# ChainSafe/co-zkvms

Measured on AMD Instinct MI355X. Metric: RISC-V cycles proved/sec (co-Jolt hot path: PST13 commit + dense GKR grand product + openings), higher is better.
Workload: dtype u32-limb BN254 Fr/Fq (254-bit Montgomery integers); 1 GPU; configs[1] restated (SURVEY 8d): 2^20-cycle trace per GPU, plain prover, 128 polys (64 Fr + 32 u16 + 16 u32 + 16 flags) PST13 batch commit, dense grand product 8 x 2^21 leaves, batch evaluate + opening reduction + PST13 open; log_n=20, polys=128, gp_batch=8, parallelism=single GPU, ranks_per_gpu=1

## Files before the change

### co-zkvms_amd/build.py

```python
import os
import subprocess
import sys

HERE = os.path.dirname(os.path.abspath(__file__))
CSRC = os.path.join(HERE, "csrc")
OUT = os.path.join(HERE, "libcozk.so")
PRIMS_SRC = os.path.join(os.path.dirname(HERE), "tests", "native", "prims.hip")
PRIMS_OUT = os.path.join(os.path.dirname(HERE), "tests", "native", "libcozk_prims.so")
HIPCC_FLAGS = ["--offload-arch=gfx950", "-O3", "-std=c++17", "-fPIC"]
SOURCES = ["capi.hip", "msm.hip", "poly.hip", "harness.hip", "shm_hub.hip", "ring.hip", "shamir.hip", "lasso_witness.hip", "rw_memory_witness.hip", "rw_memory_leaves.hip", "ts_range_witness.hip"]
HEADERS = [os.path.join("host", "spartan_pub_workers.hpp"), "fr9.hip.hpp", "fr9_consts.inc", os.path.join("host", "flow_harness.hpp"), os.path.join("host", "ts_range_proof.hpp"), os.path.join("host", "rw_memory_proof.hpp"), os.path.join("host", "jolt_r1cs.hpp"), os.path.join("host", "spartan_jolt.hpp"), "spartan_inner.inc", "ff.hip.hpp", "prf.hip.hpp", "ff_macc.inc", "ff_mul2.inc", "ec.hip.hpp", "fq9.hip.hpp", "fq9_consts.inc", "fq9_mac.inc", "fq9_mul.inc", "common.hpp", "lasso_walk.hip.hpp", "radix_pass.hip.hpp", "poly.hip.hpp", "toggle_layer.inc", "spartan_group.inc", "sparse_layer.inc", "primary_sumcheck.inc", "primary_group.inc", "shamir_deal.hip.hpp", "spartan_outer.inc", "outer_group.inc", "logup.inc", "compact_open.inc", "output_check.inc", os.path.join("host", "memory_proof.hpp"), os.path.join("host", "wire.hpp"), os.path.join("host", "net.hpp"), os.path.join("host", "prover.hpp"), os.path.join("host", "sparse_rule.hpp"), os.path.join("host", "split.hpp"), os.path.join("host", "split_harness.hpp"), os.path.join("host", "spartan_harness.hpp"), os.path.join("host", "lookups_harness.hpp"), os.path.join("host", "outer_harness.hpp"), os.path.join("host", "runner.hpp"), os.path.join("host", "shamir_gp.hpp"), os.path.join("host", "shamir_harness.hpp"), os.path.join("host", "shamir_spartan.hpp"), os.path.join("host", "shamir_jolt_spartan.hpp"), os.path.join("host", "shamir_primary.hpp"), os.path.join("..", "..", "include", "cozk.h")]


def _newer(target, deps):
    if not os.path.exists(target):
        return True
    t = os.path.getmtime(target)
    return any(os.path.getmtime(d) > t for d in deps)


def build(force=False, verbose=True):
    srcs = [os.path.join(CSRC, s) for s in SOURCES]
    deps = srcs + [os.path.join(CSRC, h) for h in HEADERS]
    objs = []
    os.makedirs(os.path.join(HERE, "build"), exist_ok=True)
    procs = []
    for s in srcs:
        o = os.path.join(HERE, "build", os.path.basename(s) + ".o")
        objs.append(o)
        if force or _newer(o, deps):
            cmd = ["hipcc"] + HIPCC_FLAGS + ["-c", s, "-o", o]
            if verbose:
                print(" ".join(cmd), flush=True)
            procs.append((cmd, subprocess.Popen(cmd)))
    for cmd, p in procs:
        if p.wait() != 0:
            raise RuntimeError("hipcc failed: " + " ".join(cmd))
    if force or procs or _newer(OUT, objs):
        cmd = ["hipcc", "--offload-arch=gfx950", "-shared", "-fPIC", "-o", OUT] + objs + ["-ldl"]
        if verbose:
            print(" ".join(cmd), flush=True)
        subprocess.check_call(cmd)
    build_prims(force, verbose)
    return OUT


def build_prims(force=False, verbose=True):
    if force or _newer(PRIMS_OUT, [PRIMS_SRC] + [os.path.join(CSRC, h) for h in HEADERS]):
        tmp = PRIMS_OUT[:-3] + ".tmp.so"
        cmd = ["hipcc"] + HIPCC_FLAGS + ["-shared", PRIMS_SRC, "-o", tmp]
        if verbose:
            print(" ".join(cmd), flush=True)
        subprocess.check_call(cmd)
        os.replace(tmp, PRIMS_OUT)
    return PRIMS_OUT


if __name__ == "__main__":
    if "--prims" in sys.argv:
        build_prims(force="--force" in sys.argv)
    else:
        build(force="--force" in sys.argv)
```

### co-zkvms_amd/csrc/ff.hip.hpp

```cpp
#pragma once
#include <hip/hip_runtime.h>
#include <stdint.h>

#define FF_HD __host__ __device__ __forceinline__
#if defined(__HIP_DEVICE_COMPILE__)
#include "ff_macc.inc"
#include "ff_mul2.inc"
#endif

struct alignas(16) fe {
    uint32_t l[8];
};

struct FrParams {
    static constexpr uint32_t MOD[8] = {0xf0000001u, 0x43e1f593u, 0x79b97091u, 0x2833e848u,
                                        0x8181585du, 0xb85045b6u, 0xe131a029u, 0x30644e72u};
    static constexpr uint32_t INV = 0xefffffffu;
    static constexpr uint32_t ONE[8] = {0x4ffffffbu, 0xac96341cu, 0x9f60cd29u, 0x36fc7695u,
                                        0x7879462eu, 0x666ea36fu, 0x9a07df2fu, 0x0e0a77c1u};
    static constexpr uint32_t R2[8] = {0xae216da7u, 0x1bb8e645u, 0xe35c59e3u, 0x53fe3ab1u,
                                       0x53bb8085u, 0x8c49833du, 0x7f4e44a5u, 0x0216d0b1u};
};

struct FqParams {
// ... 280 lines not shown
        MACC5_VS(lo, hi, m[0], m[1], m[2], m[3], m[4], P_(5), P_(4), P_(3), P_(2), P_(1));
        MSTEP_(5);
        MACC7_VV(lo, hi, A[0], A[1], A[2], A[3], A[4], A[5], A[6], B[6], B[5], B[4], B[3], B[2], B[1], B[0]);
        MACC7_VV(lo, hi, C[0], C[1], C[2], C[3], C[4], C[5], C[6], D[6], D[5], D[4], D[3], D[2], D[1], D[0]);
        MACC6_VS(lo, hi, m[0], m[1], m[2], m[3], m[4], m[5], P_(6), P_(5), P_(4), P_(3), P_(2), P_(1));
        MSTEP_(6);
        MACC8_VV(lo, hi, A[0], A[1], A[2], A[3], A[4], A[5], A[6], A[7], B[7], B[6], B[5], B[4], B[3], B[2], B[1], B[0]);
        MACC8_VV(lo, hi, C[0], C[1], C[2], C[3], C[4], C[5], C[6], C[7], D[7], D[6], D[5], D[4], D[3], D[2], D[1], D[0]);
        MACC7_VS(lo, hi, m[0], m[1], m[2], m[3], m[4], m[5], m[6], P_(7), P_(6), P_(5), P_(4), P_(3), P_(2), P_(1));
        MSTEP_(7);
        MACC7_VV(lo, hi, A[1], A[2], A[3], A[4], A[5], A[6], A[7], B[7], B[6], B[5], B[4], B[3], B[2], B[1]);
        MACC7_VV(lo, hi, C[1], C[2], C[3], C[4], C[5], C[6], C[7], D[7], D[6], D[5], D[4], D[3], D[2], D[1]);
        MACC7_VS(lo, hi, m[1], m[2], m[3], m[4], m[5], m[6], m[7], P_(7), P_(6), P_(5), P_(4), P_(3), P_(2), P_(1));
        r[0] = (uint32_t)lo; SHIFT_();
        MACC6_VV(lo, hi, A[2], A[3], A[4], A[5], A[6], A[7], B[7], B[6], B[5], B[4], B[3], B[2]);
        MACC6_VV(lo, hi, C[2], C[3], C[4], C[5], C[6], C[7], D[7], D[6], D[5], D[4], D[3], D[2]);
        MACC6_VS(lo, hi, m[2], m[3], m[4], m[5], m[6], m[7], P_(7), P_(6), P_(5), P_(4), P_(3), P_(2));
        r[1] = (uint32_t)lo; SHIFT_();
        MACC5_VV(lo, hi, A[3], A[4], A[5], A[6], A[7], B[7], B[6], B[5], B[4], B[3]);
        MACC5_VV(lo, hi, C[3], C[4], C[5], C[6], C[7], D[7], D[6], D[5], D[4], D[3]);
        MACC5_VS(lo, hi, m[3], m[4], m[5], m[6], m[7], P_(7), P_(6), P_(5), P_(4), P_(3));
        r[2] = (uint32_t)lo; SHIFT_();
        MACC4_VV(lo, hi, A[4], A[5], A[6], A[7], B[7], B[6], B[5], B[4]);
        MACC4_VV(lo, hi, C[4], C[5], C[6], C[7], D[7], D[6], D[5], D[4]);
        MACC4_VS(lo, hi, m[4], m[5], m[6], m[7], P_(7), P_(6), P_(5), P_(4));
        r[3] = (uint32_t)lo; SHIFT_();
        MACC3_VV(lo, hi, A[5], A[6], A[7], B[7], B[6], B[5]);
        MACC3_VV(lo, hi, C[5], C[6], C[7], D[7], D[6], D[5]);
        MACC3_VS(lo, hi, m[5], m[6], m[7], P_(7), P_(6), P_(5));
        r[4] = (uint32_t)lo; SHIFT_();
        MACC2_VV(lo, hi, A[6], A[7], B[7], B[6]);
        MACC2_VV(lo, hi, C[6], C[7], D[7], D[6]);
        MACC2_VS(lo, hi, m[6], m[7], P_(7), P_(6));
        r[5] = (uint32_t)lo; SHIFT_();
        MACC1_VV(lo, hi, A[7], B[7]);
        MACC1_VV(lo, hi, C[7], D[7]);
        MACC1_VS(lo, hi, m[7], P_(7));
        r[6] = (uint32_t)lo;
        r[7] = (uint32_t)(lo >> 32);
#undef P_
#undef SHIFT_
#undef MSTEP_
        fe o;
#pragma unroll
        for (int i = 0; i < 8; i++) o.l[i] = r[i];
        return o;
    }
#endif
    static FF_HD fe mul_sub2(const fe& a, const fe& b, const fe& c, const fe& d) { return mul_add2(a, b, neg(c), d); }

    static FF_HD void mul2(const fe& a, const fe& b, const fe& c, const fe& d, fe& o1, fe& o2) {
#if defined(__HIP_DEVICE_COMPILE__)
        uint64_t lo1 = 0, lo2 = 0;
        uint32_t hi1 = 0, hi2 = 0;
        uint32_t m1[8], m2[8], r1[8], r2[8];
        const uint32_t* A = a.l;
        const uint32_t* B = b.l;
        const uint32_t* C = c.l;
        const uint32_t* D = d.l;
        FF_MUL2_BODY
        fe t1, t2;
#pragma unroll
        for (int i = 0; i < 8; i++) {
            t1.l[i] = r1[i];
            t2.l[i] = r2[i];
        }
        o1 = reduce_once(t1);
        o2 = reduce_once(t2);
#else
        o1 = mul(a, b);
        o2 = mul(c, d);
#endif
    }

    static FF_HD fe two_mod() {
        fe r;
        uint32_t c = 0;
#pragma unroll
        for (int i = 0; i < 8; i++) {
            r.l[i] = (Pm::MOD[i] << 1) | c;
            c = Pm::MOD[i] >> 31;
        }
        return r;
    }
    static FF_HD fe lcanon(const fe& a) {
#if defined(__HIP_DEVICE_COMPILE__)
        return reduce_once(a);
#else
        return a;
#endif
    }
    static FF_HD fe lmul(const fe& a, const fe& b) {
#if defined(__HIP_DEVICE_COMPILE__)
        return mul_nr(a, b);
#else
        return mul(a, b);
#endif
    }
    static FF_HD void lmul2(const fe& a, const fe& b, const fe& c, const fe& d, fe& o1, fe& o2) {
#if defined(__HIP_DEVICE_COMPILE__)
        uint64_t lo1 = 0, lo2 = 0;
        uint32_t hi1 = 0, hi2 = 0;
        uint32_t m1[8], m2[8], r1[8], r2[8];
        const uint32_t* A = a.l;
        const uint32_t* B = b.l;
        const uint32_t* C = c.l;
        const uint32_t* D = d.l;
        FF_MUL2_BODY
#pragma unroll
        for (int i = 0; i < 8; i++) {
            o1.l[i] = r1[i];
            o2.l[i] = r2[i];
        }
#else
        o1 = mul(a, b);
        o2 = mul(c, d);
#endif
    }
    static FF_HD fe ladd(const fe& a, const fe& b) {
#if defined(__HIP_DEVICE_COMPILE__)
        fe s;
        uint64_t c = 0;
#pragma unroll
        for (int i = 0; i < 8; i++) {
            uint64_t t = (uint64_t)a.l[i] + b.l[i] + c;
            s.l[i] = (uint32_t)t;
            c = t >> 32;
        }
        const fe tm = two_mod();
        fe d;
        uint64_t borrow = 0;
#pragma unroll
        for (int i = 0; i < 8; i++) {
            uint64_t t = (uint64_t)s.l[i] - tm.l[i] - borrow;
            d.l[i] = (uint32_t)t;
            borrow = (t >> 63) & 1;
        }
        fe r;
#pragma unroll
        for (int i = 0; i < 8; i++) r.l[i] = borrow ? s.l[i] : d.l[i];
        return r;
#else
        return add(a, b);
#endif
    }
    static FF_HD fe lsub(const fe& a, const fe& b) {
#if defined(__HIP_DEVICE_COMPILE__)
        fe d;
        uint64_t borrow = 0;
#pragma unroll
        for (int i = 0; i < 8; i++) {
            uint64_t t = (uint64_t)a.l[i] - b.l[i] - borrow;
            d.l[i] = (uint32_t)t;
            borrow = (t >> 63) & 1;
        }
        const fe tm = two_mod();
        uint32_t mask = borrow ? 0xffffffffu : 0u;
        fe r;
        uint64_t c = 0;
#pragma unroll
        for (int i = 0; i < 8; i++) {
            uint64_t t = (uint64_t)d.l[i] + (tm.l[i] & mask) + c;
            r.l[i] = (uint32_t)t;
            c = t >> 32;
        }
        return r;
#else
        return sub(a, b);
#endif
    }
    static FF_HD fe ldbl(const fe& a) { return ladd(a, a); }
    static FF_HD fe lneg(const fe& a) { return lsub(zero(), a); }
    static FF_HD bool lis_zero(const fe& a) {
#if defined(__HIP_DEVICE_COMPILE__)
        uint32_t z = 0, m = 0;
#pragma unroll
        for (int i = 0; i < 8; i++) {
            z |= a.l[i];
            m |= a.l[i] ^ Pm::MOD[i];
        }
        return z == 0 || m == 0;
#else
        return is_zero(a);
#endif
    }
    static FF_HD fe lmul_sub2(const fe& a, const fe& b, const fe& c, const fe& d) {
#if defined(__HIP_DEVICE_COMPILE__)
        fe x = mul_add2_nr(a, b, lneg(c), d);
        const fe tm = two_mod();
        fe t;
        uint64_t borrow = 0;
#pragma unroll
        for (int i = 0; i < 8; i++) {
            uint64_t u = (uint64_t)x.l[i] - tm.l[i] - borrow;
            t.l[i] = (uint32_t)u;
            borrow = (u >> 63) & 1;
        }
        uint32_t mask = borrow ? 0u : 0xffffffffu;
        fe r;
        uint64_t bb = 0;
#pragma unroll
        for (int i = 0; i < 8; i++) {
            uint64_t u = (uint64_t)x.l[i] - (Pm::MOD[i] & mask) - bb;
            r.l[i] = (uint32_t)u;
            bb = (u >> 63) & 1;
        }
        return r;
#else
        return mul_sub2(a, b, c, d);
#endif
    }

    static FF_HD fe to_mont(const fe& a) { return mul(a, r2()); }
    static FF_HD fe from_mont(const fe& a) {
#if defined(__HIP_DEVICE_COMPILE__)
        uint64_t lo = 0;
        uint32_t hi = 0;
        uint32_t m[8], r[8];
        const uint32_t* A = a.l;
#define P_(j) Pm::MOD[j]
#define SHIFT_() lo = (lo >> 32) | ((uint64_t)hi << 32); hi = 0
#define ADDA_(k) { uint64_t t_ = lo + A[k]; hi += t_ < lo ? 1u : 0u; lo = t_; }
#define MSTEP_(k) m[k] = (uint32_t)lo * Pm::INV; MACC1_VS(lo, hi, m[k], P_(0)); SHIFT_()
        ADDA_(0);
        MSTEP_(0);
        ADDA_(1);
        MACC1_VS(lo, hi, m[0], P_(1));
        MSTEP_(1);
        ADDA_(2);
        MACC2_VS(lo, hi, m[0], m[1], P_(2), P_(1));
        MSTEP_(2);
        ADDA_(3);
        MACC3_VS(lo, hi, m[0], m[1], m[2], P_(3), P_(2), P_(1));
        MSTEP_(3);
        ADDA_(4);
        MACC4_VS(lo, hi, m[0], m[1], m[2], m[3], P_(4), P_(3), P_(2), P_(1));
        MSTEP_(4);
        ADDA_(5);
        MACC5_VS(lo, hi, m[0], m[1], m[2], m[3], m[4], P_(5), P_(4), P_(3), P_(2), P_(1));
        MSTEP_(5);
        ADDA_(6);
        MACC6_VS(lo, hi, m[0], m[1], m[2], m[3], m[4], m[5], P_(6), P_(5), P_(4), P_(3), P_(2), P_(1));
        MSTEP_(6);
        ADDA_(7);
        MACC7_VS(lo, hi, m[0], m[1], m[2], m[3], m[4], m[5], m[6], P_(7), P_(6), P_(5), P_(4), P_(3), P_(2), P_(1));
        MSTEP_(7);
        MACC7_VS(lo, hi, m[1], m[2], m[3], m[4], m[5], m[6], m[7], P_(7), P_(6), P_(5), P_(4), P_(3), P_(2), P_(1));
        r[0] = (uint32_t)lo; SHIFT_();
        MACC6_VS(lo, hi, m[2], m[3], m[4], m[5], m[6], m[7], P_(7), P_(6), P_(5), P_(4), P_(3), P_(2));
        r[1] = (uint32_t)lo; SHIFT_();
        MACC5_VS(lo, hi, m[3], m[4], m[5], m[6], m[7], P_(7), P_(6), P_(5), P_(4), P_(3));
        r[2] = (uint32_t)lo; SHIFT_();
        MACC4_VS(lo, hi, m[4], m[5], m[6], m[7], P_(7), P_(6), P_(5), P_(4));
        r[3] = (uint32_t)lo; SHIFT_();
        MACC3_VS(lo, hi, m[5], m[6], m[7], P_(7), P_(6), P_(5));
        r[4] = (uint32_t)lo; SHIFT_();
        MACC2_VS(lo, hi, m[6], m[7], P_(7), P_(6));
        r[5] = (uint32_t)lo; SHIFT_();
        MACC1_VS(lo, hi, m[7], P_(7));
        r[6] = (uint32_t)lo;
        r[7] = (uint32_t)(lo >> 32);
#undef P_
#undef SHIFT_
#undef ADDA_
#undef MSTEP_
        fe o;
#pragma unroll
        for (int i = 0; i < 8; i++) o.l[i] = r[i];
        return reduce_once(o);
#else
        fe o = zero();
        o.l[0] = 1;
        return mul(a, o);
#endif
    }
    static FF_HD fe from_u64(uint64_t v) {
        fe o = zero();
        o.l[0] = (uint32_t)v;
        o.l[1] = (uint32_t)(v >> 32);
        return to_mont(o);
    }
    static FF_HD fe pow(const fe& a, const uint32_t e[8]) {
        fe acc = one();
        for (int i = 7; i >= 0; i--) {
            for (int b = 31; b >= 0; b--) {
                acc = sqr(acc);
                if ((e[i] >> b) & 1) acc = mul(acc, a);
            }
        }
        return acc;
    }
    static FF_HD fe inv(const fe& a) {
        uint32_t e[8];
#pragma unroll
        for (int i = 0; i < 8; i++) e[i] = Pm::MOD[i];
        e[0] -= 2;
        return pow(a, e);
    }
};

typedef Field<FrParams> Fr;
typedef Field<FqParams> Fq;

static __device__ __forceinline__ fe fe_load(const fe* p) {
    const uint4* q = reinterpret_cast<const uint4*>(p);
    uint4 lo = q[0], hi = q[1];
    fe r;
    r.l[0] = lo.x; r.l[1] = lo.y; r.l[2] = lo.z; r.l[3] = lo.w;
    r.l[4] = hi.x; r.l[5] = hi.y; r.l[6] = hi.z; r.l[7] = hi.w;
    return r;
}
static __device__ __forceinline__ void fe_store(fe* p, const fe& v) {
    uint4* q = reinterpret_cast<uint4*>(p);
    q[0] = make_uint4(v.l[0], v.l[1], v.l[2], v.l[3]);
    q[1] = make_uint4(v.l[4], v.l[5], v.l[6], v.l[7]);
}
```

### co-zkvms_amd/csrc/poly.hip

```cpp
#include <atomic>
#include <chrono>
#include <map>
#include <mutex>
#include <string.h>
#include "poly.hip.hpp"
#include "prf.hip.hpp"
#include "fr9.hip.hpp"
#include "shamir_deal.hip.hpp"

static constexpr int PT = 256;
static constexpr int MAXBLK = 2048;
static constexpr unsigned ROUND_GRID_MAX = 1024;
static constexpr unsigned BATCH_GRID_MAX = 512;
static constexpr unsigned EVAL_GRID_MAX = 192;
static constexpr size_t LAYER_F9_MIN_CHUNKS = 1024;
static constexpr size_t LAYER_GROUPED_MIN_E1H = 512;

struct cozk_poly {
    cozk_ctx* ctx;
    int mode;
    fe* a0; fe* b0;
    bool own0;
    fe* buf[2][2];
    size_t cap[2];
    int cur;
    size_t len;
    size_t orig_len;
};

struct cozk_layer {
    cozk_ctx* ctx;
    int mode;
    fe* buf[2][2];
    size_t cap[2];
    int cur;
    size_t len;
};

struct cozk_spliteq {
    cozk_ctx* ctx;
    fe* E1[2]; fe* E2[2];
    int c1, c2;
    size_t E1_len, E2_len, E1_cap, E2_cap;
    int num_vars;
};

static inline unsigned grid_for(size_t n) { return (unsigned)((n + PT - 1) / PT); }
static inline unsigned grid_capped(size_t n, unsigned cap = MAXBLK) {
    size_t g = (n + PT - 1) / PT;
    return (unsigned)(g > cap ? cap : (g ? g : 1));
}
static inline unsigned sum_grid(unsigned gx) {
    const char* e = getenv("COZK_SUM_GRID_MAX");
    const long n = e ? atol(e) : 0;
    return n > 0 && (unsigned long)n < gx ? (unsigned)n : gx;
}

static unsigned eval_grid_max() {
    static const unsigned cap = getenv("COZK_EVAL_GX") ? (unsigned)atoi(getenv("COZK_EVAL_GX")) : EVAL_GRID_MAX;
    return cap;
}

static unsigned resident_grid(const void* kernel, size_t nblocks_needed, int device) {
    static const int legacy = getenv("COZK_RESIDENT_GRID") && atoi(getenv("COZK_RESIDENT_GRID")) == 0;
    if (legacy) return (unsigned)(nblocks_needed < 1024 ? (nblocks_needed ? nblocks_needed : 1) : 1024);
    static std::mutex mu;
    static std::map<std::pair<const void*, int>, unsigned> cache;
    unsigned cap;
    {
        std::lock_guard<std::mutex> g(mu);
        auto it = cache.find({kernel, device});
        if (it == cache.end()) {
            int per_cu = 0, cus = 0;
            HIP_TRY(hipOccupancyMaxActiveBlocksPerMultiprocessor(&per_cu, kernel, PT, 0));
            HIP_TRY(hipDeviceGetAttribute(&cus, hipDeviceAttributeMultiprocessorCount, device));
            unsigned v = (unsigned)(per_cu > 0 ? per_cu : 1) * (unsigned)(cus > 0 ? cus : 1);
            if (v > MAXBLK) v = MAXBLK;
            it = cache.emplace(std::make_pair(kernel, device), v).first;
        }
        cap = it->second;
    }
    return (unsigned)(nblocks_needed < cap ? (nblocks_needed ? nblocks_needed : 1) : cap);
}

static const fe* poly_a(const cozk_poly* p) { return p->cur < 0 ? p->a0 : p->buf[p->cur][0]; }
static const fe* poly_b(const cozk_poly* p) { return p->cur < 0 ? p->b0 : p->buf[p->cur][1]; }

template <int NC, int ORDER>
__global__ void __launch_bounds__(PT) k_poly_bind(const fe* __restrict__ ia, const fe* __restrict__ ib, fe* oa, fe* ob,
                                               size_t n_out, fe r) {
    size_t i = (size_t)blockIdx.x * PT + threadIdx.x;
    if (i >= n_out) return;
    size_t lo_i = ORDER == COZK_LOW_TO_HIGH ? 2 * i : i;
    size_t hi_i = ORDER == COZK_LOW_TO_HIGH ? 2 * i + 1 : i + n_out;
    Sh<NC> lo = sh_load<NC>(ia, ib, lo_i), hi = sh_load<NC>(ia, ib, hi_i);
    sh_store<NC>(oa, ob, i, sh_lerp<NC>(lo, hi, r));
}

template <int NC>
__global__ void __launch_bounds__(PT) k_poly_eval_chi(const fe* const* __restrict__ pa, const fe* const* __restrict__ pb,
                                                   const size_t* __restrict__ lens, const fe* __restrict__ chi, int k,
                                                   fe* __restrict__ partial) {
    __shared__ fe sh4[4];
    const int p0 = 2 * blockIdx.y, p1 = p0 + 1;
    const bool two = p1 < k;
    const fe* a0 = pa[p0];
    const fe* b0 = NC == 2 ? pb[p0] : nullptr;
    const fe* a1 = two ? pa[p1] : nullptr;
    const fe* b1 = (two && NC == 2) ? pb[p1] : nullptr;
    const size_t n0 = lens[p0], n1 = two ? lens[p1] : 0;
    const size_t n = n0 > n1 ? n0 : n1;
    FrWide w0, w1;
    fr_wide_zero(w0);
    fr_wide_zero(w1);
    for (size_t i = (size_t)blockIdx.x * PT + threadIdx.x; i < n; i += (size_t)gridDim.x * PT) {
        fe c = fe_load(chi + i);
        if (i < n0) fr_wide_mac(w0, sh_ab_sum<NC>(sh_load<NC>(a0, b0, i)), c);
        if (i < n1) fr_wide_mac(w1, sh_ab_sum<NC>(sh_load<NC>(a1, b1, i)), c);
    }
    fe acc = fr_block_sum(fr_wide_reduce(w0), sh4);
    if (threadIdx.x == 0) fe_store(partial + (size_t)p0 * gridDim.x + blockIdx.x, acc);
    if (two) {
        acc = fr_block_sum(fr_wide_reduce(w1), sh4);
        if (threadIdx.x == 0) fe_store(partial + (size_t)p1 * gridDim.x + blockIdx.x, acc);
    }
}

struct RoundPublish {
    unsigned* ticket;
    uint32_t* flag;
    uint32_t seq;
};
__global__ void __launch_bounds__(PT) k_finish_sums(const fe* __restrict__ partial, unsigned nper, fe scale, int apply_scale,
                                                 fe* __restrict__ out, RoundPublish pub) {
    __shared__ fe sh4[4];
    fe acc = Fr::zero();
    for (unsigned x = threadIdx.x; x < nper; x += PT) acc = Fr::add(acc, fe_load(partial + (size_t)blockIdx.x * nper + x));
    acc = fr_block_sum(acc, sh4);
    if (threadIdx.x == 0) {
        fe_store(out + blockIdx.x, apply_scale ? Fr::mul(acc, scale) : acc);
        if (pub.ticket) {
            __threadfence_system();
            if (atomicAdd(pub.ticket, 1u) == gridDim.x - 1) {
                *pub.ticket = 0;
                __threadfence_system();
                __hip_atomic_store(pub.flag, pub.seq, __ATOMIC_RELEASE, __HIP_MEMORY_SCOPE_SYSTEM);
            }
        }
    }
}

template <int NC>
__global__ void __launch_bounds__(PT) k_poly_dot_public(const fe* __restrict__ a, const fe* __restrict__ b,
                                                     const fe* __restrict__ pub, size_t n, fe* __restrict__ partial) {
    __shared__ fe sh4[4];
    FrWide w[NC];
#pragma unroll
    for (int k = 0; k < NC; k++) fr_wide_zero(w[k]);
    for (size_t i = (size_t)blockIdx.x * PT + threadIdx.x; i < n; i += (size_t)gridDim.x * PT) {
        Sh<NC> s = sh_load<NC>(a, b, i);
        fe p = fe_load(pub + i);
#pragma unroll
        for (int k = 0; k < NC; k++) fr_wide_mac(w[k], s.c[k], p);
    }
#pragma unroll
    for (int k = 0; k < NC; k++) {
        fe v = fr_block_sum(fr_wide_reduce(w[k]), sh4);
        if (threadIdx.x == 0) fe_store(partial + (size_t)k * gridDim.x + blockIdx.x, v);
    }
}

template <int NC>
__global__ void __launch_bounds__(PT) k_poly_lincomb(const fe* const* __restrict__ pa, const fe* const* __restrict__ pb,
                                                  const size_t* __restrict__ lens, const fe* __restrict__ coeffs, int k,
                                                  fe* oa, fe* ob, size_t n) {
    size_t i = (size_t)blockIdx.x * PT + threadIdx.x;
    if (i >= n) return;
    Sh<NC> acc;
    if (k >= 8) {
        FrWide w[NC];
#pragma unroll
        for (int c = 0; c < NC; c++) fr_wide_zero(w[c]);
        for (int j = 0; j < k; j++) {
            if (i < lens[j]) {
                fe cf = fe_load(coeffs + j);
                if (pa[j]) fr_wide_mac(w[0], fe_load(pa[j] + i), cf);
                if (NC == 2 && pb[j]) fr_wide_mac(w[NC - 1], fe_load(pb[j] + i), cf);
            }
        }
#pragma unroll
        for (int c = 0; c < NC; c++) acc.c[c] = fr_wide_reduce(w[c]);
        sh_store<NC>(oa, ob, i, acc);
        return;
    }
    for (int c = 0; c < NC; c++) acc.c[c] = Fr::zero();
    for (int j = 0; j < k; j++) {
        if (i < lens[j]) {
            fe cf = fe_load(coeffs + j);
            if (pa[j]) acc.c[0] = Fr::add(acc.c[0], Fr::mul(fe_load(pa[j] + i), cf));
            if (NC == 2 && pb[j]) acc.c[NC - 1] = Fr::add(acc.c[NC - 1], Fr::mul(fe_load(pb[j] + i), cf));
        }
    }
    sh_store<NC>(oa, ob, i, acc);
}

struct OpenQuadArgs {
    const fe* a[16];
    const fe* b[16];
    const fe* eq[16];
    size_t half[16];
};
template <int NC>
__global__ void __launch_bounds__(PT) k_open_quadratic_args(OpenQuadArgs args, fe* __restrict__ partial) {
    __shared__ fe sh4[4];
    const fe* a = args.a[blockIdx.y];
    const fe* b = NC == 2 ? args.b[blockIdx.y] : nullptr;
    const fe* eq = args.eq[blockIdx.y];
    size_t h = args.half[blockIdx.y];
    fe e0 = Fr::zero(), e2 = Fr::zero();
    for (size_t i = (size_t)blockIdx.x * PT + threadIdx.x; i < h; i += (size_t)gridDim.x * PT) {
        fe q0 = fe_load(eq + i), q1 = fe_load(eq + i + h);
        fe p0 = sh_ab_sum<NC>(sh_load<NC>(a, b, i)), p1 = sh_ab_sum<NC>(sh_load<NC>(a, b, i + h));
        e0 = Fr::add(e0, Fr::mul(p0, q0));
        fe pb2 = Fr::sub(Fr::dbl(p1), p0), qb2 = Fr::sub(Fr::dbl(q1), q0);
        e2 = Fr::add(e2, Fr::mul(pb2, qb2));
    }
    e0 = fr_block_sum(e0, sh4);
    if (threadIdx.x == 0) fe_store(partial + (size_t)(2 * blockIdx.y) * gridDim.x + blockIdx.x, e0);
    e2 = fr_block_sum(e2, sh4);
    if (threadIdx.x == 0) fe_store(partial + (size_t)(2 * blockIdx.y + 1) * gridDim.x + blockIdx.x, e2);
}

struct SmallCol {
    const void* p;
    int kind;
};
static __device__ __forceinline__ uint64_t small_load(const SmallCol& c, size_t i) {
    switch (c.kind) {
        case COZK_SCALAR_U8: return reinterpret_cast<const uint8_t*>(c.p)[i];
        case COZK_SCALAR_U16: return reinterpret_cast<const uint16_t*>(c.p)[i];
        case COZK_SCALAR_U32: return reinterpret_cast<const uint32_t*>(c.p)[i];
        default: return reinterpret_cast<const uint64_t*>(c.p)[i];
    }
}
template <int NC>
__global__ void __launch_bounds__(PT) k_fingerprint_leaves(const SmallCol* __restrict__ cols, const fe* __restrict__ cs, int ks,
                                                        const fe* const* __restrict__ pa, const fe* const* __restrict__ pb,
                                                        const fe* __restrict__ ds, int kp, fe constant, int pub_a, int pub_b, fe* oa, fe* ob,
                                                        size_t n) {
    size_t i = (size_t)blockIdx.x * PT + threadIdx.x;
    if (i >= n) return;
    fe pub = constant;
    for (int k = 0; k < ks; k++) {
        uint64_t v = small_load(cols[k], i);
        fe x = Fr::zero();
        x.l[0] = (uint32_t)v;
        x.l[1] = (uint32_t)(v >> 32);
        pub = Fr::add(pub, Fr::mul(fe_load(cs + k), x));
    }
    Sh<NC> acc;
    for (int c = 0; c < NC; c++) acc.c[c] = Fr::zero();
    for (int j = 0; j < kp; j++) {
        fe d = fe_load(ds + j);
        if (pa[j]) acc.c[0] = Fr::add(acc.c[0], Fr::mul(fe_load(pa[j] + i), d));
        if (NC == 2 && pb[j]) acc.c[NC - 1] = Fr::add(acc.c[NC - 1], Fr::mul(fe_load(pb[j] + i), d));
    }
    if (pub_a) acc.c[0] = Fr::add(acc.c[0], pub);
    if (NC == 2 && pub_b) acc.c[NC - 1] = Fr::add(acc.c[NC - 1], pub);
    sh_store<NC>(oa, ob, i, acc);
}

struct FingerprintArgs {
    SmallCol cols[16];
    fe cs[16];
    const fe* pa[8];
    const fe* pb[8];
    fe ds[8];
};
template <int NC>
__global__ void __launch_bounds__(PT) k_fingerprint_leaves_args(FingerprintArgs a, int ks, int kp, fe constant, int pub_a, int pub_b, fe* oa, fe* ob,
                                                             size_t n) {
    size_t i = (size_t)blockIdx.x * PT + threadIdx.x;
    if (i >= n) return;
    fe pub = constant;
    for (int k = 0; k < ks; k++) {
        uint64_t v = small_load(a.cols[k], i);
        fe x = Fr::zero();
        x.l[0] = (uint32_t)v;
        x.l[1] = (uint32_t)(v >> 32);
        pub = Fr::add(pub, Fr::mul(a.cs[k], x));
    }
    Sh<NC> acc;
    for (int c = 0; c < NC; c++) acc.c[c] = Fr::zero();
    for (int j = 0; j < kp; j++) {
        if (a.pa[j]) acc.c[0] = Fr::add(acc.c[0], Fr::mul(fe_load(a.pa[j] + i), a.ds[j]));
        if (NC == 2 && a.pb[j]) acc.c[NC - 1] = Fr::add(acc.c[NC - 1], Fr::mul(fe_load(a.pb[j] + i), a.ds[j]));
    }
    if (pub_a) acc.c[0] = Fr::add(acc.c[0], pub);
    if (NC == 2 && pub_b) acc.c[NC - 1] = Fr::add(acc.c[NC - 1], pub);
    sh_store<NC>(oa, ob, i, acc);
}

template <int NC>
__global__ void __launch_bounds__(PT) k_open_quadratic(const fe* const* __restrict__ pa, const fe* const* __restrict__ pb,
                                                    const fe* const* __restrict__ peq, const size_t* __restrict__ halves,
                                                    fe* __restrict__ partial) {
    __shared__ fe sh4[4];
    const fe* a = pa[blockIdx.y];
    const fe* b = NC == 2 ? pb[blockIdx.y] : nullptr;
    const fe* eq = peq[blockIdx.y];
    size_t h = halves[blockIdx.y];
    fe e0 = Fr::zero(), e2 = Fr::zero();
    for (size_t i = (size_t)blockIdx.x * PT + threadIdx.x; i < h; i += (size_t)gridDim.x * PT) {
        fe q0 = fe_load(eq + i), q1 = fe_load(eq + i + h);
        fe p0 = sh_ab_sum<NC>(sh_load<NC>(a, b, i)), p1 = sh_ab_sum<NC>(sh_load<NC>(a, b, i + h));
        e0 = Fr::add(e0, Fr::mul(p0, q0));
        fe pb2 = Fr::sub(Fr::dbl(p1), p0), qb2 = Fr::sub(Fr::dbl(q1), q0);
        e2 = Fr::add(e2, Fr::mul(pb2, qb2));
    }
    e0 = fr_block_sum(e0, sh4);
    if (threadIdx.x == 0) fe_store(partial + (size_t)(2 * blockIdx.y) * gridDim.x + blockIdx.x, e0);
    e2 = fr_block_sum(e2, sh4);
    if (threadIdx.x == 0) fe_store(partial + (size_t)(2 * blockIdx.y + 1) * gridDim.x + blockIdx.x, e2);
}

__global__ void __launch_bounds__(PT) k_pst_fold(const fe* __restrict__ r, fe* __restrict__ q, fe* __restrict__ rn, size_t half, fe p) {
    size_t i = (size_t)blockIdx.x * PT + threadIdx.x;
    if (i >= half) return;
    fe lo = fe_load(r + 2 * i), hi = fe_load(r + 2 * i + 1);
    fe d = Fr::sub(hi, lo);
    fe_store(q + i, d);
    fe_store(rn + i, Fr::add(lo, Fr::mul(d, p)));
}

template <int NC>
static __device__ __forceinline__ void layer_bind_chunk(const fe* ia, const fe* ib, size_t len_in, size_t ci, const fe& r, fe* oa, fe* ob, Sh<NC>& lo,
                                                        Sh<NC>& hi) {
    Sh<NC> u0 = sh_load_or_zero<NC>(ia, ib, 4 * ci, len_in), u1 = sh_load_or_zero<NC>(ia, ib, 4 * ci + 1, len_in);
    Sh<NC> u2 = sh_load_or_zero<NC>(ia, ib, 4 * ci + 2, len_in), u3 = sh_load_or_zero<NC>(ia, ib, 4 * ci + 3, len_in);
    lo = sh_lerp<NC>(u0, u2, r);
    sh_store<NC>(oa, ob, 2 * ci, lo);
    hi = sh_lerp<NC>(u1, u3, r);
    sh_store<NC>(oa, ob, 2 * ci + 1, hi);
}

static __device__ __forceinline__ void eq3(const fe& e0, const fe& e1, fe out[3]) {
    fe m = Fr::sub(e1, e0);
    out[0] = e0;
    out[1] = Fr::add(e1, m);
    out[2] = Fr::add(out[1], m);
}

static __device__ __forceinline__ size_t layer_chunk_count(size_t len, bool nested, size_t E1_half, size_t E2_len) {
    size_t nch = (len + 3) / 4;
    size_t limit = nested ? E1_half * E2_len : E2_len / 2;
    return nch > limit ? limit : nch;
}

static __device__ __forceinline__ void split_eq_at(bool nested, const fe* E1, int log_E1_half, const fe* E2, size_t c, fe e[3], fe& scale) {
    if (nested) {
        size_t x2 = c >> log_E1_half, x1 = c & (((size_t)1 << log_E1_half) - 1);
        eq3(fe_load(E1 + 2 * x1), fe_load(E1 + 2 * x1 + 1), e);
        scale = fe_load(E2 + x2);
    } else {
        eq3(fe_load(E2 + 2 * c), fe_load(E2 + 2 * c + 1), e);
    }
}
static __device__ __forceinline__ void layer_eq_at(bool nested, const fe* E1, size_t E1_half, const fe* E2, size_t c, fe e[3], fe& scale) {
    split_eq_at(nested, E1, __ffsll((long long)E1_half) - 1, E2, c, e, scale);
}
template <int NESTED>
static __device__ __forceinline__ size_t split_eq_limit(size_t E2_len, int log_E1_half) {
    return NESTED ? ((size_t)E2_len << log_E1_half) : E2_len / 2;
}
static __device__ __forceinline__ void partial_row_sum(fe v, fe* sh, fe* __restrict__ partial, size_t row) {
    v = fr_block_sum(v, sh);
    if (threadIdx.x == 0) fe_store(partial + row * gridDim.x + blockIdx.x, v);
}

template <int NC>
static __device__ __forceinline__ void layer_terms(const Sh<NC>& l0, const Sh<NC>& r0, const Sh<NC>& l1, const Sh<NC>& r1, const fe e[3], bool nested,
                                                   const fe& scale, fe& t0, fe& t2, fe& t3) {
    Sh<NC> ml = sh_sub<NC>(l1, l0), mr = sh_sub<NC>(r1, r0);
    Sh<NC> l2 = sh_add<NC>(l1, ml), r2 = sh_add<NC>(r1, mr);
    Sh<NC> l3 = sh_add<NC>(l2, ml), r3 = sh_add<NC>(r2, mr);
    t0 = Fr::mul(sh_local_mul<NC>(l0, r0), e[0]);
    t2 = Fr::mul(sh_local_mul<NC>(l2, r2), e[1]);
    t3 = Fr::mul(sh_local_mul<NC>(l3, r3), e[2]);
    if (nested) {
        t0 = Fr::mul(t0, scale);
        t2 = Fr::mul(t2, scale);
        t3 = Fr::mul(t3, scale);
    }
}

template <class Out>
static __device__ __forceinline__ void layer_finish(fe s0, fe s2, fe s3, fe* sh, Out out) {
    s0 = fr_block_sum(s0, sh);
    if (threadIdx.x == 0) fe_store(out(0), s0);
    s2 = fr_block_sum(s2, sh);
    if (threadIdx.x == 0) fe_store(out(1), s2);
    s3 = fr_block_sum(s3, sh);
    if (threadIdx.x == 0) fe_store(out(2), s3);
}

static __device__ __forceinline__ fe fold_pair(const fe* in, size_t i, const fe& r) {
    fe lo = fe_load(in + 2 * i), hi = fe_load(in + 2 * i + 1);
    return Fr::add(lo, Fr::mul(Fr::sub(hi, lo), r));
}

template <int NC>
__global__ void __launch_bounds__(PT) k_layer_bind(const fe* __restrict__ ia, const fe* __restrict__ ib, fe* oa, fe* ob,
                                                size_t len, fe r) {
    size_t c = (size_t)blockIdx.x * PT + threadIdx.x;
    size_t nch = (len + 3) / 4;
    if (c >= nch) return;
    Sh<NC> lo, hi;
    layer_bind_chunk<NC>(ia, ib, len, c, r, oa, ob, lo, hi);
}

template <int NC, int NESTED>
__global__ void __launch_bounds__(PT) k_layer_cubic(const fe* __restrict__ a, const fe* __restrict__ b, size_t len,
                                                 const fe* __restrict__ E1, size_t E1_half, const fe* __restrict__ E2,
                                                 size_t E2_len, fe* __restrict__ partial) {
    __shared__ fe sh4[4];
    const size_t nch = layer_chunk_count(len, NESTED, E1_half, E2_len);
    fe s0 = Fr::zero(), s2 = Fr::zero(), s3 = Fr::zero();
    for (size_t c = (size_t)blockIdx.x * PT + threadIdx.x; c < nch; c += (size_t)gridDim.x * PT) {
        fe e[3];
        fe scale;
        layer_eq_at(NESTED, E1, E1_half, E2, c, e, scale);
        Sh<NC> l0 = sh_load_or_zero<NC>(a, b, 4 * c, len), r0 = sh_load_or_zero<NC>(a, b, 4 * c + 1, len);
        Sh<NC> l1 = sh_load_or_zero<NC>(a, b, 4 * c + 2, len), r1 = sh_load_or_zero<NC>(a, b, 4 * c + 3, len);
        fe t0, t2, t3;
        layer_terms<NC>(l0, r0, l1, r1, e, NESTED, scale, t0, t2, t3);
        s0 = Fr::add(s0, t0);
        s2 = Fr::add(s2, t2);
        s3 = Fr::add(s3, t3);
    }
    layer_finish(s0, s2, s3, sh4, [&](unsigned k) { return partial + k * gridDim.x + blockIdx.x; });
}

template <int NC, int NESTED>
__global__ void __launch_bounds__(PT) k_layer_bind_cubic(const fe* __restrict__ ia, const fe* __restrict__ ib, fe* oa, fe* ob, size_t len_in, fe r,
                                                      const fe* __restrict__ E1, size_t E1_half, const fe* __restrict__ E2, size_t E2_len,
                                                      fe* __restrict__ partial) {
    __shared__ fe sh4[4];
    const size_t nch_in = (len_in + 3) / 4;
    const size_t len_out = 2 * nch_in;
    const size_t nch_out = (len_out + 3) / 4;
    const size_t nsum = layer_chunk_count(len_out, NESTED, E1_half, E2_len);
    fe s0 = Fr::zero(), s2 = Fr::zero(), s3 = Fr::zero();
    for (size_t c = (size_t)blockIdx.x * PT + threadIdx.x; c < nch_out; c += (size_t)gridDim.x * PT) {
        Sh<NC> v[4];
#pragma unroll
        for (int h = 0; h < 2; h++) {
            size_t ci = 2 * c + h;
            if (ci < nch_in) {
                layer_bind_chunk<NC>(ia, ib, len_in, ci, r, oa, ob, v[2 * h], v[2 * h + 1]);
            } else {
                for (int k = 0; k < NC; k++) v[2 * h].c[k] = v[2 * h + 1].c[k] = Fr::zero();
            }
        }
        if (c < nsum) {
            fe e[3];
            fe scale;
            layer_eq_at(NESTED, E1, E1_half, E2, c, e, scale);
            fe t0, t2, t3;
            layer_terms<NC>(v[0], v[1], v[2], v[3], e, NESTED, scale, t0, t2, t3);
            s0 = Fr::add(s0, t0);
            s2 = Fr::add(s2, t2);
            s3 = Fr::add(s3, t3);
        }
    }
    layer_finish(s0, s2, s3, sh4, [&](unsigned k) { return partial + k * gridDim.x + blockIdx.x; });
}

struct Layer9Group {
    f9 g0, g2, g3;
    size_t x2;
};
static __device__ __forceinline__ void layer9_group_flush(Layer9Group& grp, const fe* __restrict__ E2, f9& s0, f9& s2, f9& s3) {
    if (grp.x2 == (size_t)-1) return;
    const f9 sc = f9_from_fe(fe_load(E2 + grp.x2));
    s0 = f9_norm(fr9_add(s0, fr9_mul(grp.g0, sc)));
    s2 = f9_norm(fr9_add(s2, fr9_mul(grp.g2, sc)));
    s3 = f9_norm(fr9_add(s3, fr9_mul(grp.g3, sc)));
}
template <int NESTED>
static __device__ __forceinline__ void layer9_fold(size_t it, f9& s0, f9& s2, f9& s3, Layer9Group& grp) {
    if (it == 0 || (it & (FR9_FOLD_PERIOD - 1)) != 0) return;
    fr9_fold(s0);
    fr9_fold(s2);
    fr9_fold(s3);
    if (NESTED == 2) {
        fr9_fold(grp.g0);
        fr9_fold(grp.g2);
        fr9_fold(grp.g3);
    }
}
template <int NC, int NESTED>
static __device__ __forceinline__ void layer9_terms(const Sh9<NC>& l0, const Sh9<NC>& r0, const Sh9<NC>& l1, const Sh9<NC>& r1, const fe* __restrict__ E1,
                                                    size_t E1_half, int e1_shift, const fe* __restrict__ E2, size_t c, f9& s0, f9& s2, f9& s3,
                                                    Layer9Group& grp) {
    f9 e0, e1;
    if (NESTED == 2) {
        const size_t x2 = c >> e1_shift, x1 = c & (E1_half - 1);
        if (x2 != grp.x2) {
            layer9_group_flush(grp, E2, s0, s2, s3);
            grp.g0 = grp.g2 = grp.g3 = fr9_zero();
            grp.x2 = x2;
        }
        e0 = f9_from_fe(fe_load(E1 + 2 * x1));
        e1 = f9_from_fe(fe_load(E1 + 2 * x1 + 1));
    } else if (NESTED) {
        const size_t x2 = c >> e1_shift, x1 = c & (E1_half - 1);
        const f9 sc = f9_from_fe(fe_load(E2 + x2));
        e0 = fr9_mul(f9_from_fe(fe_load(E1 + 2 * x1)), sc);
        e1 = fr9_mul(f9_from_fe(fe_load(E1 + 2 * x1 + 1)), sc);
    } else {
        e0 = f9_from_fe(fe_load(E2 + 2 * c));
        e1 = f9_from_fe(fe_load(E2 + 2 * c + 1));
    }
    const f9 me = f9_norm(f9_sub(e1, FR9_C2, e0));
    const f9 e2 = fr9_add(e1, me), e3 = fr9_add(e2, me);
    const Sh9<NC> ml = sh9_diff<NC>(l1, l0), mr = sh9_diff<NC>(r1, r0);
    const Sh9<NC> l2 = sh9_add_norm<NC>(l1, ml), r2 = sh9_add_norm<NC>(r1, mr);
    const Sh9<NC> l3 = sh9_add_norm<NC>(l2, ml), r3 = sh9_add_norm<NC>(r2, mr);
    f9& a0 = NESTED == 2 ? grp.g0 : s0;
    f9& a2 = NESTED == 2 ? grp.g2 : s2;
    f9& a3 = NESTED == 2 ? grp.g3 : s3;
    a0 = f9_norm(fr9_add(a0, fr9_mul(e0, sh9_local_mul<NC>(l0, r0))));
    a2 = f9_norm(fr9_add(a2, fr9_mul(e2, sh9_local_mul<NC>(l2, r2))));
    a3 = f9_norm(fr9_add(a3, fr9_mul(e3, sh9_local_mul<NC>(l3, r3))));
}
static __device__ __forceinline__ void layer9_walk(int nested, size_t nch, size_t& first, size_t& end, size_t& step) {
    if (nested == 2) {
        const size_t per = ((nch + gridDim.x - 1) / gridDim.x + PT - 1) / PT * PT;
        first = (size_t)blockIdx.x * per + (threadIdx.x & ~63u);
        end = (size_t)(blockIdx.x + 1) * per < nch ? (size_t)(blockIdx.x + 1) * per : nch;
        step = PT;
    } else {
        first = (size_t)blockIdx.x * PT + (threadIdx.x & ~63u);
        end = nch;
        step = (size_t)gridDim.x * PT;
    }
}
template <int NESTED>
static __device__ __forceinline__ void layer9_finish(const f9& s0, const f9& s2, const f9& s3, fe* __restrict__ partial, fe* sh4) {
    const f9 K = f9_const(NESTED ? FR9_K3 : FR9_K2);
    fe v = fr_block_sum(fr9_to_canonical(fr9_mul(s0, K)), sh4);
    if (threadIdx.x == 0) fe_store(partial + blockIdx.x, v);
    v = fr_block_sum(fr9_to_canonical(fr9_mul(s2, K)), sh4);
    if (threadIdx.x == 0) fe_store(partial + gridDim.x + blockIdx.x, v);
    v = fr_block_sum(fr9_to_canonical(fr9_mul(s3, K)), sh4);
    if (threadIdx.x == 0) fe_store(partial + 2 * gridDim.x + blockIdx.x, v);
}


static constexpr int ST_ROW = 144;
static constexpr int ST_WAVE_BYTES = 64 * ST_ROW;
static __device__ __forceinline__ void stage_fence() {
    __builtin_amdgcn_fence(__ATOMIC_RELEASE, "wavefront");
    __builtin_amdgcn_wave_barrier();
    __builtin_amdgcn_fence(__ATOMIC_ACQUIRE, "wavefront");
}
static __device__ __forceinline__ void stage_in_rows(const char* __restrict__ g, size_t row_stride, char* st, fe out[4]) {
    const int lane = threadIdx.x & 63, piece = lane & 7, sub = lane >> 3;
    uint4 t[8];
#pragma unroll
    for (int k = 0; k < 8; k++) t[k] = *reinterpret_cast<const uint4*>(g + (size_t)(8 * k + sub) * row_stride + 16 * piece);
#pragma unroll
    for (int k = 0; k < 8; k++) *reinterpret_cast<uint4*>(st + (8 * k + sub) * ST_ROW + 16 * piece) = t[k];
    stage_fence();
#pragma unroll
    for (int j = 0; j < 4; j++) {
        const uint4 lo = *reinterpret_cast<const uint4*>(st + lane * ST_ROW + 32 * j);
        const uint4 hi = *reinterpret_cast<const uint4*>(st + lane * ST_ROW + 32 * j + 16);
        out[j].l[0] = lo.x; out[j].l[1] = lo.y; out[j].l[2] = lo.z; out[j].l[3] = lo.w;
        out[j].l[4] = hi.x; out[j].l[5] = hi.y; out[j].l[6] = hi.z; out[j].l[7] = hi.w;
    }
    stage_fence();
}
static __device__ __forceinline__ void stage_out_rows(char* __restrict__ g, char* st, const fe in[4], size_t row_stride = 128) {
    const int lane = threadIdx.x & 63, piece = lane & 7, sub = lane >> 3;
#pragma unroll
    for (int j = 0; j < 4; j++) {
        *reinterpret_cast<uint4*>(st + lane * ST_ROW + 32 * j) = make_uint4(in[j].l[0], in[j].l[1], in[j].l[2], in[j].l[3]);
        *reinterpret_cast<uint4*>(st + lane * ST_ROW + 32 * j + 16) = make_uint4(in[j].l[4], in[j].l[5], in[j].l[6], in[j].l[7]);
    }
    stage_fence();
#pragma unroll
    for (int k = 0; k < 8; k++)
        *reinterpret_cast<uint4*>(g + (size_t)(8 * k + sub) * row_stride + 16 * piece) = *reinterpret_cast<const uint4*>(st + (8 * k + sub) * ST_ROW + 16 * piece);
    stage_fence();
}

template <int NC, int NESTED>
__global__ void __launch_bounds__(PT) k_layer_cubic9(const fe* __restrict__ a, const fe* __restrict__ b, size_t len, const fe* __restrict__ E1, size_t E1_half,
                                                  const fe* __restrict__ E2, size_t E2_len, fe* __restrict__ partial) {
    __shared__ fe sh4[4];
    __shared__ __attribute__((aligned(16))) char stage[PT / 64][ST_WAVE_BYTES];
    char* st = stage[threadIdx.x >> 6];
    size_t nch = (len + 3) / 4;
    const size_t limit = NESTED ? E1_half * E2_len : E2_len / 2;
    if (nch > limit) nch = limit;
    const int e1_shift = NESTED ? __ffsll((long long)E1_half) - 1 : 0;
    f9 s0 = fr9_zero(), s2 = fr9_zero(), s3 = fr9_zero();
    Layer9Group grp;
    grp.g0 = grp.g2 = grp.g3 = fr9_zero();
    grp.x2 = (size_t)-1;
    size_t c_first, c_end, c_step;
    layer9_walk(NESTED, nch, c_first, c_end, c_step);
    size_t it = 0;
    for (size_t c0 = c_first; c0 < c_end; c0 += c_step, it++) {
        layer9_fold<NESTED>(it, s0, s2, s3, grp);
        const size_t c = c0 + (threadIdx.x & 63);
        if (c0 + 64 <= nch && 4 * (c0 + 64) <= len) {
            Sh9<NC> q[4];
            const fe* comp[2] = {a, b};
#pragma unroll
            for (int k = 0; k < NC; k++) {
                fe raw[4];
                stage_in_rows(reinterpret_cast<const char*>(comp[k] + 4 * c0), 128, st, raw);
#pragma unroll
                for (int j = 0; j < 4; j++) q[j].c[k] = f9_from_fe(raw[j]);
            }
            layer9_terms<NC, NESTED>(q[0], q[1], q[2], q[3], E1, E1_half, e1_shift, E2, c, s0, s2, s3, grp);
        } else if (c < nch) {
            const Sh9<NC> l0 = sh9_load_or_zero<NC>(a, b, 4 * c, len), r0 = sh9_load_or_zero<NC>(a, b, 4 * c + 1, len);
            const Sh9<NC> l1 = sh9_load_or_zero<NC>(a, b, 4 * c + 2, len), r1 = sh9_load_or_zero<NC>(a, b, 4 * c + 3, len);
            layer9_terms<NC, NESTED>(l0, r0, l1, r1, E1, E1_half, e1_shift, E2, c, s0, s2, s3, grp);
        }
    }
    if (NESTED == 2) layer9_group_flush(grp, E2, s0, s2, s3);
    layer9_finish<NESTED>(s0, s2, s3, partial, sh4);
}

template <int NC, int NESTED>
__global__ void __launch_bounds__(PT) k_layer_bind_cubic9(const fe* __restrict__ ia, const fe* __restrict__ ib, fe* oa, fe* ob, size_t len_in, fe r5,
                                                       const fe* __restrict__ E1, size_t E1_half, const fe* __restrict__ E2, size_t E2_len,
                                                       fe* __restrict__ partial) {
    __shared__ fe sh4[4];
    const size_t nch_in = (len_in + 3) / 4;
    const size_t len_out = 2 * nch_in;
    const size_t nch_out = (len_out + 3) / 4;
    const size_t limit = NESTED ? E1_half * E2_len : E2_len / 2;
    const int e1_shift = NESTED ? __ffsll((long long)E1_half) - 1 : 0;
    const f9 r9 = f9_from_fe(r5);
    f9 s0 = fr9_zero(), s2 = fr9_zero(), s3 = fr9_zero();
    __shared__ __attribute__((aligned(16))) char stage[PT / 64][ST_WAVE_BYTES];
    char* st = stage[threadIdx.x >> 6];
    Layer9Group grp;
    grp.g0 = grp.g2 = grp.g3 = fr9_zero();
    grp.x2 = (size_t)-1;
    size_t c_first, c_end, c_step;
    layer9_walk(NESTED, nch_out, c_first, c_end, c_step);
    size_t it = 0;
    for (size_t c0 = c_first; c0 < c_end; c0 += c_step, it++) {
        layer9_fold<NESTED>(it, s0, s2, s3, grp);
        const size_t c = c0 + (threadIdx.x & 63);
        Sh9<NC> v[4];
        if (c0 + 64 <= nch_out && 8 * (c0 + 64) <= len_in) {
            const fe* icomp[2] = {ia, ib};
            fe* ocomp[2] = {oa, ob};
#pragma unroll
            for (int h = 0; h < 2; h++) {
                Sh9<NC> u[4];
#pragma unroll
                for (int k = 0; k < NC; k++) {
                    fe raw[4];
                    stage_in_rows(reinterpret_cast<const char*>(icomp[k] + 8 * c0 + 4 * h), 256, st, raw);
#pragma unroll
                    for (int j = 0; j < 4; j++) u[j].c[k] = f9_from_fe(raw[j]);
                }
                v[2 * h] = sh9_lerp<NC>(u[0], u[2], r9);
                v[2 * h + 1] = sh9_lerp<NC>(u[1], u[3], r9);
            }
#pragma unroll
            for (int k = 0; k < NC; k++) {
                fe outv[4];
#pragma unroll
                for (int j = 0; j < 4; j++) outv[j] = fr9_to_canonical(v[j].c[k]);
                stage_out_rows(reinterpret_cast<char*>(ocomp[k] + 4 * c0), st, outv);
            }
            if (c < limit) layer9_terms<NC, NESTED>(v[0], v[1], v[2], v[3], E1, E1_half, e1_shift, E2, c, s0, s2, s3, grp);
            continue;
        }
        if (c >= nch_out) continue;
#pragma unroll
        for (int h = 0; h < 2; h++) {
            const size_t ci = 2 * c + h;
            if (ci < nch_in) {
                const Sh9<NC> u0 = sh9_load_or_zero<NC>(ia, ib, 4 * ci, len_in), u1 = sh9_load_or_zero<NC>(ia, ib, 4 * ci + 1, len_in);
                const Sh9<NC> u2 = sh9_load_or_zero<NC>(ia, ib, 4 * ci + 2, len_in), u3 = sh9_load_or_zero<NC>(ia, ib, 4 * ci + 3, len_in);
                v[2 * h] = sh9_lerp<NC>(u0, u2, r9);
                v[2 * h + 1] = sh9_lerp<NC>(u1, u3, r9);
                sh9_store<NC>(oa, ob, 2 * ci, v[2 * h]);
                sh9_store<NC>(oa, ob, 2 * ci + 1, v[2 * h + 1]);
            } else {
                for (int k = 0; k < NC; k++) v[2 * h].c[k] = v[2 * h + 1].c[k] = fr9_zero();
            }
        }
        if (c < limit) layer9_terms<NC, NESTED>(v[0], v[1], v[2], v[3], E1, E1_half, e1_shift, E2, c, s0, s2, s3, grp);
    }
    if (NESTED == 2) layer9_group_flush(grp, E2, s0, s2, s3);
    layer9_finish<NESTED>(s0, s2, s3, partial, sh4);
}

static constexpr int RT = 1024;
static constexpr size_t ROUND_SMALL_MAX = 2048;
template <int NC>
__global__ void __launch_bounds__(RT) k_layer_round_small(const fe* __restrict__ ia, const fe* __restrict__ ib, fe* oa, fe* ob, size_t len_in,
                                                       int do_bind, fe r, const fe* fold_in, fe* fold_out, size_t fold_n, fe* scale_vec,
                                                       size_t scale_n, const fe* ca, const fe* cb, size_t len, const fe* E1, size_t E1_half,
                                                       const fe* E2, size_t E2_len, int nested, fe* __restrict__ res) {
    __shared__ fe sh16[16];
    if (do_bind) {
        size_t nch_in = (len_in + 3) / 4;
        for (size_t c = threadIdx.x; c < nch_in; c += RT) {
            Sh<NC> lo, hi;
            layer_bind_chunk<NC>(ia, ib, len_in, c, r, oa, ob, lo, hi);
        }
        for (size_t i = threadIdx.x; i < fold_n; i += RT) fe_store(fold_out + i, fold_pair(fold_in, i, r));
        __syncthreads();
        if (scale_n) {
            fe s = fe_load(fold_out);
            for (size_t i = threadIdx.x; i < scale_n; i += RT) fe_store(scale_vec + i, Fr::mul(fe_load(scale_vec + i), s));
            __syncthreads();
        }
    }
    size_t nch = (len + 3) / 4;
    size_t limit = nested ? E1_half * E2_len : E2_len / 2;
    if (nch > limit) nch = limit;
    fe s0 = Fr::zero(), s2 = Fr::zero(), s3 = Fr::zero();
    for (size_t c = threadIdx.x; c < nch; c += RT) {
        fe e[3];
        fe scale = Fr::zero();
        if (nested) {
            size_t x2 = c >> (__ffsll((long long)E1_half) - 1), x1 = c & (E1_half - 1);
            eq3(fe_load(E1 + 2 * x1), fe_load(E1 + 2 * x1 + 1), e);
            scale = fe_load(E2 + x2);
        } else {
            eq3(fe_load(E2 + 2 * c), fe_load(E2 + 2 * c + 1), e);
        }
        Sh<NC> l0 = sh_load_or_zero<NC>(ca, cb, 4 * c, len), r0 = sh_load_or_zero<NC>(ca, cb, 4 * c + 1, len);
        Sh<NC> l1 = sh_load_or_zero<NC>(ca, cb, 4 * c + 2, len), r1 = sh_load_or_zero<NC>(ca, cb, 4 * c + 3, len);
        fe t0, t2, t3;
        layer_terms<NC>(l0, r0, l1, r1, e, nested, scale, t0, t2, t3);
        s0 = Fr::add(s0, t0);
        s2 = Fr::add(s2, t2);
        s3 = Fr::add(s3, t3);
    }
    layer_finish(s0, s2, s3, sh16, [&](unsigned k) { return res + k; });
}

struct LayerGroupArgs {
    const fe* ia[COZK_LAYER_GROUP_MAX];
    const fe* ib[COZK_LAYER_GROUP_MAX];
    fe* oa[COZK_LAYER_GROUP_MAX];
    fe* ob[COZK_LAYER_GROUP_MAX];
};
template <int NC>
__global__ void __launch_bounds__(RT) k_layer_group_round_small(LayerGroupArgs a, size_t len_in, int do_bind, fe r, size_t len, const fe* E1, size_t E1_half,
                                                             const fe* E2, size_t E2_len, int nested, fe* __restrict__ res) {
    __shared__ fe sh16[16];
    const unsigned m = blockIdx.x;
    const size_t c = threadIdx.x;
    const fe *ca = a.ia[m], *cb = a.ib[m];
    if (do_bind) {
        const fe *ia = a.ia[m], *ib = a.ib[m];
        fe *oa = a.oa[m], *ob = a.ob[m];
        if (c < (len_in + 3) / 4) {
#pragma unroll 1
            for (int h = 0; h < 2; h++) {
                const Sh<NC> lo = sh_load_or_zero<NC>(ia, ib, 4 * c + h, len_in), hi = sh_load_or_zero<NC>(ia, ib, 4 * c + 2 + h, len_in);
                sh_store<NC>(oa, ob, 2 * c + h, sh_lerp<NC>(lo, hi, r));
            }
        }
        __syncthreads();
        ca = oa;
        cb = ob;
    }
    const bool on = c < layer_chunk_count(len, nested, E1_half, E2_len);
    const fe* ep = E2 + 2 * c;
    const fe* sp = nullptr;
    if (nested) {
        ep = E1 + 2 * (c & (E1_half - 1));
        sp = E2 + (c >> (__ffsll((long long)E1_half) - 1));
    }
    auto side = [&](int s, int X) {
        const Sh<NC> v0 = sh_load_or_zero<NC>(ca, cb, 4 * c + s, len), v1 = sh_load_or_zero<NC>(ca, cb, 4 * c + 2 + s, len);
        if (X == 0) return v0;
        const Sh<NC> d = sh_sub<NC>(v1, v0);
        Sh<NC> v = sh_add<NC>(v1, d);
        if (X == 3) v = sh_add<NC>(v, d);
        return v;
    };
#pragma unroll 1
    for (int p = 0; p < 3; p++) {
        const int X = p ? p + 1 : 0;
        fe t = Fr::zero();
        if (on) {
            fe e = fe_load(ep);
            if (X) {
                const fe e1 = fe_load(ep + 1), d = Fr::sub(e1, e);
                e = Fr::add(e1, d);
                if (X == 3) e = Fr::add(e, d);
            }
            if (nested) e = Fr::mul(e, fe_load(sp));
            t = Fr::mul(sh_local_mul<NC>(side(0, X), side(1, X)), e);
        }
        t = fr_block_sum(t, sh16);
        if (threadIdx.x == 0) fe_store(res + 3 * m + p, t);
    }
}

static constexpr int GFT = 64;
template <int NC>
__global__ void __launch_bounds__(GFT) k_layer_group_final(LayerGroupArgs a, size_t len_in, int do_bind, fe r, fe* __restrict__ res) {
    const unsigned m = blockIdx.x, j = threadIdx.x;
    if (j >= 2) return;
    const fe *ia = a.ia[m], *ib = a.ib[m];
    Sh<NC> v;
    if (do_bind) {
        v = sh_lerp<NC>(sh_load_or_zero<NC>(ia, ib, j, len_in), sh_load_or_zero<NC>(ia, ib, j + 2, len_in), r);
        sh_store<NC>(a.oa[m], a.ob[m], j, v);
    } else {
        v = sh_load<NC>(ia, ib, j);
    }
    for (int c = 0; c < NC; c++) fe_store(res + (size_t)(2 * m + j) * NC + c, v.c[c]);
}

struct alignas(64) RoundMailbox {
    uint32_t cmd[16];
    uint32_t pad0[16];
    uint32_t res_seq;
    uint32_t status;
    uint32_t pad2[14];
    fe res[4];
    unsigned long long dbg[8];
};
static constexpr long long MB_TICKS_PER_S = 100000000ll;
static int resident_timeout_s() {
    const char* e = getenv("COZK_RESIDENT_TIMEOUT_S");
    int t = e ? atoi(e) : 10;
    return t < 1 ? 1 : (t > 600 ? 600 : t);
}
static constexpr size_t ROUND_PERSIST_MAX = 2048;

template <int NC, int TRACE>
__global__ void __launch_bounds__(RT) k_layer_rounds_persistent(fe* la0, fe* lb0, fe* la1, fe* lb1, int lcur, size_t len, fe* e1_0, fe* e1_1,
                                                             int c1, size_t E1_len, fe* e2_0, fe* e2_1, int c2, size_t E2_len, int nrounds,
                                                             int bind_first, fe r_first, RoundMailbox* mb, long long timeout_ticks) {
    __shared__ fe sh16[16];
    __shared__ fe sh_r;
    __shared__ int sh_ok;
    fe* la[2] = {la0, la1};
    fe* lb[2] = {lb0, lb1};
    fe* e1[2] = {e1_0, e1_1};
    fe* e2[2] = {e2_0, e2_1};
    uint32_t seq = 0;
    long long tk0 = TRACE ? wall_clock64() : 0, tk_wait = 0, tk_bind = 0, tk_cubic = 0, tk_pub = 0;
    for (int round = 0; round <= nrounds; round++) {
        bool do_bind = round > 0 || bind_first;
        fe r = r_first;
        if (TRACE) tk0 = wall_clock64();
        if (round > 0) {
            if (threadIdx.x < 64) {
                typedef uint32_t v4u __attribute__((ext_vector_type(4)));
                const int lane = threadIdx.x;
                const long long t0 = wall_clock64();
                int ok = 1;
                v4u v = {0u, 0u, 0u, 0u};
                for (;;) {
                    if (lane < 4) v = *reinterpret_cast<volatile v4u*>(&mb->cmd[4 * lane]);
                    const unsigned long long ready = __ballot(lane < 3 && v.w == (uint32_t)round);
                    const unsigned long long aborted = __ballot(lane == 3 && v.x != 0u);
                    if ((ready & 7ull) == 7ull) break;
                    if (aborted) {
                        ok = 0;
                        if (lane == 0) __hip_atomic_store(&mb->status, 2u, __ATOMIC_RELEASE, __HIP_MEMORY_SCOPE_SYSTEM);
                        break;
                    }
                    if (__shfl((int)(wall_clock64() - t0 > timeout_ticks), 0)) {
                        ok = 0;
                        if (lane == 0) __hip_atomic_store(&mb->status, 1u, __ATOMIC_RELEASE, __HIP_MEMORY_SCOPE_SYSTEM);
                        break;
                    }
                    __builtin_amdgcn_s_sleep(2);
                }
                fe rr;
                rr.l[0] = __shfl(v.x, 0); rr.l[1] = __shfl(v.y, 0); rr.l[2] = __shfl(v.z, 0);
                rr.l[3] = __shfl(v.x, 1); rr.l[4] = __shfl(v.y, 1); rr.l[5] = __shfl(v.z, 1);
                rr.l[6] = __shfl(v.x, 2); rr.l[7] = __shfl(v.y, 2);
                if (lane == 0) {
                    if (ok) sh_r = rr;
                    sh_ok = ok;
                }
            }
            __syncthreads();
            if (!sh_ok) return;
            r = sh_r;
        }
        if (TRACE) {
            long long t = wall_clock64();
            tk_wait += t - tk0;
            tk0 = t;
        }
        if (do_bind) {
            const fe *ia = la[lcur], *ib = lb[lcur];
            fe *oa = la[1 - lcur], *ob = lb[1 - lcur];
            size_t nch_in = (len + 3) / 4;
            for (size_t c = threadIdx.x; c < nch_in; c += RT) {
                Sh<NC> lo, hi;
                layer_bind_chunk<NC>(ia, ib, len, c, r, oa, ob, lo, hi);
            }
            lcur = 1 - lcur;
            len = 2 * nch_in;
            if (E1_len == 1) {
                size_t n = E2_len / 2;
                const fe* in = e2[c2];
                fe* out = e2[1 - c2];
                for (size_t i = RT - 1 - threadIdx.x; i < n; i += RT) fe_store(out + i, fold_pair(in, i, r));
                c2 = 1 - c2;
                E2_len = n;
                __syncthreads();
            } else {
                size_t n = E1_len / 2;
                const fe* in = e1[c1];
                fe* out = e1[1 - c1];
                for (size_t i = RT - 1 - threadIdx.x; i < n; i += RT) fe_store(out + i, fold_pair(in, i, r));
                c1 = 1 - c1;
                E1_len = n;
                __syncthreads();
                if (n == 1) {
                    fe sc = fe_load(e1[c1]);
                    fe* v = e2[c2];
                    for (size_t i = threadIdx.x; i < E2_len; i += RT) fe_store(v + i, Fr::mul(fe_load(v + i), sc));
                    __syncthreads();
                }
            }
        }
        seq++;
        if (TRACE) {
            long long t = wall_clock64();
            tk_bind += t - tk0;
            tk0 = t;
        }
        if (round == nrounds) {
            if (threadIdx.x == 0) {
                mb->dbg[0] = (unsigned long long)tk_wait;
                mb->dbg[1] = (unsigned long long)tk_bind;
                mb->dbg[2] = (unsigned long long)tk_cubic;
                mb->dbg[3] = (unsigned long long)tk_pub;
                fe z = Fr::zero();
                fe v[4] = {fe_load(la[lcur]), NC == 2 ? fe_load(lb[lcur]) : z, fe_load(la[lcur] + 1), NC == 2 ? fe_load(lb[lcur] + 1) : z};
                for (int k = 0; k < 4; k++) fe_store(&mb->res[k], v[k]);
                __threadfence_system();
                __hip_atomic_store(&mb->res_seq, seq, __ATOMIC_RELEASE, __HIP_MEMORY_SCOPE_SYSTEM);
            }
            return;
        }
        const fe *ca = la[lcur], *cb = lb[lcur];
        const fe *E1 = e1[c1], *E2 = e2[c2];
        const bool nested = E1_len != 1;
        const size_t E1_half = E1_len / 2;
        const size_t nch = layer_chunk_count(len, nested, E1_half, E2_len);
        const int wave = threadIdx.x >> 6;
        const int pt = wave / 5;
        fe acc = Fr::zero();
        if (pt < 3) {
            for (size_t c = threadIdx.x - 320 * pt; c < nch; c += 320) {
                fe e0, e1v, ek;
                if (nested) {
                    size_t x2 = c >> (__ffsll((long long)E1_half) - 1), x1 = c & (E1_half - 1);
                    e0 = fe_load(E1 + 2 * x1);
                    e1v = fe_load(E1 + 2 * x1 + 1);
                } else {
                    e0 = fe_load(E2 + 2 * c);
                    e1v = fe_load(E2 + 2 * c + 1);
                }
                Sh<NC> l0 = sh_load_or_zero<NC>(ca, cb, 4 * c, len), r0 = sh_load_or_zero<NC>(ca, cb, 4 * c + 1, len);
                Sh<NC> lk = l0, rk = r0;
                ek = e0;
                if (pt > 0) {
                    Sh<NC> l1 = sh_load_or_zero<NC>(ca, cb, 4 * c + 2, len), r1 = sh_load_or_zero<NC>(ca, cb, 4 * c + 3, len);
                    Sh<NC> ml = sh_sub<NC>(l1, l0), mr = sh_sub<NC>(r1, r0);
                    fe me = Fr::sub(e1v, e0);
                    lk = sh_add<NC>(l1, ml);
                    rk = sh_add<NC>(r1, mr);
                    ek = Fr::add(e1v, me);
                    if (pt == 2) {
                        lk = sh_add<NC>(lk, ml);
                        rk = sh_add<NC>(rk, mr);
                        ek = Fr::add(ek, me);
                    }
                }
                fe lr = sh_local_mul<NC>(lk, rk);
                fe es = nested ? Fr::mul(ek, fe_load(E2 + (c >> (__ffsll((long long)E1_half) - 1)))) : ek;
                acc = Fr::add(acc, Fr::mul(lr, es));
            }
        }
        acc = fr_wave_sum(acc);
        __syncthreads();
        if ((threadIdx.x & 63) == 0) sh16[wave] = acc;
        __syncthreads();
        if (TRACE) {
            long long t = wall_clock64();
            tk_cubic += t - tk0;
            tk0 = t;
        }
        if (threadIdx.x < 3) {
            fe v = sh16[5 * threadIdx.x];
            for (int i = 1; i < 5; i++) v = Fr::add(v, sh16[5 * threadIdx.x + i]);
            fe_store(&mb->res[threadIdx.x], v);
            __threadfence_system();
        }
        __syncthreads();
        if (threadIdx.x == 0) __hip_atomic_store(&mb->res_seq, seq, __ATOMIC_RELEASE, __HIP_MEMORY_SCOPE_SYSTEM);
        if (TRACE) {
            long long t = wall_clock64();
            tk_pub += t - tk0;
            tk0 = t;
        }
    }
}

template <int NC>
__global__ void __launch_bounds__(PT) k_layer_output(const fe* __restrict__ a, const fe* __restrict__ b, size_t len,
                                                  fe* __restrict__ out, size_t n_out, int masked, prf_key key_self,
                                                  prf_key key_prev, uint64_t ctr) {
    size_t j = (size_t)blockIdx.x * PT + threadIdx.x;
    if (j >= n_out) return;
    Sh<NC> l = sh_load_or_zero<NC>(a, b, 2 * j, len), r = sh_load_or_zero<NC>(a, b, 2 * j + 1, len);
    fe v = sh_local_mul<NC>(l, r);
    if (masked) v = Fr::add(v, Fr::sub(prf_fr(key_self, ctr + j), prf_fr(key_prev, ctr + j)));
    fe_store(out + j, v);
}

template <int NC>
__global__ void __launch_bounds__(PT) k_mul_vec_local(const fe* __restrict__ xa, const fe* __restrict__ xb,
                                                   const fe* __restrict__ ya, const fe* __restrict__ yb, size_t n,
                                                   fe* __restrict__ out, int masked, prf_key key_self, prf_key key_prev,
                                                   uint64_t ctr) {
    size_t j = (size_t)blockIdx.x * PT + threadIdx.x;
    if (j >= n) return;
    fe v = sh_local_mul<NC>(sh_load<NC>(xa, xb, j), sh_load<NC>(ya, yb, j));
    if (masked) v = Fr::add(v, Fr::sub(prf_fr(key_self, ctr + j), prf_fr(key_prev, ctr + j)));
    fe_store(out + j, v);
}

struct ProdRoundPtrs {
    const fe* a[4];
    const fe* b[4];
};
template <int NC, int M>
__global__ void __launch_bounds__(PT) k_prod_round(ProdRoundPtrs tab, int shared_idx, size_t half, int degree, fe* __restrict__ partial) {
    const fe* const* pa = tab.a;
    const fe* const* pb = tab.b;
    __shared__ fe sh4[4];
    fe acc[4];
    for (int e = 0; e < 4; e++) acc[e] = Fr::zero();
    for (size_t i = (size_t)blockIdx.x * PT + threadIdx.x; i < half; i += (size_t)gridDim.x * PT) {
        fe cur[M], step[M];
        for (int j = 0; j < M; j++) {
            fe lo, hi;
            if (NC == 2 && j == shared_idx) {
                lo = Fr::add(fe_load(pa[j] + i), fe_load(pb[j] + i));
                hi = Fr::add(fe_load(pa[j] + i + half), fe_load(pb[j] + i + half));
            } else {
                lo = fe_load(pa[j] + i);
                hi = fe_load(pa[j] + i + half);
            }
            step[j] = Fr::sub(hi, lo);
            cur[j] = lo;
        }
        for (int e = 0; e < degree; e++) {
            if (e == 1)
                for (int j = 0; j < M; j++) cur[j] = Fr::add(Fr::add(cur[j], step[j]), step[j]);
            else if (e > 1)
                for (int j = 0; j < M; j++) cur[j] = Fr::add(cur[j], step[j]);
            fe prod = cur[0];
            for (int j = 1; j < M; j++) prod = Fr::mul(prod, cur[j]);
            acc[e] = Fr::add(acc[e], prod);
        }
    }
    for (int e = 0; e < degree; e++) {
        fe v = fr_block_sum(acc[e], sh4);
        if (threadIdx.x == 0) fe_store(partial + (size_t)e * gridDim.x + blockIdx.x, v);
    }
}

template <int NC>
__global__ void __launch_bounds__(PT) k_spartan_first(const fe* __restrict__ aa, const fe* __restrict__ ab, const fe* __restrict__ ba,
                                                   const fe* __restrict__ bb, const fe* __restrict__ ca, const fe* __restrict__ cb,
                                                   const fe* __restrict__ pub, size_t half, fe* __restrict__ partial) {
    __shared__ fe sh4[4];
    fe accp[4], accc[4];
    for (int e = 0; e < 4; e++) {
        accp[e] = Fr::zero();
        accc[e] = Fr::zero();
    }
    for (size_t b = (size_t)blockIdx.x * PT + threadIdx.x; b < half; b += (size_t)gridDim.x * PT) {
        Sh<NC> A = sh_load<NC>(aa, ab, 2 * b), B = sh_load<NC>(ba, bb, 2 * b), C = sh_load<NC>(ca, cb, 2 * b);
        Sh<NC> sA = sh_sub<NC>(sh_load<NC>(aa, ab, 2 * b + 1), A), sB = sh_sub<NC>(sh_load<NC>(ba, bb, 2 * b + 1), B),
               sC = sh_sub<NC>(sh_load<NC>(ca, cb, 2 * b + 1), C);
        fe P = fe_load(pub + 2 * b);
        fe sP = Fr::sub(fe_load(pub + 2 * b + 1), P);
        for (int e = 0; e < 4; e++) {
            accp[e] = Fr::add(accp[e], Fr::mul(sh_local_mul<NC>(A, B), P));
            accc[e] = Fr::add(accc[e], Fr::mul(sh_ab_sum<NC>(C), P));
            A = sh_add<NC>(A, sA);
            B = sh_add<NC>(B, sB);
            C = sh_add<NC>(C, sC);
            P = Fr::add(P, sP);
        }
    }
    for (int e = 0; e < 4; e++) {
        fe v = fr_block_sum(accp[e], sh4);
        if (threadIdx.x == 0) fe_store(partial + (size_t)e * gridDim.x + blockIdx.x, v);
        fe w = fr_block_sum(accc[e], sh4);
        if (threadIdx.x == 0) fe_store(partial + (size_t)(4 + e) * gridDim.x + blockIdx.x, w);
    }
}

template <int NC>
__global__ void __launch_bounds__(PT) k_spartan_second(const fe* __restrict__ za, const fe* __restrict__ zb, const fe* __restrict__ pa,
                                                    const fe* __restrict__ pbv, const fe* __restrict__ pc, fe c0, fe c1, fe c2,
                                                    size_t half, fe* __restrict__ partial) {
    __shared__ fe sh4[4];
    fe acc[NC][3];
    for (int k = 0; k < NC; k++)
        for (int e = 0; e < 3; e++) acc[k][e] = Fr::zero();
    for (size_t b = (size_t)blockIdx.x * PT + threadIdx.x; b < half; b += (size_t)gridDim.x * PT) {
        Sh<NC> Z = sh_load<NC>(za, zb, 2 * b);
        Sh<NC> sZ = sh_sub<NC>(sh_load<NC>(za, zb, 2 * b + 1), Z);
        fe A = fe_load(pa + 2 * b), B = fe_load(pbv + 2 * b), C = fe_load(pc + 2 * b);
        fe sA = Fr::sub(fe_load(pa + 2 * b + 1), A), sB = Fr::sub(fe_load(pbv + 2 * b + 1), B), sC = Fr::sub(fe_load(pc + 2 * b + 1), C);
        for (int e = 0; e < 3; e++) {
            fe lin = Fr::add(Fr::add(Fr::mul(A, c0), Fr::mul(B, c1)), Fr::mul(C, c2));
            for (int k = 0; k < NC; k++) acc[k][e] = Fr::add(acc[k][e], Fr::mul(Z.c[k], lin));
            Z = sh_add<NC>(Z, sZ);
            A = Fr::add(A, sA);
            B = Fr::add(B, sB);
            C = Fr::add(C, sC);
        }
    }
    for (int k = 0; k < NC; k++)
        for (int e = 0; e < 3; e++) {
            fe v = fr_block_sum(acc[k][e], sh4);
            if (threadIdx.x == 0) fe_store(partial + (size_t)(3 * k + e) * gridDim.x + blockIdx.x, v);
        }
}

static constexpr uint32_t SPMV_LONG = 64;
static constexpr uint32_t SPMV_CHUNK = 2048;
template <int NC>
__global__ void __launch_bounds__(PT) k_sparse_matvec3(const uint32_t* __restrict__ row_ptr, const uint32_t* __restrict__ col,
                                                    const fe* __restrict__ va, const fe* __restrict__ vb, const fe* __restrict__ vc,
                                                    const fe* __restrict__ za, const fe* __restrict__ zb, size_t nrows,
                                                    fe* oa0, fe* oa1, fe* ob0, fe* ob1, fe* oc0, fe* oc1,
                                                    uint32_t* __restrict__ q, uint32_t* __restrict__ q_rows, uint32_t* __restrict__ q_items) {
    size_t r = (size_t)blockIdx.x * PT + threadIdx.x;
    if (r >= nrows) return;
    uint32_t e0 = row_ptr[r], e1 = row_ptr[r + 1];
    if (e1 - e0 > SPMV_LONG) {
        uint32_t nchunks = (e1 - e0 + SPMV_CHUNK - 1) / SPMV_CHUNK;
        uint32_t ri = atomicAdd(&q[0], 1u);
        uint32_t first = atomicAdd(&q[1], nchunks);
        q_rows[3 * ri] = (uint32_t)r;
        q_rows[3 * ri + 1] = first;
        q_rows[3 * ri + 2] = nchunks;
        for (uint32_t j = 0; j < nchunks; j++) {
            q_items[2 * (first + j)] = (uint32_t)r;
            q_items[2 * (first + j) + 1] = j;
        }
        return;
    }
    Sh<NC> A, B, C;
    for (int k = 0; k < NC; k++) A.c[k] = B.c[k] = C.c[k] = Fr::zero();
    for (uint32_t e = e0; e < e1; e++) {
        Sh<NC> z = sh_load<NC>(za, zb, col[e]);
        A = sh_add<NC>(A, sh_mul_public<NC>(z, fe_load(va + e)));
        B = sh_add<NC>(B, sh_mul_public<NC>(z, fe_load(vb + e)));
        C = sh_add<NC>(C, sh_mul_public<NC>(z, fe_load(vc + e)));
    }
    sh_store<NC>(oa0, oa1, r, A);
    sh_store<NC>(ob0, ob1, r, B);
    sh_store<NC>(oc0, oc1, r, C);
}
template <int NC>
__global__ void __launch_bounds__(PT) k_sparse_matvec3_items(const uint32_t* __restrict__ row_ptr, const uint32_t* __restrict__ col,
                                                          const fe* __restrict__ va, const fe* __restrict__ vb, const fe* __restrict__ vc,
                                                          const fe* __restrict__ za, const fe* __restrict__ zb, const uint32_t* __restrict__ q,
                                                          const uint32_t* __restrict__ q_items, fe* __restrict__ partial) {
    __shared__ fe sh4[4];
    uint32_t nitems = q[1];
    for (uint32_t it = blockIdx.x; it < nitems; it += gridDim.x) {
        uint32_t r = q_items[2 * it], j = q_items[2 * it + 1];
        uint32_t lo = row_ptr[r] + j * SPMV_CHUNK;
        uint32_t hi = min(lo + SPMV_CHUNK, row_ptr[r + 1]);
        Sh<NC> A, B, C;
        for (int k = 0; k < NC; k++) A.c[k] = B.c[k] = C.c[k] = Fr::zero();
        for (uint32_t e = lo + threadIdx.x; e < hi; e += PT) {
            Sh<NC> z = sh_load<NC>(za, zb, col[e]);
            A = sh_add<NC>(A, sh_mul_public<NC>(z, fe_load(va + e)));
            B = sh_add<NC>(B, sh_mul_public<NC>(z, fe_load(vb + e)));
            C = sh_add<NC>(C, sh_mul_public<NC>(z, fe_load(vc + e)));
        }
        fe* out = partial + (size_t)it * 3 * NC;
        for (int k = 0; k < NC; k++) {
            fe a = fr_block_sum(A.c[k], sh4), b = fr_block_sum(B.c[k], sh4), c = fr_block_sum(C.c[k], sh4);
            if (threadIdx.x == 0) {
                fe_store(out + k, a);
                fe_store(out + NC + k, b);
                fe_store(out + 2 * NC + k, c);
            }
        }
    }
}
template <int NC>
__global__ void __launch_bounds__(PT) k_sparse_matvec3_rows(const uint32_t* __restrict__ q, const uint32_t* __restrict__ q_rows,
                                                         const fe* __restrict__ partial, fe* oa0, fe* oa1, fe* ob0, fe* ob1, fe* oc0, fe* oc1) {
    __shared__ fe sh4[4];
    uint32_t nlong = q[0];
    for (uint32_t ri = blockIdx.x; ri < nlong; ri += gridDim.x) {
        uint32_t r = q_rows[3 * ri], first = q_rows[3 * ri + 1], n = q_rows[3 * ri + 2];
        fe acc[3 * NC];
        for (int k = 0; k < 3 * NC; k++) acc[k] = Fr::zero();
        for (uint32_t j = threadIdx.x; j < n; j += PT)
            for (int k = 0; k < 3 * NC; k++) acc[k] = Fr::add(acc[k], fe_load(partial + (size_t)(first + j) * 3 * NC + k));
        fe tot[3 * NC];
        for (int k = 0; k < 3 * NC; k++) tot[k] = fr_block_sum(acc[k], sh4);
        if (threadIdx.x == 0) {
            Sh<NC> A, B, C;
            for (int k = 0; k < NC; k++) {
                A.c[k] = tot[k];
                B.c[k] = tot[NC + k];
                C.c[k] = tot[2 * NC + k];
            }
            sh_store<NC>(oa0, oa1, r, A);
            sh_store<NC>(ob0, ob1, r, B);
            sh_store<NC>(oc0, oc1, r, C);
        }
    }
}

__global__ void __launch_bounds__(PT) k_fold_pairs(const fe* __restrict__ in, fe* __restrict__ out, size_t n_out, fe r) {
    size_t i = (size_t)blockIdx.x * PT + threadIdx.x;
    if (i >= n_out) return;
    fe_store(out + i, fold_pair(in, i, r));
}
__global__ void __launch_bounds__(PT) k_fold_halves(fe* __restrict__ v, size_t n_out, fe r) {
    size_t i = (size_t)blockIdx.x * PT + threadIdx.x;
    if (i >= n_out) return;
    fe lo = fe_load(v + i), hi = fe_load(v + i + n_out);
    fe_store(v + i, Fr::add(lo, Fr::mul(Fr::sub(hi, lo), r)));
}
__global__ void __launch_bounds__(PT) k_scale_by_first(fe* __restrict__ v, size_t n, const fe* __restrict__ s) {
    size_t i = (size_t)blockIdx.x * PT + threadIdx.x;
    if (i >= n) return;
    fe_store(v + i, Fr::mul(fe_load(v + i), fe_load(s)));
}
__global__ void __launch_bounds__(PT) k_eq_expand(const fe* __restrict__ in, fe* __restrict__ out, size_t n_in, fe rj) {
    size_t i = (size_t)blockIdx.x * PT + threadIdx.x;
    if (i >= n_in) return;
    fe e = fe_load(in + i);
    fe hi = Fr::mul(e, rj);
    fe_store(out + 2 * i, Fr::sub(e, hi));
    fe_store(out + 2 * i + 1, hi);
}

__global__ void k_store_fe(fe* out, fe v) { fe_store(out, v); }
__global__ void k_store_u32s(uint32_t* out, const uint32_t* __restrict__ in0, const uint32_t* __restrict__ in1, int n0, size_t stride0) {
    int i = threadIdx.x;
    if (i < n0) out[i] = in0[(size_t)i * stride0];
    if (i == n0 && in1) out[n0] = *in1;
}
struct EqBuildPoint {
    fe r[13];
};
__global__ void __launch_bounds__(1024) k_eq_build(EqBuildPoint pt, int nv, fe* __restrict__ out) {
    if (threadIdx.x == 0) fe_store(out, Fr::one());
    __syncthreads();
    size_t n = 1;
    for (int j = 0; j < nv; j++) {
        fe rj = pt.r[j];
        fe e[8];
        int cnt = 0;
        for (size_t i = threadIdx.x; i < n; i += 1024) e[cnt++] = fe_load(out + i);
        __syncthreads();
        cnt = 0;
        for (size_t i = threadIdx.x; i < n; i += 1024) {
            fe hi = Fr::mul(e[cnt], rj);
            fe_store(out + 2 * i, Fr::sub(e[cnt], hi));
            fe_store(out + 2 * i + 1, hi);
            cnt++;
        }
        __syncthreads();
        n *= 2;
    }
}

static fe* dev_alloc_fe(size_t n) { return (fe*)ctx_dev_alloc(t_cur_ctx, (n ? n : 1) * sizeof(fe)); }

static bool sync_rounds() {
    static const bool on = getenv("COZK_SYNC_ROUNDS") != nullptr;
    return on;
}
static bool trace_rounds() {
    static const bool on = getenv("COZK_TRACE_ROUNDS") != nullptr;
    return on;
}

static void stream_drain_by_flag(cozk_ctx* ctx) {
    if (sync_rounds()) {
        HIP_TRY(hipStreamSynchronize(ctx->stream));
        return;
    }
    if (!ctx->round_flag) HIP_TRY(hipHostMalloc((void**)&ctx->round_flag, 64, hipHostMallocMapped | hipHostMallocCoherent));
    uint32_t seq = ++ctx->round_seq;
    HIP_TRY(hipStreamWriteValue32(ctx->stream, (void*)ctx->round_flag, seq, 0));
    volatile uint32_t* f = ctx->round_flag;
    uint64_t spins = 0;
    while (*f != seq) {
        __builtin_ia32_pause();
        if (++spins > (1ull << 22)) {
            HIP_TRY(hipStreamSynchronize(ctx->stream));
            break;
        }
    }
}
static RoundPublish arm_round_publish(cozk_ctx* ctx) {
    static const bool on = !(getenv("COZK_FLAG_IN_FINISH") && atoi(getenv("COZK_FLAG_IN_FINISH")) == 0);
    if (!on || sync_rounds()) return RoundPublish{nullptr, nullptr, 0};
    if (!ctx->round_flag) HIP_TRY(hipHostMalloc((void**)&ctx->round_flag, 64, hipHostMallocMapped | hipHostMallocCoherent));
    if (!ctx->finish_ticket) {
        HIP_TRY(hipMalloc((void**)&ctx->finish_ticket, 64));
        HIP_TRY(hipMemsetAsync(ctx->finish_ticket, 0, 64, ctx->stream));
    }
    ctx->armed_seq = ++ctx->round_seq;
    return RoundPublish{ctx->finish_ticket, ctx->round_flag, ctx->armed_seq};
}
static void fetch_fe(cozk_ctx* ctx, const fe* d, size_t k, fe* h) {
    fe* pin = (fe*)ctx_pinned(ctx, k * sizeof(fe));
    const uint32_t armed = ctx->armed_seq;
    ctx->armed_seq = 0;
    if (d == pin && armed) {
        volatile uint32_t* f = ctx->round_flag;
        uint64_t spins = 0;
        while (*f != armed) {
            __builtin_ia32_pause();
            if (++spins > (1ull << 22)) {
                HIP_TRY(hipStreamSynchronize(ctx->stream));
                break;
            }
        }
        std::atomic_thread_fence(std::memory_order_acquire);
    } else {
        if (d != pin) HIP_TRY(hipMemcpyAsync(pin, d, k * sizeof(fe), hipMemcpyDeviceToHost, ctx->stream));
        stream_drain_by_flag(ctx);
    }
    for (size_t i = 0; i < k; i++) h[i] = pin[i];
}
static fe* result_slot(cozk_ctx* ctx, size_t k) { return (fe*)ctx_pinned(ctx, k * sizeof(fe)); }

struct SumLaunch {
    fe* partial;
    fe* res;
    char* meta;
    size_t cap;
    size_t n_res;
};
static SumLaunch sum_launch(cozk_ctx* ctx, unsigned rows, unsigned gx_max, size_t n_res, size_t meta_bytes = 0) {
    const size_t meta = (meta_bytes + 31) & ~(size_t)31, cap = (size_t)rows * gx_max;
    ctx->scratch.reserve(meta + (cap + rows) * sizeof(fe));
    char* base = (char*)ctx->scratch.p;
    return SumLaunch{(fe*)(base + meta), result_slot(ctx, n_res), base, cap, n_res};
}
static void finish_sums(cozk_ctx* ctx, const SumLaunch& sl, unsigned rows, unsigned gx, fe scale, int apply_scale, fe* out) {
    COZK_REQUIRE((size_t)rows * gx <= sl.cap && rows <= sl.n_res, "finish_sums: more block partials than sum_launch reserved");
    struct Disarm {
        cozk_ctx* ctx;
        ~Disarm() { ctx->armed_seq = 0; }
    } disarm{ctx};
    k_finish_sums<<<rows, PT, 0, ctx->stream>>>(sl.partial, gx, scale, apply_scale, sl.res, arm_round_publish(ctx));
    HIP_TRY(hipGetLastError());
    fetch_fe(ctx, sl.res, sl.n_res, out);
}


static void drain_streams(const std::vector<cozk_ctx*>& owners, const cozk_ctx* skip = nullptr) {
    for (size_t i = 0; i < owners.size(); i++) {
        cozk_ctx* c = owners[i];
        if (c == skip || std::find(owners.begin(), owners.end(), c) != owners.begin() + (long)i) continue;
        HIP_TRY(hipStreamSynchronize(c->stream));
    }
}

struct MemberNouns {
    const char *one, *on_device, *dup;
};
static constexpr MemberNouns MEMBER{"member", "member", "member"};
template <bool PLAIN, class T>
static void group_member_check(const std::string& what, const MemberNouns& w, const cozk_ctx* driver, T* const* members, int i) {
    const T* m = members[i];
    COZK_REQUIRE(m && m->ctx, what + ": null " + w.one);
    if constexpr (PLAIN) COZK_REQUIRE(m->mode == COZK_MODE_PLAIN, what + ": every " + w.one + " must be PLAIN");
    COZK_REQUIRE(m->ctx->device == driver->device, what + ": every " + w.on_device + " must live on the driver's device");
    for (int j = 0; j < i; j++) COZK_REQUIRE(members[j] != m, what + ": duplicate " + w.dup);
}

struct GroupPub {
    fe* buf[2] = {nullptr, nullptr};
    int cur = 0;
    size_t len = 0;
    void create(cozk_ctx* driver, const cozk_poly* pub) {
        len = pub->len;
        buf[0] = (fe*)ctx_dev_alloc(driver, len * sizeof(fe));
        buf[1] = (fe*)ctx_dev_alloc(driver, (len / 2) * sizeof(fe));
        HIP_TRY(hipMemcpyAsync(buf[0], poly_a(pub), len * sizeof(fe), hipMemcpyDeviceToDevice, driver->stream));
        HIP_TRY(hipStreamSynchronize(driver->stream));
    }
    void free(cozk_ctx* driver) {
        for (int i = 0; i < 2; i++) ctx_dev_free(driver, buf[i]);
    }
    const fe* in() const { return buf[cur]; }
    fe* out() const { return buf[1 - cur]; }
    void advance(size_t new_len) {
        cur = 1 - cur;
        len = new_len;
    }
    void download(cozk_ctx* ctx, uint64_t* out) const {
        std::vector<fe> h(len);
        HIP_TRY(hipMemcpyAsync(h.data(), buf[cur], len * sizeof(fe), hipMemcpyDeviceToHost, ctx->stream));
        HIP_TRY(hipStreamSynchronize(ctx->stream));
        for (size_t i = 0; i < len; i++) fe_to_u64x4(h[i], out + 4 * i);
    }
};

static constexpr unsigned GROUP_GRID_MAX = 2048;
struct GroupSums {
    cozk_ctx* ctx;
    unsigned rows, gx;
    bool small;
    SumLaunch sl;
    fe* partial;
    void fetch(fe* out) const {
        if (small) fetch_fe(ctx, partial, rows, out);
        else finish_sums(ctx, sl, rows, gx, Fr::one(), 0, out);
    }
};
static GroupSums group_sums(cozk_ctx* ctx, unsigned rows, size_t items, bool small, unsigned grid_cap) {
    GroupSums s{ctx, rows, 1u, small, SumLaunch{}, nullptr};
    if (small) s.partial = result_slot(ctx, rows);
    else {
        s.gx = sum_grid(grid_capped(items, grid_cap));
        s.sl = sum_launch(ctx, rows, s.gx, rows);
        s.partial = s.sl.partial;
    }
    return s;
}

static void fetch_u64x4(cozk_ctx* ctx, const fe* res, size_t n, uint64_t* out) {
    fe h[4 * COZK_LAYER_GROUP_MAX];
    COZK_REQUIRE(n <= sizeof h / sizeof h[0], "fetch_u64x4: more values than a group's final call returns");
    fetch_fe(ctx, res, n, h);
    for (size_t i = 0; i < n; i++) fe_to_u64x4(h[i], out + 4 * i);
}

template <class P>
static void pingpong_ensure(P* p, int which, size_t n) {
    if (p->cap[which] >= n) return;
    for (int c = 0; c < 2; c++) {
        if (p->buf[which][c]) ctx_dev_free(p->ctx, p->buf[which][c]);
        p->buf[which][c] = nullptr;
    }
    const size_t bytes = (n ? n : 1) * sizeof(fe);
    p->buf[which][0] = (fe*)ctx_dev_alloc(p->ctx, bytes);
    if (p->mode == COZK_MODE_REP3) p->buf[which][1] = (fe*)ctx_dev_alloc(p->ctx, bytes);
    p->cap[which] = n;
}

struct LayerStep {
    const fe *ia, *ib;
    fe *oa, *ob;
    size_t len_in, len_out;
};
static LayerStep layer_advance(cozk_layer* l) {
    const int dst = 1 - l->cur;
    const size_t len_out = 2 * ((l->len + 3) / 4);
    pingpong_ensure(l, dst, len_out);
    const LayerStep s{l->buf[l->cur][0], l->buf[l->cur][1], l->buf[dst][0], l->buf[dst][1], l->len, len_out};
    l->cur = dst;
    l->len = len_out;
    return s;
}

static void cubic_coeffs_out(const fe s[3], const uint64_t prev_claim[4], uint64_t out_coeffs[16]) {
    fe ev[4] = {s[0], Fr::sub(fe_from_u64x4(prev_claim), s[0]), s[1], s[2]};
    fe cf[4];
    unipoly_from_evals(ev, 4, cf);
    for (int i = 0; i < 4; i++) fe_to_u64x4(cf[i], out_coeffs + 4 * i);
}

static void eq_evals_device(cozk_ctx* ctx, const fe* r, int nv, fe* out, fe* tmp) {
    if (nv <= 13) {
        (void)tmp;
        EqBuildPoint pt;
        for (int j = 0; j < nv; j++) pt.r[j] = r[j];
        for (int j = nv; j < 13; j++) pt.r[j] = Fr::zero();
        k_eq_build<<<1, 1024, 0, ctx->stream>>>(pt, nv, out);
        HIP_TRY(hipGetLastError());
        return;
    }
    fe* cur = (nv % 2 == 0) ? out : tmp;
    fe* nxt = (nv % 2 == 0) ? tmp : out;
    k_store_fe<<<1, 1, 0, ctx->stream>>>(cur, Fr::one());
    size_t n = 1;
    for (int j = 0; j < nv; j++) {
        k_eq_expand<<<grid_for(n), PT, 0, ctx->stream>>>(cur, nxt, n, r[j]);
        std::swap(cur, nxt);
        n *= 2;
    }
    HIP_TRY(hipGetLastError());
}

extern "C" {

int cozk_poly_create(cozk_ctx* ctx, int mode, const cozk_vec* a, const cozk_vec* b, cozk_poly** out) {
    return cozk_guard(ctx, [&] {
        COZK_REQUIRE(ctx && out && a && a->kind == COZK_SCALAR_FR && (mode == COZK_MODE_PLAIN || mode == COZK_MODE_REP3),
                     "poly_create: bad argument");
        COZK_REQUIRE(mode == COZK_MODE_PLAIN || (b && b->kind == COZK_SCALAR_FR && b->n == a->n), "poly_create: share b missing");
        cozk_poly* p = new cozk_poly();
        p->ctx = ctx;
        p->mode = mode;
        p->len = p->orig_len = a->n;
        p->cur = -1;
        p->own0 = true;
        p->a0 = dev_alloc_fe(a->n);
        p->b0 = nullptr;
        HIP_TRY(hipMemcpyAsync(p->a0, a->d, a->n * sizeof(fe), hipMemcpyDeviceToDevice, ctx->stream));
        if (mode == COZK_MODE_REP3) {
            p->b0 = dev_alloc_fe(a->n);
            HIP_TRY(hipMemcpyAsync(p->b0, b->d, a->n * sizeof(fe), hipMemcpyDeviceToDevice, ctx->stream));
        }
        *out = p;
    });
}

int cozk_poly_chunk(cozk_ctx* ctx, const cozk_poly* src, size_t offset, size_t len, cozk_poly** out) {
    return cozk_guard(ctx, [&] {
        COZK_REQUIRE(ctx && src && out && src->cur < 0 && offset + len <= src->orig_len, "poly_chunk: bad argument (source must be unbound)");
        cozk_poly* p = new cozk_poly();
        p->ctx = ctx;
        p->mode = src->mode;
        p->len = p->orig_len = len;
        p->cur = -1;
        p->own0 = false;
        p->a0 = src->a0 + offset;
        p->b0 = src->b0 ? src->b0 + offset : nullptr;
        *out = p;
    });
}

int cozk_poly_free(cozk_poly* p) {
    if (!p) return COZK_OK;
    if (p->own0) {
        if (p->a0) ctx_dev_free(p->ctx, p->a0);
        if (p->b0) ctx_dev_free(p->ctx, p->b0);
    }
    for (int w = 0; w < 2; w++)
        for (int c = 0; c < 2; c++)
            if (p->buf[w][c]) ctx_dev_free(p->ctx, p->buf[w][c]);
    delete p;
    return COZK_OK;
}

size_t cozk_poly_len(const cozk_poly* p) { return p ? p->len : 0; }
int cozk_poly_mode(const cozk_poly* p) { return p ? p->mode : 0; }

int cozk_poly_download(cozk_ctx* ctx, const cozk_poly* p, uint64_t* a, uint64_t* b) {
    return cozk_guard(ctx, [&] {
        COZK_REQUIRE(ctx && p && a, "poly_download: bad argument");
        HIP_TRY(hipMemcpyAsync(a, poly_a(p), p->len * sizeof(fe), hipMemcpyDeviceToHost, ctx->stream));
        if (p->mode == COZK_MODE_REP3 && b)
            HIP_TRY(hipMemcpyAsync(b, poly_b(p), p->len * sizeof(fe), hipMemcpyDeviceToHost, ctx->stream));
        HIP_TRY(hipStreamSynchronize(ctx->stream));
    });
}

int cozk_poly_share_view(cozk_ctx* ctx, const cozk_poly* p, int component, cozk_vec** out) {
    return cozk_guard(ctx, [&] {
        COZK_REQUIRE(ctx && p && out && (component == 0 || (component == 1 && p->mode == COZK_MODE_REP3)), "poly_share_view: bad argument");
        const fe* d = component == 0 ? poly_a(p) : poly_b(p);
        *out = new cozk_vec{ctx, p->len, COZK_SCALAR_FR, (void*)d, p->len * sizeof(fe), false};
    });
}

int cozk_poly_bind(cozk_ctx* ctx, cozk_poly* p, const uint64_t r[4], int order) {
    return cozk_guard(ctx, [&] {
        COZK_REQUIRE(ctx && p && r && p->len >= 2 && (order == COZK_LOW_TO_HIGH || order == COZK_HIGH_TO_LOW), "poly_bind: bad argument");
        size_t n = p->len / 2;
        fe rr = fe_from_u64x4(r);
        const fe* ia = poly_a(p);
        const fe* ib = poly_b(p);
        int dst;
        if (p->cur >= 0 && order == COZK_HIGH_TO_LOW) {
            dst = p->cur;
        } else {
            dst = p->cur < 0 ? 0 : 1 - p->cur;
            pingpong_ensure(p, dst, n);
        }
        fe* oa = p->buf[dst][0];
        fe* ob = p->buf[dst][1];
        if (p->mode == COZK_MODE_REP3) {
            if (order == COZK_LOW_TO_HIGH) k_poly_bind<2, COZK_LOW_TO_HIGH><<<grid_for(n), PT, 0, ctx->stream>>>(ia, ib, oa, ob, n, rr);
            else k_poly_bind<2, COZK_HIGH_TO_LOW><<<grid_for(n), PT, 0, ctx->stream>>>(ia, ib, oa, ob, n, rr);
        } else {
            if (order == COZK_LOW_TO_HIGH) k_poly_bind<1, COZK_LOW_TO_HIGH><<<grid_for(n), PT, 0, ctx->stream>>>(ia, ib, oa, ob, n, rr);
            else k_poly_bind<1, COZK_HIGH_TO_LOW><<<grid_for(n), PT, 0, ctx->stream>>>(ia, ib, oa, ob, n, rr);
        }
        HIP_TRY(hipGetLastError());
        p->cur = dst;
        p->len = n;
    });
}

int cozk_poly_get_coeff(cozk_ctx* ctx, const cozk_poly* p, size_t index, uint64_t a[4], uint64_t b[4]) {
    return cozk_guard(ctx, [&] {
        COZK_REQUIRE(ctx && p && a && index < p->len, "poly_get_coeff: bad argument");
        fe h[2];
        fetch_fe(ctx, poly_a(p) + index, 1, &h[0]);
        fe_to_u64x4(h[0], a);
        if (p->mode == COZK_MODE_REP3 && b) {
            fetch_fe(ctx, poly_b(p) + index, 1, &h[1]);
            fe_to_u64x4(h[1], b);
        }
    });
}

int cozk_eq_evals(cozk_ctx* ctx, const uint64_t* r, int nv, cozk_vec** out) {
    return cozk_guard(ctx, [&] {
        COZK_REQUIRE(ctx && out && nv >= 0 && nv < 40 && (r || nv == 0), "eq_evals: bad argument");
        size_t n = (size_t)1 << nv;
        std::vector<fe> rr(nv);
        for (int j = 0; j < nv; j++) rr[j] = fe_from_u64x4(r + 4 * j);
        fe* d = dev_alloc_fe(n);
        ctx->scratch2.reserve(n * sizeof(fe));
        eq_evals_device(ctx, rr.data(), nv, d, ctx->scratch2.as<fe>());
        *out = new cozk_vec{ctx, n, COZK_SCALAR_FR, d, n * sizeof(fe), true};
    });
}

int cozk_poly_batch_evaluate_at_chi(cozk_ctx* ctx, const cozk_poly* const* polys, size_t k, const cozk_vec* chi,
                                    uint64_t* out) {
    return cozk_guard(ctx, [&] {
        COZK_REQUIRE(ctx && polys && k > 0 && chi && out && chi->kind == COZK_SCALAR_FR, "batch_evaluate: bad argument");
        int mode = polys[0]->mode;
        size_t maxlen = 0;
        std::vector<const fe*> ha(k), hb(k);
        std::vector<size_t> hl(k);
        for (size_t i = 0; i < k; i++) {
            COZK_REQUIRE(polys[i] && polys[i]->mode == mode, "batch_evaluate: mixed share modes");
            COZK_REQUIRE(polys[i]->len <= chi->n, "batch_evaluate: chi shorter than polynomial");
            ha[i] = poly_a(polys[i]);
            hb[i] = poly_b(polys[i]);
            hl[i] = polys[i]->len;
            if (hl[i] > maxlen) maxlen = hl[i];
        }
        const unsigned gx = grid_capped(maxlen, eval_grid_max());
        const SumLaunch sl = sum_launch(ctx, (unsigned)k, gx, k, k * (2 * sizeof(void*) + sizeof(size_t)));
        const fe** da = (const fe**)sl.meta;
        const fe** db = da + k;
        size_t* dl = (size_t*)(db + k);
        HIP_TRY(hipMemcpyAsync(da, ha.data(), k * sizeof(void*), hipMemcpyHostToDevice, ctx->stream));
        HIP_TRY(hipMemcpyAsync(db, hb.data(), k * sizeof(void*), hipMemcpyHostToDevice, ctx->stream));
        HIP_TRY(hipMemcpyAsync(dl, hl.data(), k * sizeof(size_t), hipMemcpyHostToDevice, ctx->stream));
        HIP_TRY(hipStreamSynchronize(ctx->stream));
        dim3 grid(gx, (unsigned)((k + 1) / 2));
        {
            uint64_t alg = (uint64_t)chi->n * 32;
            for (size_t i = 0; i < k; i++) alg += (uint64_t)hl[i] * (mode == COZK_MODE_REP3 ? 64 : 32);
            ProfScope prof(ctx, COZK_PROF_EVAL_CHI, alg);
            if (mode == COZK_MODE_REP3) k_poly_eval_chi<2><<<grid, PT, 0, ctx->stream>>>(da, db, dl, (const fe*)chi->d, (int)k, sl.partial);
            else k_poly_eval_chi<1><<<grid, PT, 0, ctx->stream>>>(da, db, dl, (const fe*)chi->d, (int)k, sl.partial);
        }
        std::vector<fe> h(k);
        finish_sums(ctx, sl, (unsigned)k, gx, fr_two_inv(), mode == COZK_MODE_REP3 ? 1 : 0, h.data());
        for (size_t i = 0; i < k; i++) fe_to_u64x4(h[i], out + 4 * i);
    });
}

int cozk_poly_dot_product_with_public(cozk_ctx* ctx, const cozk_poly* p, const cozk_vec* pub, uint64_t a[4], uint64_t b[4]) {
    return cozk_guard(ctx, [&] {
        COZK_REQUIRE(ctx && p && pub && a && pub->kind == COZK_SCALAR_FR && pub->n == p->len, "dot_product: length mismatch (zip_eq)");
        const unsigned gx = grid_capped(p->len, BATCH_GRID_MAX);
        const int nc = p->mode == COZK_MODE_REP3 ? 2 : 1;
        const SumLaunch sl = sum_launch(ctx, nc, gx, nc);
        if (nc == 2) k_poly_dot_public<2><<<gx, PT, 0, ctx->stream>>>(poly_a(p), poly_b(p), (const fe*)pub->d, p->len, sl.partial);
        else k_poly_dot_public<1><<<gx, PT, 0, ctx->stream>>>(poly_a(p), poly_b(p), (const fe*)pub->d, p->len, sl.partial);
        fe h[2];
        finish_sums(ctx, sl, nc, gx, Fr::one(), 0, h);
        fe_to_u64x4(h[0], a);
        if (nc == 2 && b) fe_to_u64x4(h[1], b);
    });
}

int cozk_poly_linear_combination(cozk_ctx* ctx, const cozk_poly* const* polys, const uint64_t* coeffs, size_t k,
                                 int out_mode, int party_id, cozk_poly** out) {
    return cozk_guard(ctx, [&] {
        COZK_REQUIRE(ctx && polys && coeffs && k > 0 && out && (out_mode == COZK_MODE_PLAIN || out_mode == COZK_MODE_REP3) &&
                         party_id >= 0 && party_id < 3,
                     "linear_combination: bad argument");
        size_t maxlen = 0;
        std::vector<const fe*> ha(k), hb(k);
        std::vector<size_t> hl(k);
        std::vector<fe> hc(k);
        for (size_t i = 0; i < k; i++) {
            const cozk_poly* p = polys[i];
            COZK_REQUIRE(p, "linear_combination: null polynomial");
            hl[i] = p->len;
            hc[i] = fe_from_u64x4(coeffs + 4 * i);
            if (p->len > maxlen) maxlen = p->len;
            if (p->mode == COZK_MODE_REP3) {
                COZK_REQUIRE(out_mode == COZK_MODE_REP3, "linear_combination: shared input needs a shared output");
                ha[i] = poly_a(p);
                hb[i] = poly_b(p);
            } else if (out_mode == COZK_MODE_REP3) {
                ha[i] = party_id == 0 ? poly_a(p) : nullptr;
                hb[i] = party_id == 1 ? poly_a(p) : nullptr;
            } else {
                ha[i] = poly_a(p);
                hb[i] = nullptr;
            }
        }
        cozk_poly* o = new cozk_poly();
        o->ctx = ctx;
        o->mode = out_mode;
        o->len = o->orig_len = maxlen;
        o->cur = -1;
        o->own0 = true;
        o->a0 = dev_alloc_fe(maxlen);
        o->b0 = out_mode == COZK_MODE_REP3 ? dev_alloc_fe(maxlen) : nullptr;
        size_t meta = k * (2 * sizeof(void*) + sizeof(size_t)) + 64 + k * sizeof(fe);
        ctx->scratch.reserve(meta + 64);
        char* base = (char*)ctx->scratch.p;
        const fe** da = (const fe**)base;
        const fe** db = da + k;
        size_t* dl = (size_t*)(db + k);
        fe* dc = (fe*)(((uintptr_t)(dl + k) + 31) & ~(uintptr_t)31);
        HIP_TRY(hipMemcpyAsync(da, ha.data(), k * sizeof(void*), hipMemcpyHostToDevice, ctx->stream));
        HIP_TRY(hipMemcpyAsync(db, hb.data(), k * sizeof(void*), hipMemcpyHostToDevice, ctx->stream));
        HIP_TRY(hipMemcpyAsync(dl, hl.data(), k * sizeof(size_t), hipMemcpyHostToDevice, ctx->stream));
        HIP_TRY(hipMemcpyAsync(dc, hc.data(), k * sizeof(fe), hipMemcpyHostToDevice, ctx->stream));
        HIP_TRY(hipStreamSynchronize(ctx->stream));
        {
            uint64_t alg = (uint64_t)maxlen * (out_mode == COZK_MODE_REP3 ? 64 : 32);
            for (size_t i = 0; i < k; i++) alg += (uint64_t)hl[i] * ((ha[i] ? 32 : 0) + (out_mode == COZK_MODE_REP3 && hb[i] ? 32 : 0));
            ProfScope prof(ctx, COZK_PROF_LINCOMB, alg);
            if (out_mode == COZK_MODE_REP3) k_poly_lincomb<2><<<grid_for(maxlen), PT, 0, ctx->stream>>>(da, db, dl, dc, (int)k, o->a0, o->b0, maxlen);
            else k_poly_lincomb<1><<<grid_for(maxlen), PT, 0, ctx->stream>>>(da, db, dl, dc, (int)k, o->a0, o->b0, maxlen);
        }
        HIP_TRY(hipGetLastError());
        *out = o;
    });
}

int cozk_fingerprint_leaves(cozk_ctx* ctx, const cozk_vec* const* cols, const uint64_t* col_coeffs, size_t ks, const cozk_poly* const* polys,
                            const uint64_t* poly_coeffs, size_t kp, const uint64_t constant[4], int mode, int party_id, cozk_vec* out_a,
                            cozk_vec* out_b, size_t offset, size_t n) {
    return cozk_guard(ctx, [&] {
        COZK_REQUIRE(ctx && constant && out_a && out_a->kind == COZK_SCALAR_FR && (mode == COZK_MODE_PLAIN || mode == COZK_MODE_REP3) &&
                         party_id >= 0 && party_id < 3 && n > 0 && offset + n <= out_a->n && (ks == 0 || (cols && col_coeffs)) &&
                         (kp == 0 || (polys && poly_coeffs)) && ks <= 32 && kp <= 32,
                     "fingerprint_leaves: bad argument");
        COZK_REQUIRE(mode == COZK_MODE_PLAIN || (out_b && out_b->kind == COZK_SCALAR_FR && out_b->n == out_a->n), "fingerprint_leaves: share b output missing");
        std::vector<SmallCol> hcols(ks);
        std::vector<fe> hcs(ks), hds(kp);
        std::vector<const fe*> ha(kp), hb(kp);
        for (size_t k = 0; k < ks; k++) {
            const cozk_vec* v = cols[k];
            COZK_REQUIRE(v && v->n >= n && (v->kind == COZK_SCALAR_U8 || v->kind == COZK_SCALAR_U16 || v->kind == COZK_SCALAR_U32 || v->kind == COZK_SCALAR_U64),
                         "fingerprint_leaves: compact columns are U8 / U16 / U32 / U64 vectors of >= n entries");
            hcols[k] = SmallCol{v->d, v->kind};
            hcs[k] = Fr::to_mont(fe_from_u64x4(col_coeffs + 4 * k));
        }
        for (size_t j = 0; j < kp; j++) {
            const cozk_poly* p = polys[j];
            COZK_REQUIRE(p && p->len >= n, "fingerprint_leaves: polynomial shorter than n");
            hds[j] = fe_from_u64x4(poly_coeffs + 4 * j);
            if (p->mode == COZK_MODE_REP3) {
                COZK_REQUIRE(mode == COZK_MODE_REP3, "fingerprint_leaves: shared input needs a shared output");
                ha[j] = poly_a(p);
                hb[j] = poly_b(p);
            } else if (mode == COZK_MODE_REP3) {
                ha[j] = party_id == 0 ? poly_a(p) : nullptr;
                hb[j] = party_id == 1 ? poly_a(p) : nullptr;
            } else {
                ha[j] = poly_a(p);
                hb[j] = nullptr;
            }
        }
        fe cst0 = fe_from_u64x4(constant);
        if (ks <= 16 && kp <= 8) {
            FingerprintArgs fa;
            memset(&fa, 0, sizeof fa);
            for (size_t k = 0; k < ks; k++) {
                fa.cols[k] = hcols[k];
                fa.cs[k] = hcs[k];
            }
            for (size_t j = 0; j < kp; j++) {
                fa.pa[j] = ha[j];
                fa.pb[j] = hb[j];
                fa.ds[j] = hds[j];
            }
            fe* oa0 = (fe*)out_a->d + offset;
            if (mode == COZK_MODE_REP3)
                k_fingerprint_leaves_args<2><<<grid_for(n), PT, 0, ctx->stream>>>(fa, (int)ks, (int)kp, cst0, party_id == 0, party_id == 1, oa0,
                                                                                 (fe*)out_b->d + offset, n);
            else
                k_fingerprint_leaves_args<1><<<grid_for(n), PT, 0, ctx->stream>>>(fa, (int)ks, (int)kp, cst0, 1, 0, oa0, nullptr, n);
            HIP_TRY(hipGetLastError());
            return;
        }
        size_t meta = ks * sizeof(SmallCol) + 64 + (ks + kp) * sizeof(fe) + 64 + 2 * kp * sizeof(void*) + 64;
        ctx->scratch.reserve(meta);
        char* base = (char*)ctx->scratch.p;
        SmallCol* dcols = (SmallCol*)base;
        fe* dcs = (fe*)(((uintptr_t)(dcols + ks) + 31) & ~(uintptr_t)31);
        fe* dds = dcs + ks;
        const fe** da = (const fe**)(((uintptr_t)(dds + kp) + 15) & ~(uintptr_t)15);
        const fe** db = da + kp;
        if (ks) {
            HIP_TRY(hipMemcpyAsync(dcols, hcols.data(), ks * sizeof(SmallCol), hipMemcpyHostToDevice, ctx->stream));
            HIP_TRY(hipMemcpyAsync(dcs, hcs.data(), ks * sizeof(fe), hipMemcpyHostToDevice, ctx->stream));
        }
        if (kp) {
            HIP_TRY(hipMemcpyAsync(dds, hds.data(), kp * sizeof(fe), hipMemcpyHostToDevice, ctx->stream));
            HIP_TRY(hipMemcpyAsync(da, ha.data(), kp * sizeof(void*), hipMemcpyHostToDevice, ctx->stream));
            HIP_TRY(hipMemcpyAsync(db, hb.data(), kp * sizeof(void*), hipMemcpyHostToDevice, ctx->stream));
        }
        HIP_TRY(hipStreamSynchronize(ctx->stream));
        fe cst = fe_from_u64x4(constant);
        fe* oa = (fe*)out_a->d + offset;
        if (mode == COZK_MODE_REP3)
            k_fingerprint_leaves<2><<<grid_for(n), PT, 0, ctx->stream>>>(dcols, dcs, (int)ks, da, db, dds, (int)kp, cst, party_id == 0, party_id == 1, oa,
                                                                        (fe*)out_b->d + offset, n);
        else
            k_fingerprint_leaves<1><<<grid_for(n), PT, 0, ctx->stream>>>(dcols, dcs, (int)ks, da, db, dds, (int)kp, cst, 1, 0, oa, nullptr, n);
        HIP_TRY(hipGetLastError());
    });
}

int cozk_open_quadratic_evals(cozk_ctx* ctx, const cozk_poly* const* polys, const cozk_poly* const* eqs, size_t k,
                              uint64_t* out) {
    return cozk_guard(ctx, [&] {
        COZK_REQUIRE(ctx && polys && eqs && k > 0 && out, "open_quadratic: bad argument");
        COZK_REQUIRE(polys[0], "open_quadratic: null polynomial");
        int mode = polys[0]->mode;
        std::vector<const fe*> ha(k), hb(k), he(k);
        std::vector<size_t> hh(k);
        size_t maxh = 0;
        for (size_t i = 0; i < k; i++) {
            COZK_REQUIRE(polys[i] && eqs[i] && polys[i]->mode == mode && eqs[i]->mode == COZK_MODE_PLAIN &&
                             eqs[i]->len == polys[i]->len && polys[i]->len >= 2,
                         "open_quadratic: polynomial / eq mismatch");
            ha[i] = poly_a(polys[i]);
            hb[i] = poly_b(polys[i]);
            he[i] = poly_a(eqs[i]);
            hh[i] = polys[i]->len / 2;
            if (hh[i] > maxh) maxh = hh[i];
        }
        const unsigned gx = grid_capped(maxh, BATCH_GRID_MAX);
        const SumLaunch sl = sum_launch(ctx, (unsigned)(2 * k), gx, 2 * k, k * (3 * sizeof(void*) + sizeof(size_t)));
        fe* partial = sl.partial;
        const fe** da = (const fe**)sl.meta;
        const fe** db = da + k;
        const fe** de = db + k;
        size_t* dh = (size_t*)(de + k);
        dim3 grid(gx, (unsigned)k);
        if (k <= 16) {
            OpenQuadArgs args;
            for (size_t i = 0; i < 16; i++) {
                args.a[i] = i < k ? ha[i] : nullptr;
                args.b[i] = i < k ? hb[i] : nullptr;
                args.eq[i] = i < k ? he[i] : nullptr;
                args.half[i] = i < k ? hh[i] : 0;
            }
            if (mode == COZK_MODE_REP3) k_open_quadratic_args<2><<<grid, PT, 0, ctx->stream>>>(args, partial);
            else k_open_quadratic_args<1><<<grid, PT, 0, ctx->stream>>>(args, partial);
        } else {
            HIP_TRY(hipMemcpyAsync(da, ha.data(), k * sizeof(void*), hipMemcpyHostToDevice, ctx->stream));
            HIP_TRY(hipMemcpyAsync(db, hb.data(), k * sizeof(void*), hipMemcpyHostToDevice, ctx->stream));
            HIP_TRY(hipMemcpyAsync(de, he.data(), k * sizeof(void*), hipMemcpyHostToDevice, ctx->stream));
            HIP_TRY(hipMemcpyAsync(dh, hh.data(), k * sizeof(size_t), hipMemcpyHostToDevice, ctx->stream));
            HIP_TRY(hipStreamSynchronize(ctx->stream));
            if (mode == COZK_MODE_REP3) k_open_quadratic<2><<<grid, PT, 0, ctx->stream>>>(da, db, de, dh, partial);
            else k_open_quadratic<1><<<grid, PT, 0, ctx->stream>>>(da, db, de, dh, partial);
        }
        std::vector<fe> h(2 * k);
        finish_sums(ctx, sl, (unsigned)(2 * k), gx, fr_two_inv(), mode == COZK_MODE_REP3 ? 1 : 0, h.data());
        for (size_t i = 0; i < 2 * k; i++) fe_to_u64x4(h[i], out + 4 * i);
    });
}

int cozk_prod_sumcheck_evals(cozk_ctx* ctx, const cozk_poly* const* polys, size_t m, int degree, uint64_t* out) {
    return cozk_guard(ctx, [&] {
        COZK_REQUIRE(ctx && polys && out && m >= 1 && m <= 4 && degree >= 1 && degree <= 4, "prod_sumcheck: bad argument");
        COZK_REQUIRE(polys[0], "prod_sumcheck: null polynomial");
        size_t len = polys[0]->len;
        int shared = -1;
        const fe* ha[4] = {nullptr, nullptr, nullptr, nullptr};
        const fe* hb[4] = {nullptr, nullptr, nullptr, nullptr};
        for (size_t j = 0; j < m; j++) {
            COZK_REQUIRE(polys[j] && polys[j]->len == len && len >= 2, "prod_sumcheck: length mismatch");
            ha[j] = poly_a(polys[j]);
            hb[j] = poly_b(polys[j]);
            if (polys[j]->mode == COZK_MODE_REP3) {
                COZK_REQUIRE(shared < 0, "prod_sumcheck: at most one shared factor (a shared x shared product needs a reshare)");
                shared = (int)j;
            }
        }
        size_t half = len / 2;
        const unsigned gx = grid_capped(half, BATCH_GRID_MAX);
        const SumLaunch sl = sum_launch(ctx, 4, gx, (size_t)degree);
        ProdRoundPtrs tab;
        for (int j = 0; j < 4; j++) {
            tab.a[j] = ha[j];
            tab.b[j] = hb[j];
        }
        using ProdRoundKernel = void (*)(ProdRoundPtrs, int, size_t, int, fe*);
        static const ProdRoundKernel kernels[2][4] = {{k_prod_round<1, 1>, k_prod_round<1, 2>, k_prod_round<1, 3>, k_prod_round<1, 4>},
                                                      {k_prod_round<2, 1>, k_prod_round<2, 2>, k_prod_round<2, 3>, k_prod_round<2, 4>}};
        kernels[shared >= 0][m - 1]<<<gx, PT, 0, ctx->stream>>>(tab, shared, half, degree, sl.partial);
        fe h[4];
        finish_sums(ctx, sl, (unsigned)degree, gx, fr_two_inv(), shared >= 0 ? 1 : 0, h);
        for (int e = 0; e < degree; e++) fe_to_u64x4(h[e], out + 4 * e);
    });
}

int cozk_spartan_first_round(cozk_ctx* ctx, const cozk_poly* za, const cozk_poly* zb, const cozk_poly* zc, const cozk_poly* pub,
                             uint64_t out[16]) {
    return cozk_guard(ctx, [&] {
        COZK_REQUIRE(ctx && za && zb && zc && pub && out && pub->mode == COZK_MODE_PLAIN && za->mode == zb->mode && za->mode == zc->mode &&
                         za->len == zb->len && za->len == zc->len && za->len == pub->len && za->len >= 2,
                     "spartan_first_round: bad argument");
        size_t half = za->len / 2;
        const unsigned gx = grid_capped(half, BATCH_GRID_MAX);
        const SumLaunch sl = sum_launch(ctx, 8, gx, 8);
        fe* partial = sl.partial;
        if (za->mode == COZK_MODE_REP3)
// ... 115 lines not shown
            const_cast<cozk_vec*>(a)->owned = false;
            if (mode == COZK_MODE_REP3) {
                l->buf[0][1] = (fe*)b->d;
                const_cast<cozk_vec*>(b)->owned = false;
            }
        } else {
            l->buf[0][0] = dev_alloc_fe(a->n);
            HIP_TRY(hipMemcpyAsync(l->buf[0][0], a->d, a->n * sizeof(fe), hipMemcpyDeviceToDevice, ctx->stream));
            if (mode == COZK_MODE_REP3) {
                l->buf[0][1] = dev_alloc_fe(a->n);
                HIP_TRY(hipMemcpyAsync(l->buf[0][1], b->d, a->n * sizeof(fe), hipMemcpyDeviceToDevice, ctx->stream));
            }
        }
        *out = l;
    });
}

int cozk_layer_free(cozk_layer* l) {
    if (!l) return COZK_OK;
    for (int w = 0; w < 2; w++)
        for (int c = 0; c < 2; c++)
            if (l->buf[w][c]) ctx_dev_free(l->ctx, l->buf[w][c]);
    delete l;
    return COZK_OK;
}

size_t cozk_layer_len(const cozk_layer* l) { return l ? l->len : 0; }

int cozk_layer_download(cozk_ctx* ctx, const cozk_layer* l, uint64_t* a, uint64_t* b) {
    return cozk_guard(ctx, [&] {
        COZK_REQUIRE(ctx && l && a, "layer_download: bad argument");
        HIP_TRY(hipMemcpyAsync(a, l->buf[l->cur][0], l->len * sizeof(fe), hipMemcpyDeviceToHost, ctx->stream));
        if (l->mode == COZK_MODE_REP3 && b)
            HIP_TRY(hipMemcpyAsync(b, l->buf[l->cur][1], l->len * sizeof(fe), hipMemcpyDeviceToHost, ctx->stream));
        HIP_TRY(hipStreamSynchronize(ctx->stream));
    });
}

int cozk_layer_clone(cozk_ctx* ctx, const cozk_layer* src, cozk_layer** out) {
    return cozk_guard(ctx, [&] {
        COZK_REQUIRE(ctx && src && out, "layer_clone: bad argument");
        cozk_layer* l = new cozk_layer();
        l->ctx = ctx;
        l->mode = src->mode;
        l->len = src->len;
        l->cur = 0;
        l->cap[0] = src->len;
        for (int c = 0; c < (src->mode == COZK_MODE_REP3 ? 2 : 1); c++) {
            l->buf[0][c] = dev_alloc_fe(src->len);
            HIP_TRY(hipMemcpyAsync(l->buf[0][c], src->buf[src->cur][c], src->len * sizeof(fe), hipMemcpyDeviceToDevice, ctx->stream));
        }
        *out = l;
    });
}

int cozk_layer_as_poly(cozk_ctx* ctx, const cozk_layer* l, cozk_poly** out) {
    return cozk_guard(ctx, [&] {
        COZK_REQUIRE(ctx && l && out, "layer_as_poly: bad argument");
        cozk_poly* p = new cozk_poly();
        p->ctx = ctx;
        p->mode = l->mode;
        p->len = p->orig_len = l->len;
        p->cur = -1;
        p->own0 = false;
        p->a0 = l->buf[l->cur][0];
        p->b0 = l->buf[l->cur][1];
        *out = p;
    });
}

int cozk_layer_bind(cozk_ctx* ctx, cozk_layer* l, const uint64_t r[4]) {
    return cozk_guard(ctx, [&] {
        COZK_REQUIRE(ctx && l && r && l->len >= 2, "layer_bind: bad argument");
        const LayerStep b = layer_advance(l);
        auto* const kernel = l->mode == COZK_MODE_REP3 ? k_layer_bind<2> : k_layer_bind<1>;
        kernel<<<grid_for(b.len_out / 2), PT, 0, ctx->stream>>>(b.ia, b.ib, b.oa, b.ob, b.len_in, fe_from_u64x4(r));
        HIP_TRY(hipGetLastError());
    });
}

int cozk_spliteq_new(cozk_ctx* ctx, const uint64_t* w, int nv, cozk_spliteq** out) {
    return cozk_guard(ctx, [&] {
        COZK_REQUIRE(ctx && out && nv >= 0 && nv < 60 && (w || nv == 0), "spliteq_new: bad argument");
        int m = nv / 2;
        cozk_spliteq* e = new cozk_spliteq();
        e->ctx = ctx;
        e->num_vars = nv;
        e->E2_len = e->E2_cap = (size_t)1 << m;
        e->E1_len = e->E1_cap = (size_t)1 << (nv - m);
        for (int k = 0; k < 2; k++) {
            e->E1[k] = dev_alloc_fe(e->E1_cap);
            e->E2[k] = dev_alloc_fe(e->E2_cap);
        }
        std::vector<fe> rr(nv);
        for (int j = 0; j < nv; j++) rr[j] = fe_from_u64x4(w + 4 * j);
        eq_evals_device(ctx, rr.data(), m, e->E2[0], e->E2[1]);
        eq_evals_device(ctx, rr.data() + m, nv - m, e->E1[0], e->E1[1]);
        e->c1 = e->c2 = 0;
        *out = e;
    });
}

int cozk_spliteq_free(cozk_spliteq* e) {
    if (!e) return COZK_OK;
    for (int k = 0; k < 2; k++) {
        if (e->E1[k]) ctx_dev_free(e->ctx, e->E1[k]);
        if (e->E2[k]) ctx_dev_free(e->ctx, e->E2[k]);
    }
    delete e;
    return COZK_OK;
}

int cozk_spliteq_lens(const cozk_spliteq* e, size_t* e1_len, size_t* e2_len) {
    if (!e) return COZK_ERR_INVALID_ARG;
    if (e1_len) *e1_len = e->E1_len;
    if (e2_len) *e2_len = e->E2_len;
    return COZK_OK;
}

int cozk_spliteq_download(cozk_ctx* ctx, const cozk_spliteq* e, uint64_t* e1, uint64_t* e2) {
    return cozk_guard(ctx, [&] {
        COZK_REQUIRE(ctx && e, "spliteq_download: bad argument");
        COZK_REQUIRE(e->ctx == ctx, "spliteq_download: the eq polynomial belongs to another context");
        if (e1) HIP_TRY(hipMemcpyAsync(e1, e->E1[e->c1], e->E1_len * sizeof(fe), hipMemcpyDeviceToHost, ctx->stream));
        if (e2) HIP_TRY(hipMemcpyAsync(e2, e->E2[e->c2], e->E2_len * sizeof(fe), hipMemcpyDeviceToHost, ctx->stream));
        HIP_TRY(hipStreamSynchronize(ctx->stream));
    });
}

static bool spliteq_bound(const cozk_spliteq* e) { return e->E1_len == 1 && e->E2_len < 2; }
struct SpliteqStep {
    const fe* fold_in;
    fe* fold_out;
    size_t fold_n;
    fe* scale_vec;
    size_t scale_n;
};
static SpliteqStep spliteq_advance(cozk_spliteq* e) {
    SpliteqStep s{};
    if (e->E1_len == 1) {
        s.fold_in = e->E2[e->c2];
        s.fold_out = e->E2[1 - e->c2];
        s.fold_n = e->E2_len / 2;
        e->c2 = 1 - e->c2;
        e->E2_len = s.fold_n;
    } else {
        s.fold_in = e->E1[e->c1];
        s.fold_out = e->E1[1 - e->c1];
        s.fold_n = e->E1_len / 2;
        e->c1 = 1 - e->c1;
        e->E1_len = s.fold_n;
        if (s.fold_n == 1) {
            s.scale_vec = e->E2[e->c2];
            s.scale_n = e->E2_len;
        }
    }
    return s;
}
static void spliteq_bind_launch(cozk_ctx* ctx, cozk_spliteq* e, const fe& rr) {
    const SpliteqStep s = spliteq_advance(e);
    k_fold_pairs<<<grid_for(s.fold_n), PT, 0, ctx->stream>>>(s.fold_in, s.fold_out, s.fold_n, rr);
    if (s.scale_n) k_scale_by_first<<<grid_for(s.scale_n), PT, 0, ctx->stream>>>(s.scale_vec, s.scale_n, s.fold_out);
    HIP_TRY(hipGetLastError());
}
int cozk_spliteq_bind(cozk_ctx* ctx, cozk_spliteq* e, const uint64_t r[4]) {
    return cozk_guard(ctx, [&] {
        COZK_REQUIRE(ctx && e && r, "spliteq_bind: bad argument");
        COZK_REQUIRE(!spliteq_bound(e), "spliteq_bind: polynomial already fully bound");
        spliteq_bind_launch(ctx, e, fe_from_u64x4(r));
    });
}

struct LayerVariant {
    bool f9;
    int nested;
};
static LayerVariant layer_variant(const cozk_layer* l, const cozk_spliteq* e, size_t chunks) {
    static const bool f9_env = (getenv("COZK_LAYER_F9") ? atoi(getenv("COZK_LAYER_F9")) : 1) != 0;
    static const bool group_env = !(getenv("COZK_LAYER_GROUPED") && atoi(getenv("COZK_LAYER_GROUPED")) == 0);
    const bool f9 = f9_env && chunks >= LAYER_F9_MIN_CHUNKS, nested = e->E1_len != 1;
    const bool grouped = f9 && nested && group_env && l->mode == COZK_MODE_PLAIN && e->E1_len / 2 >= LAYER_GROUPED_MIN_E1H;
    return LayerVariant{f9, grouped ? 2 : (nested ? 1 : 0)};
}
using LayerCubicKernel = void (*)(const fe*, const fe*, size_t, const fe*, size_t, const fe*, size_t, fe*);
static LayerCubicKernel layer_cubic_kernel(int mode, LayerVariant v) {
    if (mode == COZK_MODE_REP3) {
        if (v.f9) return v.nested ? k_layer_cubic9<2, 1> : k_layer_cubic9<2, 0>;
        return v.nested ? k_layer_cubic<2, 1> : k_layer_cubic<2, 0>;
    }
    if (v.f9) return v.nested == 2 ? k_layer_cubic9<1, 2> : (v.nested ? k_layer_cubic9<1, 1> : k_layer_cubic9<1, 0>);
    return v.nested ? k_layer_cubic<1, 1> : k_layer_cubic<1, 0>;
}
using LayerBindCubicKernel = void (*)(const fe*, const fe*, fe*, fe*, size_t, fe, const fe*, size_t, const fe*, size_t, fe*);
static LayerBindCubicKernel layer_bind_cubic_kernel(int mode, LayerVariant v) {
    if (mode == COZK_MODE_REP3) {
        if (v.f9) return v.nested ? k_layer_bind_cubic9<2, 1> : k_layer_bind_cubic9<2, 0>;
        return v.nested ? k_layer_bind_cubic<2, 1> : k_layer_bind_cubic<2, 0>;
    }
    if (v.f9) return v.nested == 2 ? k_layer_bind_cubic9<1, 2> : (v.nested ? k_layer_bind_cubic9<1, 1> : k_layer_bind_cubic9<1, 0>);
    return v.nested ? k_layer_bind_cubic<1, 1> : k_layer_bind_cubic<1, 0>;
}
static unsigned layer_sum_grid(cozk_ctx* ctx, const void* kernel, bool f9, size_t chunks) {
    return sum_grid(f9 ? resident_grid(kernel, (chunks + PT - 1) / PT, ctx->device) : grid_capped(chunks, ROUND_GRID_MAX));
}

struct LayerCubicPlan {
    LayerVariant v;
    LayerCubicKernel kernel;
    unsigned gx;
};
static LayerCubicPlan layer_cubic_plan(cozk_ctx* ctx, const cozk_layer* l, const cozk_spliteq* eq) {
    const size_t nch = (l->len + 3) / 4;
    const LayerVariant v = layer_variant(l, eq, nch);
    const LayerCubicKernel kernel = layer_cubic_kernel(l->mode, v);
    return LayerCubicPlan{v, kernel, layer_sum_grid(ctx, (const void*)kernel, v.f9, nch)};
}
static void layer_cubic_launch(cozk_ctx* ctx, const cozk_layer* l, const cozk_spliteq* eq, const LayerCubicPlan& p, fe* partial) {
    p.kernel<<<p.gx, PT, 0, ctx->stream>>>(l->buf[l->cur][0], l->buf[l->cur][1], l->len, eq->E1[eq->c1], p.v.nested ? eq->E1_len / 2 : 0, eq->E2[eq->c2],
                                           eq->E2_len, partial);
}
static void layer_cubic_sums(cozk_ctx* ctx, const cozk_layer* l, const cozk_spliteq* eq, fe s[3]) {
    const LayerCubicPlan p = layer_cubic_plan(ctx, l, eq);
    const SumLaunch sl = sum_launch(ctx, 3, p.gx, 3);
    layer_cubic_launch(ctx, l, eq, p, sl.partial);
    finish_sums(ctx, sl, 3, p.gx, Fr::one(), 0, s);
}

struct LayerBindCubicPlan {
    LayerVariant v;
    LayerBindCubicKernel kernel;
    unsigned gx;
};
static LayerBindCubicPlan layer_bind_cubic_plan(cozk_ctx* ctx, const cozk_layer* l, const cozk_spliteq* e) {
    const size_t nout = 2 * ((l->len + 3) / 4), nch_out = (nout + 3) / 4;
    const LayerVariant v = layer_variant(l, e, nch_out);
    const LayerBindCubicKernel kernel = layer_bind_cubic_kernel(l->mode, v);
    return LayerBindCubicPlan{v, kernel, layer_sum_grid(ctx, (const void*)kernel, v.f9, nch_out)};
}
static void layer_bind_cubic_launch(cozk_ctx* ctx, cozk_layer* l, const cozk_spliteq* e, const LayerBindCubicPlan& p, const uint64_t r[4], fe* partial) {
    const LayerStep b = layer_advance(l);
    fe rr = fe_from_u64x4(r);
    if (p.v.f9)
        for (int d = 0; d < 5; d++) rr = Fr::dbl(rr);
    const bool rep3 = l->mode == COZK_MODE_REP3;
    {
        const uint64_t S = rep3 ? 64 : 32;
        ProfScope prof(ctx, COZK_PROF_BIND_CUBIC, (uint64_t)b.len_in * S + (uint64_t)b.len_out * S + (uint64_t)(e->E1_len + e->E2_len) * 32);
        p.kernel<<<p.gx, PT, 0, ctx->stream>>>(b.ia, b.ib, b.oa, b.ob, b.len_in, rr, e->E1[e->c1], p.v.nested ? e->E1_len / 2 : 0, e->E2[e->c2], e->E2_len,
                                               partial);
    }
}

int cozk_layer_compute_cubic(cozk_ctx* ctx, const cozk_layer* l, const cozk_spliteq* eq, const uint64_t prev_claim[4],
                             uint64_t out_coeffs[16]) {
    return cozk_guard(ctx, [&] {
        COZK_REQUIRE(ctx && l && eq && prev_claim && out_coeffs, "compute_cubic: bad argument");
        fe s[3];
        layer_cubic_sums(ctx, l, eq, s);
        cubic_coeffs_out(s, prev_claim, out_coeffs);
    });
}

int cozk_layer_round(cozk_ctx* ctx, cozk_layer* l, cozk_spliteq* e, const uint64_t* r, const uint64_t prev_claim[4],
                     uint64_t out_coeffs[16]) {
    if (!ctx || !l || !e || !prev_claim || !out_coeffs) return COZK_ERR_INVALID_ARG;
    if (l->len > ROUND_SMALL_MAX) {
        if (!r) return cozk_layer_compute_cubic(ctx, l, e, prev_claim, out_coeffs);
        int rc = cozk_spliteq_bind(ctx, e, r);
        if (rc != COZK_OK) return rc;
        return cozk_guard(ctx, [&] {
            const LayerBindCubicPlan p = layer_bind_cubic_plan(ctx, l, e);
            const SumLaunch sl = sum_launch(ctx, 3, p.gx, 3);
            layer_bind_cubic_launch(ctx, l, e, p, r, sl.partial);
            fe sres[3];
            finish_sums(ctx, sl, 3, p.gx, Fr::one(), 0, sres);
            cubic_coeffs_out(sres, prev_claim, out_coeffs);
        });
    }
    return cozk_guard(ctx, [&] {
        if (r) {
            COZK_REQUIRE(l->len >= 2, "layer_round: layer already fully bound");
            COZK_REQUIRE(!spliteq_bound(e), "layer_round: eq polynomial already fully bound");
        }
        LayerStep b{};
        SpliteqStep f{};
        fe rr = Fr::zero();
        if (r) {
            rr = fe_from_u64x4(r);
            b = layer_advance(l);
            f = spliteq_advance(e);
        }
        fe* res = result_slot(ctx, 3);
        auto* const kernel = l->mode == COZK_MODE_REP3 ? k_layer_round_small<2> : k_layer_round_small<1>;
        kernel<<<1, RT, 0, ctx->stream>>>(b.ia, b.ib, b.oa, b.ob, b.len_in, r != nullptr, rr, f.fold_in, f.fold_out, f.fold_n, f.scale_vec, f.scale_n,
                                          l->buf[l->cur][0], l->buf[l->cur][1], l->len, e->E1[e->c1], e->E1_len / 2, e->E2[e->c2], e->E2_len, e->E1_len != 1,
                                          res);
        HIP_TRY(hipGetLastError());
        fe sres[3];
        fetch_fe(ctx, res, 3, sres);
        cubic_coeffs_out(sres, prev_claim, out_coeffs);
    });
}

int cozk_layer_prove_rounds(cozk_ctx* ctx, cozk_layer* l, cozk_spliteq* e, const uint64_t claim[4], int num_rounds, cozk_round_cb cb,
                            void* user, uint64_t* out_r, uint64_t final_claims[16]) {
    if (!ctx || !l || !e || !claim || !cb || !final_claims || num_rounds < 0 || (num_rounds > 0 && !out_r)) return COZK_ERR_INVALID_ARG;
    static const bool no_persist = getenv("COZK_NO_PERSIST") != nullptr;
    uint64_t pc[4], rr[4], coeffs[16], nc[4];
    memcpy(pc, claim, sizeof pc);
    bool have_r = false;
    int round = 0;
    bool allow_resident = !no_persist && ctx_resident_rounds_enabled(ctx);
    for (;;) {
        for (; round < num_rounds; round++) {
            if (allow_resident && l->len <= ROUND_PERSIST_MAX && l->len >= 2) break;
            int rc = cozk_layer_round(ctx, l, e, have_r ? rr : nullptr, pc, coeffs);
            if (rc != COZK_OK) return rc;
            if (cb(user, round, coeffs, rr, nc) != 0) {
                ctx->last_error = "layer_prove_rounds: round callback failed";
                return COZK_ERR_INTERNAL;
            }
            memcpy(out_r + 4 * round, rr, sizeof rr);
            memcpy(pc, nc, sizeof pc);
            have_r = true;
        }
        if (round == num_rounds) {
            if (have_r) {
                int rc = cozk_layer_bind(ctx, l, rr);
                if (rc != COZK_OK) return rc;
                rc = cozk_spliteq_bind(ctx, e, rr);
                if (rc != COZK_OK) return rc;
            }
            return cozk_layer_final_claims(ctx, l, final_claims);
        }
        int rounds_done = -1;
        int rc = cozk_guard(ctx, [&] {
            const int nrem = num_rounds - round;
            pingpong_ensure(l, 1 - l->cur, l->len);
            if (!ctx->mailbox) HIP_TRY(hipHostMalloc(&ctx->mailbox, sizeof(RoundMailbox), hipHostMallocMapped | hipHostMallocCoherent));
            RoundMailbox* mb = (RoundMailbox*)ctx->mailbox;
            memset(mb, 0, sizeof *mb);
            std::atomic_thread_fence(std::memory_order_seq_cst);
            fe r_first = have_r ? fe_from_u64x4(rr) : Fr::zero();
            const long long ticks = (long long)resident_timeout_s() * MB_TICKS_PER_S;
            const bool rep3 = l->mode == COZK_MODE_REP3;
            auto* const kernel = rep3 ? (trace_rounds() ? k_layer_rounds_persistent<2, 1> : k_layer_rounds_persistent<2, 0>)
                                      : (trace_rounds() ? k_layer_rounds_persistent<1, 1> : k_layer_rounds_persistent<1, 0>);
            kernel<<<1, RT, 0, ctx->stream>>>(l->buf[0][0], l->buf[0][1], l->buf[1][0], l->buf[1][1], l->cur, l->len, e->E1[0], e->E1[1], e->c1, e->E1_len,
                                              e->E2[0], e->E2[1], e->c2, e->E2_len, nrem, have_r ? 1 : 0, r_first, mb, ticks);
            HIP_TRY(hipGetLastError());
            volatile uint32_t* res_seq = &mb->res_seq;
            volatile uint32_t* status = &mb->status;
            auto give_up = [&](const char* why) {
                *(volatile uint32_t*)&mb->cmd[12] = 1;
                std::atomic_thread_fence(std::memory_order_seq_cst);
                (void)hipStreamSynchronize(ctx->stream);
                throw CozkError(COZK_ERR_INTERNAL, why);
            };
            auto wait_result = [&](uint32_t want) -> bool {
                auto t0 = std::chrono::steady_clock::now();
                uint64_t spins = 0;
                while (*res_seq != want) {
                    if (*status == 1) return false;
                    if (*status) give_up("layer_prove_rounds: the resident kernel stopped");
                    __builtin_ia32_pause();
                    if ((++spins & 0xfffff) == 0 && std::chrono::steady_clock::now() - t0 > std::chrono::seconds(resident_timeout_s() + 5))
                        give_up("layer_prove_rounds: no result from the resident kernel");
                }
                std::atomic_thread_fence(std::memory_order_acquire);
                return true;
            };
            auto mirror_binds = [&](int binds) {
                for (int b = 0; b < binds; b++) {
                    (void)layer_advance(l);
                    (void)spliteq_advance(e);
                }
            };
            const int bind_first = have_r ? 1 : 0;
            int j = 0;
            bool alive = true;
            for (; j < nrem; j++) {
                if (!(alive = wait_result((uint32_t)j + 1))) break;
                const fe sres[3] = {mb->res[0], mb->res[1], mb->res[2]};
                cubic_coeffs_out(sres, pc, coeffs);
                if (cb(user, round + j, coeffs, rr, nc) != 0) give_up("layer_prove_rounds: round callback failed");
                memcpy(out_r + 4 * (round + j), rr, sizeof rr);
                memcpy(pc, nc, sizeof pc);
                have_r = true;
                {
                    const fe rv = fe_from_u64x4(rr);
                    const uint32_t tag = (uint32_t)j + 1;
                    const uint32_t pay[9] = {rv.l[0], rv.l[1], rv.l[2], rv.l[3], rv.l[4], rv.l[5], rv.l[6], rv.l[7], 0u};
                    for (int k = 0; k < 3; k++) {
                        volatile uint64_t* piece = reinterpret_cast<volatile uint64_t*>(&mb->cmd[4 * k]);
                        piece[0] = (uint64_t)pay[3 * k] | ((uint64_t)pay[3 * k + 1] << 32);
                        std::atomic_thread_fence(std::memory_order_release);
                        piece[1] = (uint64_t)pay[3 * k + 2] | ((uint64_t)tag << 32);
                    }
                }
            }
            if (alive) alive = wait_result((uint32_t)nrem + 1);
            if (!alive) {
                HIP_TRY(hipStreamSynchronize(ctx->stream));
                mirror_binds(j > 0 ? j - 1 + bind_first : 0);
                rounds_done = j;
                return;
            }
            for (int k = 0; k < 4; k++) fe_to_u64x4(mb->res[k], final_claims + 4 * k);
            if (trace_rounds())
                fprintf(stderr, "[mailbox] %d rounds: device us/round: wait %.1f bind %.1f cubic %.1f publish %.1f\n", nrem,
                        mb->dbg[0] / 100.0 / (nrem + 1), mb->dbg[1] / 100.0 / (nrem + 1), mb->dbg[2] / 100.0 / nrem, mb->dbg[3] / 100.0 / nrem);
            mirror_binds(nrem + bind_first);
        });
        if (rc != COZK_OK || rounds_done < 0) return rc;
        round += rounds_done;
        allow_resident = false;
    }
}

namespace {
struct EvalsShim {
    cozk_round_evals_cb cb;
    void* user;
};
int evals_shim_cb(void* user, int round, const uint64_t coeffs[16], uint64_t r_out[4], uint64_t next_claim_out[4]) {
    EvalsShim* sh = static_cast<EvalsShim*>(user);
    std::vector<fe> cf(4);
    for (int i = 0; i < 4; i++) cf[i] = fe_from_u64x4(coeffs + 4 * i);
    uint64_t ev[12];
    fe_to_u64x4(cf[0], ev);
    auto horner = [&](const fe& x) { return Fr::add(cf[0], Fr::mul(x, Fr::add(cf[1], Fr::mul(x, Fr::add(cf[2], Fr::mul(x, cf[3])))))); };
    fe_to_u64x4(horner(Fr::from_u64(2)), ev + 4);
    fe_to_u64x4(horner(Fr::from_u64(3)), ev + 8);
    for (int i = 0; i < 4; i++) next_claim_out[i] = 0;
    return sh->cb(sh->user, round, ev, r_out);
}
}
int cozk_layer_prove_rounds_evals(cozk_ctx* ctx, cozk_layer* l, cozk_spliteq* e, int num_rounds, cozk_round_evals_cb cb, void* user,
                                  uint64_t* out_r, uint64_t final_claims[16]) {
    if (!cb) return COZK_ERR_INVALID_ARG;
    EvalsShim sh{cb, user};
    const uint64_t zero[4] = {0, 0, 0, 0};
    return cozk_layer_prove_rounds(ctx, l, e, zero, num_rounds, evals_shim_cb, &sh, out_r, final_claims);
}

int cozk_layer_compute_cubic_evals(cozk_ctx* ctx, const cozk_layer* l, const cozk_spliteq* eq, uint64_t out_evals[12]) {
    return cozk_guard(ctx, [&] {
        COZK_REQUIRE(ctx && l && eq && out_evals, "compute_cubic_evals: bad argument");
        fe s[3];
        layer_cubic_sums(ctx, l, eq, s);
        for (int i = 0; i < 3; i++) fe_to_u64x4(s[i], out_evals + 4 * i);
    });
}

int cozk_layer_final_claims(cozk_ctx* ctx, const cozk_layer* l, uint64_t out[16]) {
    return cozk_guard(ctx, [&] {
        COZK_REQUIRE(ctx && l && out && l->len == 2, "final_claims: layer must be fully bound (len == 2)");
        fe h[2];
        fetch_fe(ctx, l->buf[l->cur][0], 2, h);
        fe_to_u64x4(h[0], out);
        fe_to_u64x4(h[1], out + 8);
        if (l->mode == COZK_MODE_REP3) {
            fetch_fe(ctx, l->buf[l->cur][1], 2, h);
            fe_to_u64x4(h[0], out + 4);
            fe_to_u64x4(h[1], out + 12);
        } else {
            for (int i = 0; i < 4; i++) out[4 + i] = out[12 + i] = 0;
        }
    });
}

struct cozk_layer_group {
    cozk_ctx* driver;
    int mode;
    std::vector<cozk_layer*> m;
};

static size_t layer_group_len(const cozk_layer_group* g, size_t k, const char* what) {
    for (size_t i = 1; i < k; i++) COZK_REQUIRE(g->m[i]->len == g->m[0]->len, std::string(what) + ": the members must have one length");
    return k ? g->m[0]->len : 0;
}

int cozk_layer_group_create(cozk_ctx* driver, cozk_layer* const* layers, int k, cozk_layer_group** out) {
    if (out) *out = nullptr;
    return cozk_guard(driver, [&] {
        COZK_REQUIRE(driver && layers && out, "layer_group_create: null argument");
        COZK_REQUIRE(k >= 1 && k <= COZK_LAYER_GROUP_MAX, "layer_group_create: 1 <= k <= COZK_LAYER_GROUP_MAX");
        std::vector<cozk_ctx*> owners;
        for (int i = 0; i < k; i++) {
            const cozk_layer* l = layers[i];
            group_member_check<false>("layer_group_create", MEMBER, driver, layers, i);
            COZK_REQUIRE(l->mode == layers[0]->mode, "layer_group_create: the members must have one mode");
            COZK_REQUIRE(l->len == layers[0]->len && l->len >= 2, "layer_group_create: the members must have one length >= 2");
            owners.push_back(l->ctx);
        }
        drain_streams(owners);
        for (int i = 0; i < k; i++) {
            cozk_layer* l = layers[i];
            pingpong_ensure(l, 1 - l->cur, 2 * ((l->len + 3) / 4));
        }
        cozk_layer_group* g = new cozk_layer_group();
        g->driver = driver;
        g->mode = layers[0]->mode;
        g->m.assign(layers, layers + k);
        *out = g;
    });
}

int cozk_layer_group_free(cozk_layer_group* g) {
    delete g;
    return COZK_OK;
}

static LayerGroupArgs layer_group_args(const cozk_layer_group* g, size_t k, bool bind) {
    LayerGroupArgs a;
    memset(&a, 0, sizeof a);
    for (size_t m = 0; m < k; m++) {
        cozk_layer* l = g->m[m];
        if (bind) {
            const LayerStep b = layer_advance(l);
            a.ia[m] = b.ia;
            a.ib[m] = b.ib;
            a.oa[m] = b.oa;
            a.ob[m] = b.ob;
        } else {
            a.ia[m] = l->buf[l->cur][0];
            a.ib[m] = l->buf[l->cur][1];
        }
    }
    return a;
}

int cozk_layer_group_round(cozk_layer_group* g, cozk_spliteq* e, const uint64_t* r, const uint64_t prev_claim[4], uint64_t* out_coeffs) {
    if (!g) return COZK_ERR_INVALID_ARG;
    cozk_ctx* const ctx = g->driver;
    return cozk_guard(ctx, [&] {
        COZK_REQUIRE(e && prev_claim && out_coeffs, "layer_group_round: null argument");
        COZK_REQUIRE(e->ctx == ctx, "layer_group_round: the eq polynomial must be the driver's");
        const unsigned k = (unsigned)g->m.size();
        const size_t len = layer_group_len(g, k, "layer_group_round");
        if (r) {
            COZK_REQUIRE(len > 2, "layer_group_round: the members are already fully bound");
            COZK_REQUIRE(!spliteq_bound(e), "layer_group_round: eq polynomial already fully bound");
        }
        const bool rep3 = g->mode == COZK_MODE_REP3;
        fe s[3 * COZK_LAYER_GROUP_MAX];
        if (len > ROUND_SMALL_MAX) {
            if (!r) {
                const LayerCubicPlan p = layer_cubic_plan(ctx, g->m[0], e);
                const SumLaunch sl = sum_launch(ctx, 3 * k, p.gx, 3 * k);
                for (unsigned m = 0; m < k; m++) layer_cubic_launch(ctx, g->m[m], e, p, sl.partial + (size_t)3 * m * p.gx);
                finish_sums(ctx, sl, 3 * k, p.gx, Fr::one(), 0, s);
            } else {
                spliteq_bind_launch(ctx, e, fe_from_u64x4(r));
                const LayerBindCubicPlan p = layer_bind_cubic_plan(ctx, g->m[0], e);
                const SumLaunch sl = sum_launch(ctx, 3 * k, p.gx, 3 * k);
                for (unsigned m = 0; m < k; m++) layer_bind_cubic_launch(ctx, g->m[m], e, p, r, sl.partial + (size_t)3 * m * p.gx);
                finish_sums(ctx, sl, 3 * k, p.gx, Fr::one(), 0, s);
            }
        } else {
            const LayerGroupArgs a = layer_group_args(g, k, r != nullptr);
            fe rr = Fr::zero();
            if (r) {
                rr = fe_from_u64x4(r);
                spliteq_bind_launch(ctx, e, rr);
            }
            const size_t len_now = g->m[0]->len;
            const int nested = e->E1_len != 1;
            fe* res = result_slot(ctx, (size_t)3 * k);
            auto* const kernel = rep3 ? k_layer_group_round_small<2> : k_layer_group_round_small<1>;
            kernel<<<k, RT, 0, ctx->stream>>>(a, len, r != nullptr, rr, len_now, e->E1[e->c1], e->E1_len / 2, e->E2[e->c2], e->E2_len, nested, res);
            HIP_TRY(hipGetLastError());
            fetch_fe(ctx, res, (size_t)3 * k, s);
        }
        for (unsigned m = 0; m < k; m++) cubic_coeffs_out(s + 3 * m, prev_claim, out_coeffs + 16 * m);
    });
}

int cozk_layer_group_final(cozk_layer_group* g, cozk_spliteq* e, const uint64_t* r, int k_final, uint64_t* out_claims) {
    if (!g) return COZK_ERR_INVALID_ARG;
    cozk_ctx* const ctx = g->driver;
    return cozk_guard(ctx, [&] {
        COZK_REQUIRE(e && out_claims, "layer_group_final: null argument");
        COZK_REQUIRE(e->ctx == ctx, "layer_group_final: the eq polynomial must be the driver's");
        COZK_REQUIRE(k_final >= 0 && k_final <= (int)g->m.size(), "layer_group_final: 0 <= k_final <= k");
        const size_t len = layer_group_len(g, (size_t)k_final, "layer_group_final");
        COZK_REQUIRE(k_final == 0 || (r ? len <= 4 : len == 2), "layer_group_final: the members must be fully bound (len == 2) after the bind");
        if (r) COZK_REQUIRE(!spliteq_bound(e), "layer_group_final: eq polynomial already fully bound");
        const bool rep3 = g->mode == COZK_MODE_REP3;
        const int nc = rep3 ? 2 : 1;
        const LayerGroupArgs a = layer_group_args(g, (size_t)k_final, r != nullptr);
        fe rr = Fr::zero();
        if (r) {
            rr = fe_from_u64x4(r);
            spliteq_bind_launch(ctx, e, rr);
        }
        if (k_final == 0) {
            if (r) stream_drain_by_flag(ctx);
            return;
        }
        const size_t n_res = (size_t)2 * nc * (size_t)k_final;
        fe* res = result_slot(ctx, n_res);
        auto* const kernel = rep3 ? k_layer_group_final<2> : k_layer_group_final<1>;
        kernel<<<k_final, GFT, 0, ctx->stream>>>(a, len, r != nullptr, rr, res);
        HIP_TRY(hipGetLastError());
        fe h[4 * COZK_LAYER_GROUP_MAX];
        fetch_fe(ctx, res, n_res, h);
        for (int m = 0; m < k_final; m++) {
            uint64_t* out = out_claims + 16 * m;
            for (int i = 0; i < 16; i++) out[i] = 0;
            for (int side = 0; side < 2; side++)
                for (int c = 0; c < nc; c++) fe_to_u64x4(h[(2 * m + side) * nc + c], out + 8 * side + 4 * c);
        }
    });
}

int cozk_layer_output_local(cozk_ctx* ctx, const cozk_layer* l, int masked, const uint8_t* key_self_b, const uint8_t* key_prev_b,
                            uint64_t counter, cozk_vec** out) {
    return cozk_guard(ctx, [&] {
        COZK_REQUIRE(ctx && l && out && l->len >= 2 && (!masked || (key_self_b && key_prev_b)), "layer_output_local: bad argument");
        prf_key seed_self{}, seed_prev{};
        if (masked) {
            seed_self = prf_key_from_bytes(key_self_b);
            seed_prev = prf_key_from_bytes(key_prev_b);
        }
        size_t n = (l->len + 1) / 2;
        fe* d = dev_alloc_fe(n);
        const fe* a = l->buf[l->cur][0];
        const fe* b = l->buf[l->cur][1];
        {
            ProfScope prof(ctx, COZK_PROF_LAYER_OUTPUT, (uint64_t)l->len * (l->mode == COZK_MODE_REP3 ? 64 : 32) + (uint64_t)n * 32);
            if (l->mode == COZK_MODE_REP3) k_layer_output<2><<<grid_for(n), PT, 0, ctx->stream>>>(a, b, l->len, d, n, masked, seed_self, seed_prev, counter);
            else k_layer_output<1><<<grid_for(n), PT, 0, ctx->stream>>>(a, b, l->len, d, n, masked, seed_self, seed_prev, counter);
        }
        HIP_TRY(hipGetLastError());
        *out = new cozk_vec{ctx, n, COZK_SCALAR_FR, d, n * sizeof(fe), true};
    });
}

int cozk_rep3_mul_vec_local(cozk_ctx* ctx, int mode, const cozk_vec* xa, const cozk_vec* xb, const cozk_vec* ya,
                            const cozk_vec* yb, int masked, const uint8_t* key_self_b, const uint8_t* key_prev_b, uint64_t counter,
                            cozk_vec** out) {
    return cozk_guard(ctx, [&] {
        COZK_REQUIRE(ctx && xa && ya && out && xa->n == ya->n && (mode == COZK_MODE_PLAIN || (xb && yb && xb->n == xa->n && yb->n == xa->n)) &&
                         (!masked || (key_self_b && key_prev_b)),
                     "mul_vec_local: bad argument");
        COZK_REQUIRE(xa->kind == COZK_SCALAR_FR && ya->kind == COZK_SCALAR_FR &&
                         (mode == COZK_MODE_PLAIN || (xb->kind == COZK_SCALAR_FR && yb->kind == COZK_SCALAR_FR)),
                     "mul_vec_local: the share components must be FR vectors");
        prf_key seed_self{}, seed_prev{};
        if (masked) {
            seed_self = prf_key_from_bytes(key_self_b);
            seed_prev = prf_key_from_bytes(key_prev_b);
        }
        size_t n = xa->n;
        fe* d = dev_alloc_fe(n);
        if (mode == COZK_MODE_REP3)
            k_mul_vec_local<2><<<grid_for(n), PT, 0, ctx->stream>>>((const fe*)xa->d, (const fe*)xb->d, (const fe*)ya->d, (const fe*)yb->d, n, d, masked, seed_self, seed_prev, counter);
        else
            k_mul_vec_local<1><<<grid_for(n), PT, 0, ctx->stream>>>((const fe*)xa->d, nullptr, (const fe*)ya->d, nullptr, n, d, masked, seed_self, seed_prev, counter);
        HIP_TRY(hipGetLastError());
        *out = new cozk_vec{ctx, n, COZK_SCALAR_FR, d, n * sizeof(fe), true};
    });
}

int cozk_layer_claimed_outputs(cozk_ctx* ctx, const cozk_layer* l, uint64_t* out) {
    return cozk_guard(ctx, [&] {
        COZK_REQUIRE(ctx && l && out && l->len >= 2 && l->len % 2 == 0, "claimed_outputs: bad argument");
        size_t n = l->len / 2;
        ctx->scratch.reserve(n * sizeof(fe));
        fe* d = ctx->scratch.as<fe>();
        const fe* a = l->buf[l->cur][0];
        const fe* b = l->buf[l->cur][1];
        if (l->mode == COZK_MODE_REP3) k_layer_output<2><<<grid_for(n), PT, 0, ctx->stream>>>(a, b, l->len, d, n, 0, prf_key{}, prf_key{}, 0);
        else k_layer_output<1><<<grid_for(n), PT, 0, ctx->stream>>>(a, b, l->len, d, n, 0, prf_key{}, prf_key{}, 0);
        HIP_TRY(hipGetLastError());
        std::vector<fe> h(n);
        fetch_fe(ctx, d, n, h.data());
        for (size_t i = 0; i < n; i++) fe_to_u64x4(h[i], out + 4 * i);
    });
}

}

#include "toggle_layer.inc"
#include "spartan_group.inc"
#include "sparse_layer.inc"
#include "primary_sumcheck.inc"
#include "primary_group.inc"
#include "spartan_outer.inc"
#include "outer_group.inc"
#include "spartan_inner.inc"
#include "logup.inc"
#include "compact_open.inc"
#include "output_check.inc"
```

### co-zkvms_amd/csrc/poly.hip.hpp

```cpp
#pragma once
#include "common.hpp"

template <int NC>
struct Sh {
    fe c[NC];
};

static FF_HD fe fr_two_inv() {
    fe r;
    const uint32_t v[8] = {0x1ffffffeu, 0x783c14d8u, 0x0c8d1eddu, 0xaf982f6fu,
                           0xfcfd4f45u, 0x8f5f7492u, 0x3d9cbfacu, 0x1f37631au};
    for (int i = 0; i < 8; i++) r.l[i] = v[i];
    return r;
}

template <int NC>
static __device__ __forceinline__ Sh<NC> sh_load(const fe* a, const fe* b, size_t i) {
    Sh<NC> s;
    s.c[0] = fe_load(a + i);
    if (NC == 2) s.c[NC - 1] = fe_load(b + i);
    return s;
}
template <int NC>
static __device__ __forceinline__ Sh<NC> sh_load_or_zero(const fe* a, const fe* b, size_t i, size_t len) {
    if (i < len) return sh_load<NC>(a, b, i);
    Sh<NC> s;
    for (int k = 0; k < NC; k++) s.c[k] = Fr::zero();
    return s;
}
template <int NC>
static __device__ __forceinline__ void sh_store(fe* a, fe* b, size_t i, const Sh<NC>& s) {
    fe_store(a + i, s.c[0]);
    if (NC == 2) fe_store(b + i, s.c[NC - 1]);
}
template <int NC>
static FF_HD Sh<NC> sh_add(const Sh<NC>& x, const Sh<NC>& y) {
    Sh<NC> r;
    for (int k = 0; k < NC; k++) r.c[k] = Fr::add(x.c[k], y.c[k]);
    return r;
}
template <int NC>
static FF_HD Sh<NC> sh_sub(const Sh<NC>& x, const Sh<NC>& y) {
    Sh<NC> r;
    for (int k = 0; k < NC; k++) r.c[k] = Fr::sub(x.c[k], y.c[k]);
    return r;
}
template <int NC>
static FF_HD Sh<NC> sh_mul_public(const Sh<NC>& x, const fe& p) {
    Sh<NC> r;
    for (int k = 0; k < NC; k++) r.c[k] = Fr::mul(x.c[k], p);
    return r;
}
template <int NC>
static FF_HD Sh<NC> sh_lerp(const Sh<NC>& lo, const Sh<NC>& hi, const fe& r) {
    Sh<NC> o;
    for (int k = 0; k < NC; k++) o.c[k] = Fr::add(lo.c[k], Fr::mul(Fr::sub(hi.c[k], lo.c[k]), r));
    return o;
}
template <int NC>
static FF_HD fe sh_local_mul(const Sh<NC>& x, const Sh<NC>& y) {
    if (NC == 1) return Fr::mul(x.c[0], y.c[0]);
    return Fr::add(Fr::mul(x.c[0], Fr::add(y.c[0], y.c[NC - 1])), Fr::mul(x.c[NC - 1], y.c[0]));
}
template <int NC>
static FF_HD fe sh_ab_sum(const Sh<NC>& x) {
    if (NC == 1) return x.c[0];
    return Fr::add(x.c[0], x.c[NC - 1]);
}

struct FrWide {
    uint64_t lo[15];
    uint32_t hi[15];
};
#if defined(__HIP_DEVICE_COMPILE__)
static __device__ __forceinline__ void fr_wide_zero(FrWide& w) {
#pragma unroll
    for (int k = 0; k < 15; k++) {
        w.lo[k] = 0;
        w.hi[k] = 0;
    }
}
static __device__ __forceinline__ void fr_wide_mac(FrWide& w, const fe& a, const fe& b) {
    const uint32_t* A = a.l;
    const uint32_t* B = b.l;
    MACC1_VV(w.lo[0], w.hi[0], A[0], B[0]);
    MACC2_VV(w.lo[1], w.hi[1], A[0], A[1], B[1], B[0]);
    MACC3_VV(w.lo[2], w.hi[2], A[0], A[1], A[2], B[2], B[1], B[0]);
    MACC4_VV(w.lo[3], w.hi[3], A[0], A[1], A[2], A[3], B[3], B[2], B[1], B[0]);
    MACC5_VV(w.lo[4], w.hi[4], A[0], A[1], A[2], A[3], A[4], B[4], B[3], B[2], B[1], B[0]);
    MACC6_VV(w.lo[5], w.hi[5], A[0], A[1], A[2], A[3], A[4], A[5], B[5], B[4], B[3], B[2], B[1], B[0]);
    MACC7_VV(w.lo[6], w.hi[6], A[0], A[1], A[2], A[3], A[4], A[5], A[6], B[6], B[5], B[4], B[3], B[2], B[1], B[0]);
    MACC8_VV(w.lo[7], w.hi[7], A[0], A[1], A[2], A[3], A[4], A[5], A[6], A[7], B[7], B[6], B[5], B[4], B[3], B[2], B[1], B[0]);
    MACC7_VV(w.lo[8], w.hi[8], A[1], A[2], A[3], A[4], A[5], A[6], A[7], B[7], B[6], B[5], B[4], B[3], B[2], B[1]);
    MACC6_VV(w.lo[9], w.hi[9], A[2], A[3], A[4], A[5], A[6], A[7], B[7], B[6], B[5], B[4], B[3], B[2]);
    MACC5_VV(w.lo[10], w.hi[10], A[3], A[4], A[5], A[6], A[7], B[7], B[6], B[5], B[4], B[3]);
    MACC4_VV(w.lo[11], w.hi[11], A[4], A[5], A[6], A[7], B[7], B[6], B[5], B[4]);
    MACC3_VV(w.lo[12], w.hi[12], A[5], A[6], A[7], B[7], B[6], B[5]);
    MACC2_VV(w.lo[13], w.hi[13], A[6], A[7], B[7], B[6]);
    MACC1_VV(w.lo[14], w.hi[14], A[7], B[7]);
}
static __device__ __forceinline__ fe fr_wide_reduce(const FrWide& w) {
    uint32_t t[18];
    uint64_t carry = 0;
#pragma unroll
    for (int k = 0; k < 15; k++) {
        uint64_t s = w.lo[k] + carry;
        uint32_t h = w.hi[k] + (s < carry ? 1u : 0u);
        t[k] = (uint32_t)s;
        carry = (s >> 32) | ((uint64_t)h << 32);
    }
    t[15] = (uint32_t)carry;
    t[16] = (uint32_t)(carry >> 32);
    t[17] = 0;
    fe t0, t1, t2 = Fr::zero();
#pragma unroll
    for (int i = 0; i < 8; i++) {
        t0.l[i] = t[i];
        t1.l[i] = t[8 + i];
    }
    t2.l[0] = t[16];
    t2.l[1] = t[17];
    fe r = Fr::add(Fr::from_mont(t0), Fr::to_mont(Fr::from_mont(t1)));
    return Fr::add(r, Fr::to_mont(t2));
}
#else
__device__ void fr_wide_zero(FrWide& w);
__device__ void fr_wide_mac(FrWide& w, const fe& a, const fe& b);
__device__ fe fr_wide_reduce(const FrWide& w);
#endif

static __device__ __forceinline__ fe fr_wave_sum(fe v) {
#pragma unroll
    for (int off = 32; off > 0; off >>= 1) {
        fe o;
#pragma unroll
        for (int k = 0; k < 8; k++) o.l[k] = __shfl_down(v.l[k], off);
        v = Fr::add(v, o);
    }
    return v;
}
static __device__ __forceinline__ fe fr_block_sum(fe v, fe* sh4) {
    v = fr_wave_sum(v);
    int lane = threadIdx.x & 63, w = threadIdx.x >> 6;
    __syncthreads();
    if (lane == 0) sh4[w] = v;
    __syncthreads();
    if (threadIdx.x == 0) {
        v = sh4[0];
        for (int i = 1; i < (int)(blockDim.x >> 6); i++) v = Fr::add(v, sh4[i]);
    }
    return v;
}

static inline fe fe_from_u64x4(const uint64_t v[4]) {
    fe r;
    for (int i = 0; i < 4; i++) {
        r.l[2 * i] = (uint32_t)v[i];
        r.l[2 * i + 1] = (uint32_t)(v[i] >> 32);
    }
    return r;
}
static inline void fe_to_u64x4(const fe& a, uint64_t v[4]) {
    for (int i = 0; i < 4; i++) v[i] = (uint64_t)a.l[2 * i] | ((uint64_t)a.l[2 * i + 1] << 32);
}

static inline void unipoly_from_evals(const fe* ev, int n, fe* coeffs) {
    fe inv2 = fr_two_inv();
    if (n == 3) {
        fe c2 = Fr::mul(Fr::add(Fr::sub(ev[2], Fr::dbl(ev[1])), ev[0]), inv2);
        coeffs[0] = ev[0];
        coeffs[2] = c2;
        coeffs[1] = Fr::sub(Fr::sub(ev[1], ev[0]), c2);
        return;
    }
    fe inv6;
    {
        const uint32_t v6[8] = {0x0aaaaaaau, 0x7d695c48u, 0xaed9b4f4u, 0x3a880fcfu,
                                0xa9a9c517u, 0xda7526dbu, 0x69deea8eu, 0x0a67cbb3u};
        for (int i = 0; i < 8; i++) inv6.l[i] = v6[i];
    }
    fe d1 = Fr::sub(ev[1], ev[0]);
    fe d2 = Fr::add(Fr::sub(ev[2], Fr::dbl(ev[1])), ev[0]);
    fe three_e2 = Fr::add(Fr::dbl(ev[2]), ev[2]), three_e1 = Fr::add(Fr::dbl(ev[1]), ev[1]);
    fe d3 = Fr::sub(Fr::add(Fr::sub(ev[3], three_e2), three_e1), ev[0]);
    fe a3 = Fr::mul(d3, inv6);
    fe h2 = Fr::mul(d2, inv2);
    fe three_a3 = Fr::add(Fr::dbl(a3), a3);
    coeffs[0] = ev[0];
    coeffs[1] = Fr::add(Fr::sub(d1, h2), Fr::dbl(a3));
    coeffs[2] = Fr::sub(h2, three_a3);
    coeffs[3] = a3;
}
static inline void cubic_from_round_evals(const fe& claim, const uint64_t ev[12], fe coeffs[4]) {
    const fe g0 = fe_from_u64x4(ev);
    const fe pts[4] = {g0, Fr::sub(claim, g0), fe_from_u64x4(ev + 4), fe_from_u64x4(ev + 8)};
    unipoly_from_evals(pts, 4, coeffs);
}
```

Before: 9.333 million cycles/s.

## Finish small GKR layer sumcheck rounds on host via mailbox tail handoff

Adds a host-side implementation of the layer sumcheck rounds (sums, bind, eq folding) and hands over the remaining small tail of layer data through the pinned mailbox once the shape falls below a cap. The resident persistent kernel now stops early and exports the tail, and the host finishes the remaining rounds without per-round GPU round-trips. Field helpers become host/device callable so they can be shared. This trades GPU launch and mailbox latency on tiny rounds for CPU field arithmetic and a device-to-host copy, and it enlarges the mapped mailbox.

```diff
diff --git a/co-zkvms_amd/build.py b/co-zkvms_amd/build.py
--- a/co-zkvms_amd/build.py
+++ b/co-zkvms_amd/build.py
@@ -7,9 +7,11 @@
 OUT = os.path.join(HERE, "libcozk.so")
 PRIMS_SRC = os.path.join(os.path.dirname(HERE), "tests", "native", "prims.hip")
 PRIMS_OUT = os.path.join(os.path.dirname(HERE), "tests", "native", "libcozk_prims.so")
+TAIL_SRC = os.path.join(os.path.dirname(HERE), "tests", "native", "layer_tail_check.hip")
+TAIL_OUT = os.path.join(os.path.dirname(HERE), "tests", "native", "layer_tail_check")
 HIPCC_FLAGS = ["--offload-arch=gfx950", "-O3", "-std=c++17", "-fPIC"]
 SOURCES = ["capi.hip", "msm.hip", "poly.hip", "harness.hip", "shm_hub.hip", "ring.hip", "shamir.hip", "lasso_witness.hip", "rw_memory_witness.hip", "rw_memory_leaves.hip", "ts_range_witness.hip"]
-HEADERS = [os.path.join("host", "spartan_pub_workers.hpp"), "fr9.hip.hpp", "fr9_consts.inc", os.path.join("host", "flow_harness.hpp"), os.path.join("host", "ts_range_proof.hpp"), os.path.join("host", "rw_memory_proof.hpp"), os.path.join("host", "jolt_r1cs.hpp"), os.path.join("host", "spartan_jolt.hpp"), "spartan_inner.inc", "ff.hip.hpp", "prf.hip.hpp", "ff_macc.inc", "ff_mul2.inc", "ec.hip.hpp", "fq9.hip.hpp", "fq9_consts.inc", "fq9_mac.inc", "fq9_mul.inc", "common.hpp", "lasso_walk.hip.hpp", "radix_pass.hip.hpp", "poly.hip.hpp", "toggle_layer.inc", "spartan_group.inc", "sparse_layer.inc", "primary_sumcheck.inc", "primary_group.inc", "shamir_deal.hip.hpp", "spartan_outer.inc", "outer_group.inc", "logup.inc", "compact_open.inc", "output_check.inc", os.path.join("host", "memory_proof.hpp"), os.path.join("host", "wire.hpp"), os.path.join("host", "net.hpp"), os.path.join("host", "prover.hpp"), os.path.join("host", "sparse_rule.hpp"), os.path.join("host", "split.hpp"), os.path.join("host", "split_harness.hpp"), os.path.join("host", "spartan_harness.hpp"), os.path.join("host", "lookups_harness.hpp"), os.path.join("host", "outer_harness.hpp"), os.path.join("host", "runner.hpp"), os.path.join("host", "shamir_gp.hpp"), os.path.join("host", "shamir_harness.hpp"), os.path.join("host", "shamir_spartan.hpp"), os.path.join("host", "shamir_jolt_spartan.hpp"), os.path.join("host", "shamir_primary.hpp"), os.path.join("..", "..", "include", "cozk.h")]
+HEADERS = [os.path.join("host", "layer_tail.hpp"), os.path.join("host", "spartan_pub_workers.hpp"), "fr9.hip.hpp", "fr9_consts.inc", os.path.join("host", "flow_harness.hpp"), os.path.join("host", "ts_range_proof.hpp"), os.path.join("host", "rw_memory_proof.hpp"), os.path.join("host", "jolt_r1cs.hpp"), os.path.join("host", "spartan_jolt.hpp"), "spartan_inner.inc", "ff.hip.hpp", "prf.hip.hpp", "ff_macc.inc", "ff_mul2.inc", "ec.hip.hpp", "fq9.hip.hpp", "fq9_consts.inc", "fq9_mac.inc", "fq9_mul.inc", "common.hpp", "lasso_walk.hip.hpp", "radix_pass.hip.hpp", "poly.hip.hpp", "toggle_layer.inc", "spartan_group.inc", "sparse_layer.inc", "primary_sumcheck.inc", "primary_group.inc", "shamir_deal.hip.hpp", "spartan_outer.inc", "outer_group.inc", "logup.inc", "compact_open.inc", "output_check.inc", os.path.join("host", "memory_proof.hpp"), os.path.join("host", "wire.hpp"), os.path.join("host", "net.hpp"), os.path.join("host", "prover.hpp"), os.path.join("host", "sparse_rule.hpp"), os.path.join("host", "split.hpp"), os.path.join("host", "split_harness.hpp"), os.path.join("host", "spartan_harness.hpp"), os.path.join("host", "lookups_harness.hpp"), os.path.join("host", "outer_harness.hpp"), os.path.join("host", "runner.hpp"), os.path.join("host", "shamir_gp.hpp"), os.path.join("host", "shamir_harness.hpp"), os.path.join("host", "shamir_spartan.hpp"), os.path.join("host", "shamir_jolt_spartan.hpp"), os.path.join("host", "shamir_primary.hpp"), os.path.join("..", "..", "include", "cozk.h")]
 
 
 def _newer(target, deps):
@@ -42,6 +44,7 @@
             print(" ".join(cmd), flush=True)
         subprocess.check_call(cmd)
     build_prims(force, verbose)
+    build_layer_tail(force, verbose)
     return OUT
 
 
@@ -56,8 +59,21 @@
     return PRIMS_OUT
 
 
+def build_layer_tail(force=False, verbose=True, extra_flags=(), out=TAIL_OUT):
+    if force or _newer(out, [TAIL_SRC] + [os.path.join(CSRC, h) for h in HEADERS]):
+        tmp = out + ".tmp"
+        cmd = ["hipcc"] + HIPCC_FLAGS + list(extra_flags) + [TAIL_SRC, "-o", tmp]
+        if verbose:
+            print(" ".join(cmd), flush=True)
+        subprocess.check_call(cmd)
+        os.replace(tmp, out)
+    return out
+
+
 if __name__ == "__main__":
     if "--prims" in sys.argv:
         build_prims(force="--force" in sys.argv)
+    elif "--layer-tail" in sys.argv:
+        build_layer_tail(force="--force" in sys.argv)
     else:
         build(force="--force" in sys.argv)
diff --git a/co-zkvms_amd/csrc/ff.hip.hpp b/co-zkvms_amd/csrc/ff.hip.hpp
--- a/co-zkvms_amd/csrc/ff.hip.hpp
+++ b/co-zkvms_amd/csrc/ff.hip.hpp
@@ -606,16 +606,24 @@
 typedef Field<FrParams> Fr;
 typedef Field<FqParams> Fq;
 
-static __device__ __forceinline__ fe fe_load(const fe* p) {
+static FF_HD fe fe_load(const fe* p) {
+#if defined(__HIP_DEVICE_COMPILE__)
     const uint4* q = reinterpret_cast<const uint4*>(p);
     uint4 lo = q[0], hi = q[1];
     fe r;
     r.l[0] = lo.x; r.l[1] = lo.y; r.l[2] = lo.z; r.l[3] = lo.w;
     r.l[4] = hi.x; r.l[5] = hi.y; r.l[6] = hi.z; r.l[7] = hi.w;
     return r;
+#else
+    return *p;
+#endif
 }
-static __device__ __forceinline__ void fe_store(fe* p, const fe& v) {
+static FF_HD void fe_store(fe* p, const fe& v) {
+#if defined(__HIP_DEVICE_COMPILE__)
     uint4* q = reinterpret_cast<uint4*>(p);
     q[0] = make_uint4(v.l[0], v.l[1], v.l[2], v.l[3]);
     q[1] = make_uint4(v.l[4], v.l[5], v.l[6], v.l[7]);
+#else
+    *p = v;
+#endif
 }
diff --git a/co-zkvms_amd/csrc/host/layer_tail.hpp b/co-zkvms_amd/csrc/host/layer_tail.hpp
--- /dev/null
+++ b/co-zkvms_amd/csrc/host/layer_tail.hpp
@@ -0,0 +1,160 @@
+#pragma once
+#include "../poly.hip.hpp"
+
+template <int NC>
+static FF_HD void layer_bind_chunk(const fe* ia, const fe* ib, size_t len_in, size_t ci, const fe& r, fe* oa, fe* ob, Sh<NC>& lo, Sh<NC>& hi) {
+    Sh<NC> u0 = sh_load_or_zero<NC>(ia, ib, 4 * ci, len_in), u1 = sh_load_or_zero<NC>(ia, ib, 4 * ci + 1, len_in);
+    Sh<NC> u2 = sh_load_or_zero<NC>(ia, ib, 4 * ci + 2, len_in), u3 = sh_load_or_zero<NC>(ia, ib, 4 * ci + 3, len_in);
+    lo = sh_lerp<NC>(u0, u2, r);
+    sh_store<NC>(oa, ob, 2 * ci, lo);
+    hi = sh_lerp<NC>(u1, u3, r);
+    sh_store<NC>(oa, ob, 2 * ci + 1, hi);
+}
+
+static FF_HD void eq3(const fe& e0, const fe& e1, fe out[3]) {
+    fe m = Fr::sub(e1, e0);
+    out[0] = e0;
+    out[1] = Fr::add(e1, m);
+    out[2] = Fr::add(out[1], m);
+}
+
+static FF_HD size_t layer_chunk_count(size_t len, bool nested, size_t E1_half, size_t E2_len) {
+    size_t nch = (len + 3) / 4;
+    size_t limit = nested ? E1_half * E2_len : E2_len / 2;
+    return nch > limit ? limit : nch;
+}
+
+static FF_HD void split_eq_at(bool nested, const fe* E1, int log_E1_half, const fe* E2, size_t c, fe e[3], fe& scale) {
+    if (nested) {
+        size_t x2 = c >> log_E1_half, x1 = c & (((size_t)1 << log_E1_half) - 1);
+        eq3(fe_load(E1 + 2 * x1), fe_load(E1 + 2 * x1 + 1), e);
+        scale = fe_load(E2 + x2);
+    } else {
+        eq3(fe_load(E2 + 2 * c), fe_load(E2 + 2 * c + 1), e);
+    }
+}
+static FF_HD void layer_eq_at(bool nested, const fe* E1, size_t E1_half, const fe* E2, size_t c, fe e[3], fe& scale) {
+#if defined(__HIP_DEVICE_COMPILE__)
+    split_eq_at(nested, E1, __ffsll((long long)E1_half) - 1, E2, c, e, scale);
+#else
+    split_eq_at(nested, E1, __builtin_ffsll((long long)E1_half) - 1, E2, c, e, scale);
+#endif
+}
+
+template <int NC>
+static FF_HD void layer_terms(const Sh<NC>& l0, const Sh<NC>& r0, const Sh<NC>& l1, const Sh<NC>& r1, const fe e[3], bool nested, const fe& scale, fe& t0,
+                              fe& t2, fe& t3) {
+    Sh<NC> ml = sh_sub<NC>(l1, l0), mr = sh_sub<NC>(r1, r0);
+    Sh<NC> l2 = sh_add<NC>(l1, ml), r2 = sh_add<NC>(r1, mr);
+    Sh<NC> l3 = sh_add<NC>(l2, ml), r3 = sh_add<NC>(r2, mr);
+    t0 = Fr::mul(sh_local_mul<NC>(l0, r0), e[0]);
+    t2 = Fr::mul(sh_local_mul<NC>(l2, r2), e[1]);
+    t3 = Fr::mul(sh_local_mul<NC>(l3, r3), e[2]);
+    if (nested) {
+        t0 = Fr::mul(t0, scale);
+        t2 = Fr::mul(t2, scale);
+        t3 = Fr::mul(t3, scale);
+    }
+}
+
+static FF_HD fe fold_pair(const fe* in, size_t i, const fe& r) {
+    fe lo = fe_load(in + 2 * i), hi = fe_load(in + 2 * i + 1);
+    return Fr::add(lo, Fr::mul(Fr::sub(hi, lo), r));
+}
+
+struct LayerTailView {
+    fe *la, *lb;
+    size_t len;
+    fe* E1;
+    size_t E1_len;
+    fe* E2;
+    size_t E2_len;
+};
+static inline size_t layer_tail_entries(int nc, size_t len, size_t E1_len, size_t E2_len) { return (size_t)nc * len + E1_len + E2_len; }
+static inline LayerTailView layer_tail_view(fe* area, int nc, size_t len, size_t E1_len, size_t E2_len) {
+    fe* eq = area + (size_t)nc * len;
+    return LayerTailView{area, nc == 2 ? area + len : nullptr, len, eq, E1_len, eq + E1_len, E2_len};
+}
+
+struct LayerTailShape {
+    size_t len, E1_len, E2_len;
+};
+static inline LayerTailShape layer_tail_shape_bound(LayerTailShape s) {
+    s.len = 2 * ((s.len + 3) / 4);
+    if (s.E1_len == 1) s.E2_len /= 2;
+    else s.E1_len /= 2;
+    return s;
+}
+
+template <int NC>
+static inline void layer_tail_sums(const LayerTailView& t, fe s[3]) {
+    const bool nested = t.E1_len != 1;
+    const size_t E1_half = t.E1_len / 2;
+    const size_t nch = layer_chunk_count(t.len, nested, E1_half, t.E2_len);
+    s[0] = s[1] = s[2] = Fr::zero();
+    for (size_t c = 0; c < nch; c++) {
+        fe e[3];
+        fe scale = Fr::zero();
+        layer_eq_at(nested, t.E1, E1_half, t.E2, c, e, scale);
+        Sh<NC> l0 = sh_load_or_zero<NC>(t.la, t.lb, 4 * c, t.len), r0 = sh_load_or_zero<NC>(t.la, t.lb, 4 * c + 1, t.len);
+        Sh<NC> l1 = sh_load_or_zero<NC>(t.la, t.lb, 4 * c + 2, t.len), r1 = sh_load_or_zero<NC>(t.la, t.lb, 4 * c + 3, t.len);
+        fe t0, t2, t3;
+        layer_terms<NC>(l0, r0, l1, r1, e, nested, scale, t0, t2, t3);
+        s[0] = Fr::add(s[0], t0);
+        s[1] = Fr::add(s[1], t2);
+        s[2] = Fr::add(s[2], t3);
+    }
+}
+
+template <int NC>
+static inline void layer_tail_bind(LayerTailView& t, const fe& r) {
+    const size_t nch_in = (t.len + 3) / 4;
+    for (size_t c = 0; c < nch_in; c++) {
+        Sh<NC> lo, hi;
+        layer_bind_chunk<NC>(t.la, t.lb, t.len, c, r, t.la, t.lb, lo, hi);
+    }
+    t.len = 2 * nch_in;
+    if (t.E1_len == 1) {
+        const size_t n = t.E2_len / 2;
+        for (size_t i = 0; i < n; i++) fe_store(t.E2 + i, fold_pair(t.E2, i, r));
+        t.E2_len = n;
+    } else {
+        const size_t n = t.E1_len / 2;
+        for (size_t i = 0; i < n; i++) fe_store(t.E1 + i, fold_pair(t.E1, i, r));
+        t.E1_len = n;
+        if (n == 1) {
+            const fe sc = fe_load(t.E1);
+            for (size_t i = 0; i < t.E2_len; i++) fe_store(t.E2 + i, Fr::mul(fe_load(t.E2 + i), sc));
+        }
+    }
+}
+
+template <int NC>
+static inline void layer_tail_final_claims(const LayerTailView& t, fe out[4]) {
+    const fe z = Fr::zero();
+    out[0] = fe_load(t.la);
+    out[1] = NC == 2 ? fe_load(t.lb) : z;
+    out[2] = fe_load(t.la + 1);
+    out[3] = NC == 2 ? fe_load(t.lb + 1) : z;
+}
+
+template <int NC, class Exchange>
+static inline int layer_tail_rounds(LayerTailView& t, bool have_r, fe r, int nrounds, Exchange&& exchange, fe final[4]) {
+    int binds = 0;
+    for (int j = 0; j < nrounds; j++) {
+        if (have_r) {
+            layer_tail_bind<NC>(t, r);
+            binds++;
+        }
+        fe s[3];
+        layer_tail_sums<NC>(t, s);
+        r = exchange(j, s);
+        have_r = true;
+    }
+    if (have_r) {
+        layer_tail_bind<NC>(t, r);
+        binds++;
+    }
+    layer_tail_final_claims<NC>(t, final);
+    return binds;
+}
diff --git a/co-zkvms_amd/csrc/poly.hip b/co-zkvms_amd/csrc/poly.hip
--- a/co-zkvms_amd/csrc/poly.hip
+++ b/co-zkvms_amd/csrc/poly.hip
@@ -7,6 +7,7 @@
 #include "prf.hip.hpp"
 #include "fr9.hip.hpp"
 #include "shamir_deal.hip.hpp"
+#include "host/layer_tail.hpp"
 
 static constexpr int PT = 256;
 static constexpr int MAXBLK = 2048;
@@ -333,42 +334,6 @@
     fe_store(rn + i, Fr::add(lo, Fr::mul(d, p)));
 }
 
-template <int NC>
-static __device__ __forceinline__ void layer_bind_chunk(const fe* ia, const fe* ib, size_t len_in, size_t ci, const fe& r, fe* oa, fe* ob, Sh<NC>& lo,
-                                                        Sh<NC>& hi) {
-    Sh<NC> u0 = sh_load_or_zero<NC>(ia, ib, 4 * ci, len_in), u1 = sh_load_or_zero<NC>(ia, ib, 4 * ci + 1, len_in);
-    Sh<NC> u2 = sh_load_or_zero<NC>(ia, ib, 4 * ci + 2, len_in), u3 = sh_load_or_zero<NC>(ia, ib, 4 * ci + 3, len_in);
-    lo = sh_lerp<NC>(u0, u2, r);
-    sh_store<NC>(oa, ob, 2 * ci, lo);
-    hi = sh_lerp<NC>(u1, u3, r);
-    sh_store<NC>(oa, ob, 2 * ci + 1, hi);
-}
-
-static __device__ __forceinline__ void eq3(const fe& e0, const fe& e1, fe out[3]) {
-    fe m = Fr::sub(e1, e0);
-    out[0] = e0;
-    out[1] = Fr::add(e1, m);
-    out[2] = Fr::add(out[1], m);
-}
-
-static __device__ __forceinline__ size_t layer_chunk_count(size_t len, bool nested, size_t E1_half, size_t E2_len) {
-    size_t nch = (len + 3) / 4;
-    size_t limit = nested ? E1_half * E2_len : E2_len / 2;
-    return nch > limit ? limit : nch;
-}
-
-static __device__ __forceinline__ void split_eq_at(bool nested, const fe* E1, int log_E1_half, const fe* E2, size_t c, fe e[3], fe& scale) {
-    if (nested) {
-        size_t x2 = c >> log_E1_half, x1 = c & (((size_t)1 << log_E1_half) - 1);
-        eq3(fe_load(E1 + 2 * x1), fe_load(E1 + 2 * x1 + 1), e);
-        scale = fe_load(E2 + x2);
-    } else {
-        eq3(fe_load(E2 + 2 * c), fe_load(E2 + 2 * c + 1), e);
-    }
-}
-static __device__ __forceinline__ void layer_eq_at(bool nested, const fe* E1, size_t E1_half, const fe* E2, size_t c, fe e[3], fe& scale) {
-    split_eq_at(nested, E1, __ffsll((long long)E1_half) - 1, E2, c, e, scale);
-}
 template <int NESTED>
 static __device__ __forceinline__ size_t split_eq_limit(size_t E2_len, int log_E1_half) {
     return NESTED ? ((size_t)E2_len << log_E1_half) : E2_len / 2;
@@ -376,22 +341,6 @@
 static __device__ __forceinline__ void partial_row_sum(fe v, fe* sh, fe* __restrict__ partial, size_t row) {
     v = fr_block_sum(v, sh);
     if (threadIdx.x == 0) fe_store(partial + row * gridDim.x + blockIdx.x, v);
-}
-
-template <int NC>
-static __device__ __forceinline__ void layer_terms(const Sh<NC>& l0, const Sh<NC>& r0, const Sh<NC>& l1, const Sh<NC>& r1, const fe e[3], bool nested,
-                                                   const fe& scale, fe& t0, fe& t2, fe& t3) {
-    Sh<NC> ml = sh_sub<NC>(l1, l0), mr = sh_sub<NC>(r1, r0);
-    Sh<NC> l2 = sh_add<NC>(l1, ml), r2 = sh_add<NC>(r1, mr);
-    Sh<NC> l3 = sh_add<NC>(l2, ml), r3 = sh_add<NC>(r2, mr);
-    t0 = Fr::mul(sh_local_mul<NC>(l0, r0), e[0]);
-    t2 = Fr::mul(sh_local_mul<NC>(l2, r2), e[1]);
-    t3 = Fr::mul(sh_local_mul<NC>(l3, r3), e[2]);
-    if (nested) {
-        t0 = Fr::mul(t0, scale);
-        t2 = Fr::mul(t2, scale);
-        t3 = Fr::mul(t3, scale);
-    }
 }
 
 template <class Out>
@@ -402,11 +351,6 @@
     if (threadIdx.x == 0) fe_store(out(1), s2);
     s3 = fr_block_sum(s3, sh);
     if (threadIdx.x == 0) fe_store(out(2), s3);
-}
-
-static __device__ __forceinline__ fe fold_pair(const fe* in, size_t i, const fe& r) {
-    fe lo = fe_load(in + 2 * i), hi = fe_load(in + 2 * i + 1);
-    return Fr::add(lo, Fr::mul(Fr::sub(hi, lo), r));
 }
 
 template <int NC>
@@ -832,14 +776,18 @@
     for (int c = 0; c < NC; c++) fe_store(res + (size_t)(2 * m + j) * NC + c, v.c[c]);
 }
 
+static constexpr size_t HOST_TAIL_CAP = 2048;
+static constexpr size_t HOST_TAIL_AREA = 3 * HOST_TAIL_CAP;
 struct alignas(64) RoundMailbox {
     uint32_t cmd[16];
     uint32_t pad0[16];
     uint32_t res_seq;
     uint32_t status;
-    uint32_t pad2[14];
+    uint32_t tail_n[3];
+    uint32_t pad2[11];
     fe res[4];
     unsigned long long dbg[8];
+    fe tail[HOST_TAIL_AREA];
 };
 static constexpr long long MB_TICKS_PER_S = 100000000ll;
 static int resident_timeout_s() {
@@ -849,10 +797,35 @@
 }
 static constexpr size_t ROUND_PERSIST_MAX = 2048;
 
+template <int NC>
+static __device__ __forceinline__ void layer_tail_out(const fe* la, const fe* lb, size_t len, const fe* E1, size_t E1_len, const fe* E2, size_t E2_len,
+                                                      fe* area, int nt) {
+    for (size_t i = threadIdx.x; i < len; i += nt) {
+        fe_store(area + i, fe_load(la + i));
+        if (NC == 2) fe_store(area + len + i, fe_load(lb + i));
+    }
+    fe* eq = area + NC * len;
+    for (size_t i = threadIdx.x; i < E1_len; i += nt) fe_store(eq + i, fe_load(E1 + i));
+    for (size_t i = threadIdx.x; i < E2_len; i += nt) fe_store(eq + E1_len + i, fe_load(E2 + i));
+}
+template <int NC>
+__global__ void __launch_bounds__(RT) k_layer_tail_out(const fe* la, const fe* lb, size_t len, const fe* E1, size_t E1_len, const fe* E2, size_t E2_len,
+                                                    fe* area) {
+    layer_tail_out<NC>(la, lb, len, E1, E1_len, E2, E2_len, area, RT);
+}
+static constexpr int TAIL_BACK_MAX = 8;
+struct TailBackArgs {
+    fe v[TAIL_BACK_MAX];
+    fe* dst[TAIL_BACK_MAX];
+};
+__global__ void __launch_bounds__(64) k_layer_tail_back(TailBackArgs a, int n) {
+    if ((int)threadIdx.x < n) fe_store(a.dst[threadIdx.x], a.v[threadIdx.x]);
+}
+
 template <int NC, int TRACE>
 __global__ void __launch_bounds__(RT) k_layer_rounds_persistent(fe* la0, fe* lb0, fe* la1, fe* lb1, int lcur, size_t len, fe* e1_0, fe* e1_1,
                                                              int c1, size_t E1_len, fe* e2_0, fe* e2_1, int c2, size_t E2_len, int nrounds,
-                                                             int bind_first, fe r_first, RoundMailbox* mb, long long timeout_ticks) {
+                                                             int bind_first, fe r_first, RoundMailbox* mb, long long timeout_ticks, int tail_out) {
     __shared__ fe sh16[16];
     __shared__ fe sh_r;
     __shared__ int sh_ok;
@@ -949,14 +922,25 @@
             tk0 = t;
         }
         if (round == nrounds) {
+            if (tail_out) {
+                layer_tail_out<NC>(la[lcur], lb[lcur], len, e1[c1], E1_len, e2[c2], E2_len, mb->tail, RT);
+                __threadfence_system();
+                __syncthreads();
+            }
             if (threadIdx.x == 0) {
                 mb->dbg[0] = (unsigned long long)tk_wait;
                 mb->dbg[1] = (unsigned long long)tk_bind;
                 mb->dbg[2] = (unsigned long long)tk_cubic;
                 mb->dbg[3] = (unsigned long long)tk_pub;
-                fe z = Fr::zero();
-                fe v[4] = {fe_load(la[lcur]), NC == 2 ? fe_load(lb[lcur]) : z, fe_load(la[lcur] + 1), NC == 2 ? fe_load(lb[lcur] + 1) : z};
-                for (int k = 0; k < 4; k++) fe_store(&mb->res[k], v[k]);
+                if (tail_out) {
+                    mb->tail_n[0] = (uint32_t)len;
+                    mb->tail_n[1] = (uint32_t)E1_len;
+                    mb->tail_n[2] = (uint32_t)E2_len;
+                } else {
+                    fe z = Fr::zero();
+                    fe v[4] = {fe_load(la[lcur]), NC == 2 ? fe_load(lb[lcur]) : z, fe_load(la[lcur] + 1), NC == 2 ? fe_load(lb[lcur] + 1) : z};
+                    for (int k = 0; k < 4; k++) fe_store(&mb->res[k], v[k]);
+                }
                 __threadfence_system();
                 __hip_atomic_store(&mb->res_seq, seq, __ATOMIC_RELEASE, __HIP_MEMORY_SCOPE_SYSTEM);
             }
@@ -1272,6 +1256,13 @@
     fe_store(out + 2 * i + 1, hi);
 }
 
+__global__ void __launch_bounds__(PT) k_eq_outer(const fe* __restrict__ hi, const fe* __restrict__ lo, int m, size_t n, fe* __restrict__ out) {
+    const size_t per = ((n / PT + gridDim.x - 1) / gridDim.x) * PT;
+    const size_t first = (size_t)blockIdx.x * per, end = first + per < n ? first + per : n;
+    const size_t mask = ((size_t)1 << m) - 1;
+    for (size_t i = first + threadIdx.x; i < end; i += PT) fe_store(out + i, Fr::mul(fe_load(hi + (i >> m)), fe_load(lo + (i & mask))));
+}
+
 __global__ void k_store_fe(fe* out, fe v) { fe_store(out, v); }
 __global__ void k_store_u32s(uint32_t* out, const uint32_t* __restrict__ in0, const uint32_t* __restrict__ in1, int n0, size_t stride0) {
     int i = threadIdx.x;
@@ -1505,13 +1496,34 @@
     for (int i = 0; i < 4; i++) fe_to_u64x4(cf[i], out_coeffs + 4 * i);
 }
 
+static constexpr int EQ_BUILD_MAX_NV = 13, EQ_OUTER_MAX_NV = 2 * EQ_BUILD_MAX_NV;
+static bool eq_by_levels(int nv) { return nv > EQ_OUTER_MAX_NV || getenv("COZK_EQ_LEVELS") != nullptr; }
+static size_t eq_tmp_entries(int nv) {
+    if (nv <= EQ_BUILD_MAX_NV) return 0;
+    if (eq_by_levels(nv)) return (size_t)1 << nv;
+    const int m = (nv + 1) / 2;
+    return ((size_t)1 << m) + ((size_t)1 << (nv - m));
+}
+static void eq_build_launch(cozk_ctx* ctx, const fe* r, int nv, fe* out) {
+    EqBuildPoint pt;
+    for (int j = 0; j < nv; j++) pt.r[j] = r[j];
+    for (int j = nv; j < EQ_BUILD_MAX_NV; j++) pt.r[j] = Fr::zero();
+    k_eq_build<<<1, 1024, 0, ctx->stream>>>(pt, nv, out);
+}
 static void eq_evals_device(cozk_ctx* ctx, const fe* r, int nv, fe* out, fe* tmp) {
-    if (nv <= 13) {
+    if (nv <= EQ_BUILD_MAX_NV) {
         (void)tmp;
-        EqBuildPoint pt;
-        for (int j = 0; j < nv; j++) pt.r[j] = r[j];
-        for (int j = nv; j < 13; j++) pt.r[j] = Fr::zero();
-        k_eq_build<<<1, 1024, 0, ctx->stream>>>(pt, nv, out);
+        eq_build_launch(ctx, r, nv, out);
+        HIP_TRY(hipGetLastError());
+        return;
+    }
+    if (!eq_by_levels(nv)) {
+        const int m = (nv + 1) / 2;
+        const size_t n = (size_t)1 << nv;
+        fe *lo = tmp, *hi = tmp + ((size_t)1 << m);
+        eq_build_launch(ctx, r + (nv - m), m, lo);
+        eq_build_launch(ctx, r, nv - m, hi);
+        k_eq_outer<<<grid_capped(n), PT, 0, ctx->stream>>>(hi, lo, m, n, out);
         HIP_TRY(hipGetLastError());
         return;
     }
@@ -1649,7 +1661,7 @@
         std::vector<fe> rr(nv);
         for (int j = 0; j < nv; j++) rr[j] = fe_from_u64x4(r + 4 * j);
         fe* d = dev_alloc_fe(n);
-        ctx->scratch2.reserve(n * sizeof(fe));
+        ctx->scratch2.reserve(eq_tmp_entries(nv) * sizeof(fe));
         eq_evals_device(ctx, rr.data(), nv, d, ctx->scratch2.as<fe>());
         *out = new cozk_vec{ctx, n, COZK_SCALAR_FR, d, n * sizeof(fe), true};
     });
@@ -2371,6 +2383,100 @@
     });
 }
 
+extern "C++" {
+static constexpr size_t HOST_TAIL_RESIDENT = 256, HOST_TAIL_LAUNCHED = 512;
+static size_t host_tail_max(bool resident) {
+    const char* s = getenv("COZK_HOST_TAIL_MAX");
+    const long n = s ? atol(s) : (long)(resident ? HOST_TAIL_RESIDENT : HOST_TAIL_LAUNCHED);
+    return n <= 0 ? 0 : ((size_t)n > HOST_TAIL_CAP ? HOST_TAIL_CAP : (size_t)n);
+}
+static RoundMailbox* ctx_mailbox(cozk_ctx* ctx) {
+    if (!ctx->mailbox) HIP_TRY(hipHostMalloc(&ctx->mailbox, sizeof(RoundMailbox), hipHostMallocMapped | hipHostMallocCoherent));
+    return (RoundMailbox*)ctx->mailbox;
+}
+static int spliteq_binds_left(size_t E1_len, size_t E2_len) {
+    int n = 0;
+    for (size_t v = E1_len; v > 1; v >>= 1) n++;
+    for (size_t v = E2_len; v > 1; v >>= 1) n++;
+    return n;
+}
+static bool host_tail_takes(LayerTailShape s, int nc, size_t tail_max, int binds) {
+    return s.len >= 2 && s.len <= tail_max && layer_tail_entries(nc, s.len, s.E1_len, s.E2_len) <= HOST_TAIL_AREA &&
+           spliteq_binds_left(s.E1_len, s.E2_len) >= binds;
+}
+template <int NC>
+static void layer_host_tail(cozk_ctx* ctx, cozk_layer* l, cozk_spliteq* e, fe* area, bool have_r, uint64_t rr[4], uint64_t pc[4], int round, int num_rounds,
+                            cozk_round_cb cb, void* user, uint64_t* out_r, uint64_t final_claims[16]) {
+    using clk = std::chrono::steady_clock;
+    const bool trace = trace_rounds();
+    LayerTailView t = layer_tail_view(area, NC, l->len, e->E1_len, e->E2_len);
+    double us_cb = 0;
+    const clk::time_point t_start = trace ? clk::now() : clk::time_point();
+    fe fin[4];
+    const int binds = layer_tail_rounds<NC>(
+        t, have_r, have_r ? fe_from_u64x4(rr) : Fr::zero(), num_rounds - round,
+        [&](int j, const fe s[3]) {
+            uint64_t coeffs[16], nc[4];
+            cubic_coeffs_out(s, pc, coeffs);
+            const clk::time_point t0 = trace ? clk::now() : clk::time_point();
+            if (cb(user, round + j, coeffs, rr, nc) != 0) throw CozkError(COZK_ERR_INTERNAL, "layer_prove_rounds: round callback failed");
+            if (trace) us_cb += std::chrono::duration<double, std::micro>(clk::now() - t0).count();
+            memcpy(out_r + 4 * (round + j), rr, 4 * sizeof(uint64_t));
+            memcpy(pc, nc, 4 * sizeof(uint64_t));
+            return fe_from_u64x4(rr);
+        },
+        fin);
+    COZK_REQUIRE(t.len == 2, "final_claims: layer must be fully bound (len == 2)");
+    for (int k = 0; k < 4; k++) fe_to_u64x4(fin[k], final_claims + 4 * k);
+    if (trace && num_rounds > round) {
+        const double us = std::chrono::duration<double, std::micro>(clk::now() - t_start).count();
+        fprintf(stderr, "[host tail] %d rounds from %zu elements: host us/round: callback %.1f compute %.1f\n", num_rounds - round, (size_t)l->len,
+                us_cb / (num_rounds - round), (us - us_cb) / (num_rounds - round));
+    }
+    for (int b = 0; b < binds; b++) {
+        (void)layer_advance(l);
+        (void)spliteq_advance(e);
+    }
+    COZK_REQUIRE(l->len == t.len && e->E1_len == t.E1_len && e->E2_len == t.E2_len, "layer_prove_rounds: host tail out of step with the layer");
+    if (!binds) return;
+    const size_t nback = layer_tail_entries(NC, t.len, t.E1_len, t.E2_len);
+    if (nback <= (size_t)TAIL_BACK_MAX) {
+        TailBackArgs a{};
+        int n = 0;
+        auto put = [&](fe* dst, const fe* src, size_t cnt) {
+            for (size_t i = 0; i < cnt; i++, n++) {
+                a.v[n] = src[i];
+                a.dst[n] = dst + i;
+            }
+        };
+        put(l->buf[l->cur][0], t.la, t.len);
+        if (NC == 2) put(l->buf[l->cur][1], t.lb, t.len);
+        put(e->E1[e->c1], t.E1, t.E1_len);
+        put(e->E2[e->c2], t.E2, t.E2_len);
+        k_layer_tail_back<<<1, 64, 0, ctx->stream>>>(a, n);
+        HIP_TRY(hipGetLastError());
+    } else {
+        HIP_TRY(hipMemcpyAsync(l->buf[l->cur][0], t.la, t.len * sizeof(fe), hipMemcpyHostToDevice, ctx->stream));
+        if (NC == 2) HIP_TRY(hipMemcpyAsync(l->buf[l->cur][1], t.lb, t.len * sizeof(fe), hipMemcpyHostToDevice, ctx->stream));
+        HIP_TRY(hipMemcpyAsync(e->E1[e->c1], t.E1, t.E1_len * sizeof(fe), hipMemcpyHostToDevice, ctx->stream));
+        if (t.E2_len) HIP_TRY(hipMemcpyAsync(e->E2[e->c2], t.E2, t.E2_len * sizeof(fe), hipMemcpyHostToDevice, ctx->stream));
+        HIP_TRY(hipStreamSynchronize(ctx->stream));
+    }
+}
+static void layer_host_tail_gathered(cozk_ctx* ctx, cozk_layer* l, cozk_spliteq* e, bool have_r, uint64_t rr[4], uint64_t pc[4], int round, int num_rounds,
+                                     cozk_round_cb cb, void* user, uint64_t* out_r, uint64_t final_claims[16]) {
+    RoundMailbox* mb = ctx_mailbox(ctx);
+    const bool rep3 = l->mode == COZK_MODE_REP3;
+    auto* const kernel = rep3 ? k_layer_tail_out<2> : k_layer_tail_out<1>;
+    kernel<<<1, RT, 0, ctx->stream>>>(l->buf[l->cur][0], l->buf[l->cur][1], l->len, e->E1[e->c1], e->E1_len, e->E2[e->c2], e->E2_len, mb->tail);
+    HIP_TRY(hipGetLastError());
+    stream_drain_by_flag(ctx);
+    std::atomic_thread_fence(std::memory_order_acquire);
+    if (rep3) layer_host_tail<2>(ctx, l, e, mb->tail, have_r, rr, pc, round, num_rounds, cb, user, out_r, final_claims);
+    else layer_host_tail<1>(ctx, l, e, mb->tail, have_r, rr, pc, round, num_rounds, cb, user, out_r, final_claims);
+}
+}
+
 int cozk_layer_prove_rounds(cozk_ctx* ctx, cozk_layer* l, cozk_spliteq* e, const uint64_t claim[4], int num_rounds, cozk_round_cb cb,
                             void* user, uint64_t* out_r, uint64_t final_claims[16]) {
     if (!ctx || !l || !e || !claim || !cb || !final_claims || num_rounds < 0 || (num_rounds > 0 && !out_r)) return COZK_ERR_INVALID_ARG;
@@ -2379,9 +2485,14 @@
     memcpy(pc, claim, sizeof pc);
     bool have_r = false;
     int round = 0;
+    const int nc_layer = l->mode == COZK_MODE_REP3 ? 2 : 1;
     bool allow_resident = !no_persist && ctx_resident_rounds_enabled(ctx);
     for (;;) {
+        bool host_tail = false;
         for (; round < num_rounds; round++) {
+            host_tail = host_tail_takes(LayerTailShape{l->len, e->E1_len, e->E2_len}, nc_layer, host_tail_max(allow_resident),
+                                        num_rounds - round + (have_r ? 1 : 0));
+            if (host_tail) break;
             if (allow_resident && l->len <= ROUND_PERSIST_MAX && l->len >= 2) break;
             int rc = cozk_layer_round(ctx, l, e, have_r ? rr : nullptr, pc, coeffs);
             if (rc != COZK_OK) return rc;
@@ -2402,21 +2513,37 @@
             }
             return cozk_layer_final_claims(ctx, l, final_claims);
         }
+        if (host_tail)
+            return cozk_guard(ctx, [&] { layer_host_tail_gathered(ctx, l, e, have_r, rr, pc, round, num_rounds, cb, user, out_r, final_claims); });
         int rounds_done = -1;
         int rc = cozk_guard(ctx, [&] {
             const int nrem = num_rounds - round;
             pingpong_ensure(l, 1 - l->cur, l->len);
-            if (!ctx->mailbox) HIP_TRY(hipHostMalloc(&ctx->mailbox, sizeof(RoundMailbox), hipHostMallocMapped | hipHostMallocCoherent));
-            RoundMailbox* mb = (RoundMailbox*)ctx->mailbox;
-            memset(mb, 0, sizeof *mb);
+            RoundMailbox* mb = ctx_mailbox(ctx);
+            memset(mb, 0, offsetof(RoundMailbox, tail));
             std::atomic_thread_fence(std::memory_order_seq_cst);
+            const int bind_first = have_r ? 1 : 0;
+            int nker = nrem;
+            {
+                const size_t tail_max = host_tail_max(true);
+                LayerTailShape sh{l->len, e->E1_len, e->E2_len};
+                if (bind_first) sh = layer_tail_shape_bound(sh);
+                for (int k = 1; k < nrem && tail_max; k++) {
+                    sh = layer_tail_shape_bound(sh);
+                    if (host_tail_takes(sh, nc_layer, tail_max, nrem - k)) {
+                        nker = k;
+                        break;
+                    }
+                }
+            }
+            const bool tail_out = nker < nrem;
             fe r_first = have_r ? fe_from_u64x4(rr) : Fr::zero();
             const long long ticks = (long long)resident_timeout_s() * MB_TICKS_PER_S;
             const bool rep3 = l->mode == COZK_MODE_REP3;
             auto* const kernel = rep3 ? (trace_rounds() ? k_layer_rounds_persistent<2, 1> : k_layer_rounds_persistent<2, 0>)
                                       : (trace_rounds() ? k_layer_rounds_persistent<1, 1> : k_layer_rounds_persistent<1, 0>);
             kernel<<<1, RT, 0, ctx->stream>>>(l->buf[0][0], l->buf[0][1], l->buf[1][0], l->buf[1][1], l->cur, l->len, e->E1[0], e->E1[1], e->c1, e->E1_len,
-                                              e->E2[0], e->E2[1], e->c2, e->E2_len, nrem, have_r ? 1 : 0, r_first, mb, ticks);
+                                              e->E2[0], e->E2[1], e->c2, e->E2_len, nker, bind_first, r_first, mb, ticks, tail_out ? 1 : 0);
             HIP_TRY(hipGetLastError());
             volatile uint32_t* res_seq = &mb->res_seq;
             volatile uint32_t* status = &mb->status;
@@ -2445,10 +2572,9 @@
                     (void)spliteq_advance(e);
                 }
             };
-            const int bind_first = have_r ? 1 : 0;
             int j = 0;
             bool alive = true;
-            for (; j < nrem; j++) {
+            for (; j < nker; j++) {
                 if (!(alive = wait_result((uint32_t)j + 1))) break;
                 const fe sres[3] = {mb->res[0], mb->res[1], mb->res[2]};
                 cubic_coeffs_out(sres, pc, coeffs);
@@ -2468,18 +2594,25 @@
                     }
                 }
             }
-            if (alive) alive = wait_result((uint32_t)nrem + 1);
+            if (alive) alive = wait_result((uint32_t)nker + 1);
             if (!alive) {
                 HIP_TRY(hipStreamSynchronize(ctx->stream));
                 mirror_binds(j > 0 ? j - 1 + bind_first : 0);
                 rounds_done = j;
                 return;
             }
-            for (int k = 0; k < 4; k++) fe_to_u64x4(mb->res[k], final_claims + 4 * k);
             if (trace_rounds())
-                fprintf(stderr, "[mailbox] %d rounds: device us/round: wait %.1f bind %.1f cubic %.1f publish %.1f\n", nrem,
-                        mb->dbg[0] / 100.0 / (nrem + 1), mb->dbg[1] / 100.0 / (nrem + 1), mb->dbg[2] / 100.0 / nrem, mb->dbg[3] / 100.0 / nrem);
-            mirror_binds(nrem + bind_first);
+                fprintf(stderr, "[mailbox] %d rounds: device us/round: wait %.1f bind %.1f cubic %.1f publish %.1f\n", nker,
+                        mb->dbg[0] / 100.0 / (nker + 1), mb->dbg[1] / 100.0 / (nker + 1), mb->dbg[2] / 100.0 / nker, mb->dbg[3] / 100.0 / nker);
+            mirror_binds(nker + bind_first);
+            if (!tail_out) {
+                for (int k = 0; k < 4; k++) fe_to_u64x4(mb->res[k], final_claims + 4 * k);
+                return;
+            }
+            COZK_REQUIRE(mb->tail_n[0] == l->len && mb->tail_n[1] == e->E1_len && mb->tail_n[2] == e->E2_len,
+                         "layer_prove_rounds: the resident kernel handed over another tail than expected");
+            if (rep3) layer_host_tail<2>(ctx, l, e, mb->tail, false, rr, pc, round + nker, num_rounds, cb, user, out_r, final_claims);
+            else layer_host_tail<1>(ctx, l, e, mb->tail, false, rr, pc, round + nker, num_rounds, cb, user, out_r, final_claims);
         });
         if (rc != COZK_OK || rounds_done < 0) return rc;
         round += rounds_done;
diff --git a/co-zkvms_amd/csrc/poly.hip.hpp b/co-zkvms_amd/csrc/poly.hip.hpp
--- a/co-zkvms_amd/csrc/poly.hip.hpp
+++ b/co-zkvms_amd/csrc/poly.hip.hpp
@@ -15,21 +15,21 @@
 }
 
 template <int NC>
-static __device__ __forceinline__ Sh<NC> sh_load(const fe* a, const fe* b, size_t i) {
+static FF_HD Sh<NC> sh_load(const fe* a, const fe* b, size_t i) {
     Sh<NC> s;
     s.c[0] = fe_load(a + i);
     if (NC == 2) s.c[NC - 1] = fe_load(b + i);
     return s;
 }
 template <int NC>
-static __device__ __forceinline__ Sh<NC> sh_load_or_zero(const fe* a, const fe* b, size_t i, size_t len) {
+static FF_HD Sh<NC> sh_load_or_zero(const fe* a, const fe* b, size_t i, size_t len) {
     if (i < len) return sh_load<NC>(a, b, i);
     Sh<NC> s;
     for (int k = 0; k < NC; k++) s.c[k] = Fr::zero();
     return s;
 }
 template <int NC>
-static __device__ __forceinline__ void sh_store(fe* a, fe* b, size_t i, const Sh<NC>& s) {
+static FF_HD void sh_store(fe* a, fe* b, size_t i, const Sh<NC>& s) {
     fe_store(a + i, s.c[0]);
     if (NC == 2) fe_store(b + i, s.c[NC - 1]);
 }
```

Measured after the change: 9.451 million cycles/s (median of 6 runs). 1.01x the previous value.
